# Gadersd/stable-diffusion-burn

Hardware: AMD Instinct MI355X
Metric: images/sec @512x512, 20-step DDIM CFG=7.5, SD v1.4 (higher is better)
Workload: dtype f32

## Files before the change

### stable_diffusion_burn_amd/build.py

```python
from __future__ import annotations

import hashlib
import os
import subprocess
import sys
from concurrent.futures import ThreadPoolExecutor
from pathlib import Path

PKG = Path(__file__).resolve().parent
CSRC = PKG / "csrc"
LIBDIR = PKG / "lib"
LIB = LIBDIR / "libsdmi.so"
OBJDIR = PKG / "build"
BINDIR = PKG / "bin"
CLI = BINDIR / "sdmi_sample"

SOURCES = ["k_gemm.hip", "k_gemm2.hip", "k_gemm2x.hip", "k_gemm3x.hip", "k_gemm3p.hip", "k_gemm_bf16.hip", "k_gemm_bf16x.hip", "k_gemm_bf16t.hip", "k_attn.hip", "k_attn_bf16.hip", "k_attn_split.hip", "k_norm.hip", "k_elem.hip", "k_img2img.hip", "k_inpaint.hip", "k_control.hip", "k_sampler.hip", "k_resize.hip", "k_lora.hip", "k_unpack.hip", "k_bf16.hip", "k_fp8.hip", "engine.cpp", "gemm_plan.cpp", "attn_plan.cpp", "multi.cpp", "mpk_reader.cpp", "safetensors_reader.cpp", "ckpt_keys.cpp", "lora_keys.cpp", "tokenizer.cpp", "prompt.cpp", "png_writer.cpp", "sdmi_capi.cpp"]
CLI_SOURCE = "sample_main.cpp"
HEADERS = [CLI_SOURCE] + sorted(p.name for p in CSRC.glob("*.hpp")) + sorted(p.name for p in CSRC.glob("*.inc")) + ["../../include/sdmi.h"]
ARCH = "gfx950"
CXXFLAGS = ["-O3", "-std=c++17", "-fPIC", f"--offload-arch={ARCH}", "-Wall", "-Wno-unused-function"]


def hipcc() -> str:
# ... 2 lines not shown
            return cand
    raise RuntimeError("hipcc not found")


_TOOLCHAIN = None


def _toolchain() -> bytes:
    global _TOOLCHAIN
    if _TOOLCHAIN is None:
        try:
            _TOOLCHAIN = subprocess.run([hipcc(), "--version"], capture_output=True, text=True, timeout=60).stdout.encode()
        except Exception:
            _TOOLCHAIN = b"unknown"
    return _TOOLCHAIN


def _digest() -> str:
    h = hashlib.sha256()
    h.update(_toolchain())
    for name in SOURCES + HEADERS:
        h.update(name.encode())
        h.update((CSRC / name).read_bytes())
    h.update(" ".join(CXXFLAGS).encode())
    return h.hexdigest()


def gen_tuning_table() -> None:
    _gen_table("gfx950_fp32.txt", "tuning_table.inc")
    _gen_table("gfx950_fp32_mfma.txt", "tuning_table_mfma.inc")
    _gen_table("gfx950_bf16.txt", "tuning_table_bf16.inc")
    _gen_table("gfx950_fp32_planes.txt", "tuning_table_planes.inc")
    _gen_table("gfx950_fp32_pairs.txt", "tuning_table_pairs.inc")


def _gen_table(src_name: str, out_name: str) -> None:
    src = PKG / "tuning" / src_name
    lines = []
    if src.exists():
        for ln in src.read_text().split():
            if "=" in ln and not ln.startswith("#"):
                key, val = ln.split("=")
                cfg, splits = val.split(",")
                lines.append(f'{{"{key}", {int(cfg)}, {int(splits)}}},')
    out = CSRC / out_name
    text = f"// generated by build.py from tuning/{src_name} -- do not edit\n" + "\n".join(lines) + "\n"
    if not out.exists() or out.read_text() != text:
        out.write_text(text)


def _unit_digest(src: str) -> str:
    h = hashlib.sha256()
    h.update(_toolchain())
    for name in [src] + HEADERS:
        h.update(name.encode())
        h.update((CSRC / name).read_bytes())
    h.update(" ".join(CXXFLAGS).encode())
    return h.hexdigest()


def _compile(src: str) -> Path:
    obj = OBJDIR / (src.replace("/", "_") + ".o")
    stamp = obj.with_suffix(".sha256")
    digest = _unit_digest(src)
    if obj.exists() and stamp.exists() and stamp.read_text().strip() == digest and not os.environ.get("SDMI_REBUILD_ALL"):
        return obj
# ... 42 lines not shown
```

### stable_diffusion_burn_amd/csrc/engine.cpp

```cpp
#include "engine.hpp"
#include "ckpt_keys.hpp"
#include "lora_keys.hpp"
#include "mpk_reader.hpp"
#include "safetensors_reader.hpp"

#include <dlfcn.h>

#include <algorithm>
#include <cmath>
#include <cstdarg>
#include <cstdio>
#include <cstring>
#include <fstream>
#include <sstream>

namespace sdmi {

static constexpr size_t kAlign = 256;
static constexpr size_t kSlabMin = (size_t)1 << 30;

DevPool::~DevPool() {
    for (auto& s : slabs_) (void)hipFree(s.base);
}

// ... 385 lines not shown
        s.fold_entries[2] = entry_index_.at(path + "/proj_out/weight");
    };

    add(this, "alphas_cumprod", 3, {1000}, nullptr);
    add_meta("n_steps", 1, 1000.f, 0.f, nullptr);

    lin(lin1_time_, "unet/lin1_time_embed", mc, ed, true, true);
    lin(lin2_time_, "unet/lin2_time_embed", ed, ed, true, true);
    struct Spec { BlockKind kind; const char* name; int cin, cout; };
    const Spec in_spec[12] = {
        {BK_CONV, "conv", cfg_.unet_in_ch, c1},   {BK_RES_ST, "rt1", c1, c1}, {BK_RES_ST, "rt2", c1, c1}, {BK_DOWN, "d1", c1, c1},
        {BK_RES_ST, "rt3", c1, c2}, {BK_RES_ST, "rt4", c2, c2}, {BK_DOWN, "d2", c2, c2},    {BK_RES_ST, "rt5", c2, c4},
        {BK_RES_ST, "rt6", c4, c4}, {BK_DOWN, "d3", c4, c4},    {BK_RES, "r1", c4, c4},     {BK_RES, "r2", c4, c4}};
    const Spec out_spec[12] = {
        {BK_RES, "r1", 2 * c4, c4},        {BK_RES, "r2", 2 * c4, c4},        {BK_RES_UP, "ru", 2 * c4, c4},
        {BK_RES_ST, "rt1", 2 * c4, c4},    {BK_RES_ST, "rt2", 2 * c4, c4},    {BK_RES_ST_UP, "rtu1", c4 + c2, c4},
        {BK_RES_ST, "rt3", c4 + c2, c2},   {BK_RES_ST, "rt4", 2 * c2, c2},    {BK_RES_ST_UP, "rtu2", c2 + c1, c2},
        {BK_RES_ST, "rt5", c2 + c1, c1},   {BK_RES_ST, "rt6", 2 * c1, c1},    {BK_RES_ST, "rt7", 2 * c1, c1}};
    in_blocks_.resize(12);
    out_blocks_.resize(12);
    auto def_block = [&](UBlock& b, const Spec& s, const std::string& root) {
        b.kind = s.kind; b.cin = s.cin; b.cout = s.cout;
        const std::string path = root + "/" + s.name;
        switch (s.kind) {
            case BK_CONV: conv(b.conv, path, s.cin, s.cout, 3); break;
            case BK_DOWN: conv(b.conv, path, s.cin, s.cout, 3, 2); fp8_copy(b.conv, path + "/weight"); break;
            case BK_RES: res(b.res, path, s.cin, s.cout, true); break;
            default:
                res(b.res, path + "/res", s.cin, s.cout, true);
                if (s.kind == BK_RES_ST || s.kind == BK_RES_ST_UP) spatial(b.st, path + "/transformer", s.cout);
                if (s.kind == BK_RES_UP || s.kind == BK_RES_ST_UP) { conv(b.up, path + "/upsample/conv", s.cout, s.cout, 3); fp8_copy(b.up, path + "/upsample/conv/weight"); }
        }
    };
    for (int i = 0; i < 12; ++i) def_block(in_blocks_[i], in_spec[i], "unet/input_blocks");
    res(mid_res1_, "unet/middle_block/res1", c4, c4, true);
    spatial(mid_st_, "unet/middle_block/transformer", c4);
    res(mid_res2_, "unet/middle_block/res2", c4, c4, true);
    for (int i = 0; i < 12; ++i) def_block(out_blocks_[i], out_spec[i], "unet/output_blocks");
    norm(unet_norm_out_, "unet/norm_out", c1);
    conv(unet_conv_out_, "unet/conv_out", c1, 4, 3);

    auto idx_res = [&](ResW& r) { r.temb_index = (int)res_list_.size(); res_list_.push_back(&r); };
    auto idx_st = [&](SpatialW& s) {
        s.ctx_index = (int)st_list_.size();
        st_list_.push_back(&s);
        for (int i : s.fold_entries) entries_[(size_t)i].fold_st = s.ctx_index;
    };
    auto idx_block = [&](UBlock& b) {
        if (b.kind == BK_CONV || b.kind == BK_DOWN) return;
        idx_res(b.res);
        if (b.kind == BK_RES_ST || b.kind == BK_RES_ST_UP) idx_st(b.st);
    };
    for (auto& b : in_blocks_) idx_block(b);
    idx_res(mid_res1_); idx_st(mid_st_); idx_res(mid_res2_);
    for (auto& b : out_blocks_) idx_block(b);
    n_res_unet_ = res_list_.size();
    n_st_unet_ = st_list_.size();

    const int vc = cfg_.vae_ch;
    const int dch[4][2] = {{4 * vc, 4 * vc}, {4 * vc, 4 * vc}, {4 * vc, 2 * vc}, {2 * vc, vc}};
    conv(post_quant_, "autoencoder/post_quant_conv", 4, 4, 1);
    conv(dec_conv_in_, "autoencoder/decoder/conv_in", 4, 4 * vc, 3);
    res(dec_mid1_, "autoencoder/decoder/mid/block_1", 4 * vc, 4 * vc, false);
    dec_attn_.c = 4 * vc;
    norm(dec_attn_.norm, "autoencoder/decoder/mid/attn/norm", 4 * vc);
    conv(dec_attn_.q, "autoencoder/decoder/mid/attn/q", 4 * vc, 4 * vc, 1);
    conv(dec_attn_.k, "autoencoder/decoder/mid/attn/k", 4 * vc, 4 * vc, 1);
    conv(dec_attn_.v, "autoencoder/decoder/mid/attn/v", 4 * vc, 4 * vc, 1);
    conv(dec_attn_.proj_out, "autoencoder/decoder/mid/attn/proj_out", 4 * vc, 4 * vc, 1);
    res(dec_mid2_, "autoencoder/decoder/mid/block_2", 4 * vc, 4 * vc, false);
    for (int i = 0; i < 4; ++i) {
        DecBlockW& b = dec_blocks_[i];
        b.cin = dch[i][0]; b.cout = dch[i][1]; b.has_up = i != 3;
        const std::string bp = "autoencoder/decoder/blocks/" + std::to_string(i);
        res(b.res[0], bp + "/res1", b.cin, b.cout, false);
        res(b.res[1], bp + "/res2", b.cout, b.cout, false);
        res(b.res[2], bp + "/res3", b.cout, b.cout, false);
        if (b.has_up) conv(b.upsampler, bp + "/upsampler", b.cout, b.cout, 3);
    }
    norm(dec_norm_out_, "autoencoder/decoder/norm_out", vc);
    conv(dec_conv_out_, "autoencoder/decoder/conv_out", vc, 3, 3);

    if (cfg_.clip_layers > 0) {
        const int cs = cd, L = cfg_.clip_layers, H = cfg_.clip_heads;
        if (H <= 0 || cs % H || !attn_supported_head_dim(cs / H) || cfg_.clip_vocab <= 0 || cfg_.clip_ctx <= 0 || cs % 32)
            throw Error(SDMI_ERR_UNSUPPORTED, "CLIP: ctx_dim / clip_heads must be one of the fused attention head dims (40, 64, 80, 160)");
        cur_group_ = 1;
        add(this, "clip/token_embedding/weight", 2, {cfg_.clip_vocab, cs}, &clip_tok_);
        add(this, "clip/position_embedding/weight", 2, {cfg_.clip_ctx, cs}, &clip_pos_);
        clip_blocks_.resize(L);
        for (int i = 0; i < L; ++i) {
            ClipBlockW& b = clip_blocks_[i];
            const std::string bp = "clip/blocks/" + std::to_string(i);
            void* w = persistent_alloc((size_t)3 * cs * cs * sizeof(float));
            weight_allocs_.push_back(w);
            void* bias = persistent_alloc((size_t)3 * cs * sizeof(float));
            weight_allocs_.push_back(bias);
            b.q.bt = reinterpret_cast<float*>(w); b.k.bt = b.q.bt + (size_t)cs * cs; b.v.bt = b.q.bt + (size_t)2 * cs * cs;
            b.q.bias = reinterpret_cast<float*>(bias); b.k.bias = b.q.bias + cs; b.v.bias = b.q.bias + 2 * cs;
            norm(b.attn_ln, bp + "/attn_ln", cs, false);
            lin(b.q, bp + "/attn/query", cs, cs, true, true);
            lin(b.k, bp + "/attn/key", cs, cs, true, true);
            lin(b.v, bp + "/attn/value", cs, cs, true, true);
            lin(b.out, bp + "/attn/out", cs, cs, true, true);
            norm(b.mlp_ln, bp + "/mlp_ln", cs, false);
            lin(b.fc1, bp + "/mlp/fc1", cs, 4 * cs, true, true);
            lin(b.fc2, bp + "/mlp/fc2", 4 * cs, cs, true, true);
        }
        norm(clip_ln_, "clip/layer_norm", cs, false);
        cur_group_ = 0;
    }
// ... 565 lines not shown
}


void Engine::fold_weights(const float* proj_bt, const float* lin_bt, const float* lin_bias, int cout, int cmid, int k_main, float* wf, float* bf) {
    ProfScope ps(this, PC_OTHER, 2.0 * cout * (double)cmid * k_main, ((double)cout * cmid + (double)cmid * k_main + (double)cout * k_main) * 4.0);
    ps.set_tag("fold %d,%d,%d", cout, k_main, cmid);
    SDMI_HIP(launch_fold_matmul_f64(proj_bt, lin_bt, wf, cout, cmid, k_main, cmid, k_main, k_main, stream_));
    if (lin_bias) SDMI_HIP(launch_fold_matmul_f64(proj_bt, lin_bias, bf, cout, cmid, 1, cmid, 1, 1, stream_));
    else SDMI_HIP(hipMemsetAsync(bf, 0, (size_t)cout * sizeof(float), stream_));
}

void Engine::rebuild_folds() {
    if (bf16_) return;
    for (SpatialW* s : st_list_) {
        if (s->fold_fresh || s->fold_entries[0] < 0) continue;
        bool ready = true;
        for (int i : s->fold_entries) ready = ready && entries_[(size_t)i].set;
        const int C = s->c;
        if (!ready || C % 32 || !split_planes(s->proj_out.bt) || !split_planes(s->mlp_lin.bt)) continue;
        const size_t w_bytes = (size_t)C * 4 * C * sizeof(float);
        if (!s->fold_bt) {
            char* base = static_cast<char*>(persistent_alloc(w_bytes + (size_t)C * sizeof(float)));
            weight_allocs_.push_back(base);
            char* planes = static_cast<char*>(persistent_alloc(w_bytes / 2 * 3));
            weight_allocs_.push_back(planes);
            split_regions_.push_back(SplitRegion{base, w_bytes, planes});
            s->fold_bt = reinterpret_cast<float*>(base);
            s->fold_bias = reinterpret_cast<float*>(base + w_bytes);
        }
        fold_weights(s->proj_out.bt, s->mlp_lin.bt, s->mlp_lin.bias, C, C, 4 * C, s->fold_bt, s->fold_bias);
        SDMI_HIP(launch_pack_split3(s->fold_bt, const_cast<void*>(split_planes(s->fold_bt)), C, 4 * C, stream_, b3_grouped(C)));
        s->fold_fresh = true;
    }
}
bool Engine::lora_owned(const sdmi_lora* a) const { return a && std::find(loras_.begin(), loras_.end(), a) != loras_.end(); }

bool Engine::lora_active_on(int entry) const {
    for (const sdmi_lora* a : loras_) {
        if (a->scale == 0) continue;
        for (const LoraTarget& t : a->targets)
            if (t.entry == entry) return true;
    }
    return false;
}

void Engine::lora_refuse_bulk_load(const char* what) const {
    for (const sdmi_lora* a : loras_)
        if (a->scale != 0 && !a->targets.empty())
            throw Error(SDMI_ERR_STATE, std::string(what) + ": a LoRA adapter with a non-zero scale is attached: set its scale to 0 first");
}

sdmi_lora* Engine::lora_create() {
    if (!finalized_) throw Error(SDMI_ERR_STATE, "lora_create: weights not finalized");
    if (!opt_keep_masters_) throw Error(SDMI_ERR_STATE, "lora_create: the context keeps no fp32 master weights (option keep_masters=1, set before the weights are loaded)");
    sdmi_lora* a = new sdmi_lora{};
    a->engine = this;
    loras_.push_back(a);
    return a;
}

void Engine::lora_add(sdmi_lora* a, const char* target, const float* down, const float* up, int rank, float alpha) {
    if (!lora_owned(a)) throw Error(SDMI_ERR_INVALID, "lora_add: not an adapter of this context");
    if (!target || !down || !up) throw Error(SDMI_ERR_INVALID, "lora_add: null argument");
    if (a->scale != 0) throw Error(SDMI_ERR_STATE, "lora_add: targets are added while the adapter's scale is 0");
    auto it = entry_index_.find(target);
    if (it == entry_index_.end()) throw Error(SDMI_ERR_INVALID, std::string("lora_add: unknown tensor '") + target + "'");
    const WeightEntry& e = entries_[it->second];
// ... 344 lines not shown
    else if (key == "attn_kv_splits") aopt_.attn_kv_splits = std::stoi(value);
    else if (key == "attn_kv_prefer8") aopt_.attn_kv_prefer8 = std::stoi(value);
    else if (key == "b3_grouped") {
        if (!entries_.empty() && std::any_of(entries_.begin(), entries_.end(), [](const WeightEntry& w) { return w.set; }))
            throw Error(SDMI_ERR_STATE, "b3_grouped selects the layout the weight planes are packed in: set it before the first weight is loaded");
        opt_b3_grouped_ = std::stoi(value);
    }
    else if (key == "keep_masters") {
        if (std::any_of(entries_.begin(), entries_.end(), [](const WeightEntry& w) { return w.set; }) || arena_done_[0] || arena_done_[1] || arena_done_[2] || arena_done_[3])
            throw Error(SDMI_ERR_STATE, "keep_masters decides what the weight arenas hold: set it before the first weight is loaded");
        opt_keep_masters_ = std::stoi(value) != 0;
    }
    else if (key == "attn_pack_tail") aopt_.attn_pack_tail = (value == "default") ? AttnPlanOpts().attn_pack_tail : std::stoi(value);
    else if (key == "gn32_min_wgs") opt_gn32_min_wgs_ = (opt_gn32_min_wgs_ & ~0xFFFF) | (std::stoi(value) & 0xFFFF);
    else if (key == "gn32_stats_min_wgs") opt_gn32_min_wgs_ = (opt_gn32_min_wgs_ & 0xFFFF) | ((std::stoi(value) + 1) << 16);
    else if (key == "gn_target_wgs") gn_tune_.target_wgs = std::stoi(value);
    else if (key == "gn_max_threads") gn_tune_.max_threads = std::stoi(value);
    else if (key == "gn_unroll") gn_tune_.unroll = std::stoi(value);
    else if (key == "fp8_tile") opt_fp8_tile_ = (value == "auto") ? -1 : std::stoi(value);
    else if (key == "resid_acc") opt_resid_acc_ = std::stoi(value);
    else if (key == "attn_bf16") aopt_.attn_bf16 = std::stoi(value);
    else if (key == "attn_bf16_variant") aopt_.attn_bf16_variant = (value == "default") ? AttnPlanOpts().attn_bf16_variant : std::stoi(value, nullptr, 0);
    else if (key == "attn_split") aopt_.attn_split = std::stoi(value);
    else if (key == "gemm_bf16x") gopt_.gemm_bf16x = std::stoi(value);
    else if (key == "gemm_x32") gopt_.gemm_x32 = std::stoi(value);
    else if (key == "gemm_f32s") gopt_.gemm_f32s = std::stoi(value);
    else if (key == "bench_cold") opt_bench_cold_ = std::stoi(value);
    else if (key == "gemm_probe") opt_gemm_probe_ = std::stoi(value);
    else if (key == "conv3_reuse") gopt_.conv3_reuse = std::stoi(value);
    else if (key == "gemm_planes") gopt_.gemm_planes = (value == "default") ? GemmPlanOpts().gemm_planes : std::stoi(value);
    else if (key == "gemm3x_variant") opt_gemm3x_variant_ = (value == "default") ? kGemm3xVariantDefault : std::stoi(value);
    else if (key == "gemm_bf16x_variant") opt_gemm_bf16x_variant_ = (value == "default") ? kGemmBf16xVariantDefault : std::stoi(value);
    else if (key == "geglu_fuse") opt_geglu_fuse_ = std::stoi(value);
    else if (key == "record_shapes") { record_shapes_ = std::stoi(value) != 0; if (record_shapes_) { shape_counts_.clear(); choice_counts_.clear(); } }
    else if (key == "dump_shapes") {
        std::ofstream f(value);
        if (!f) throw Error(SDMI_ERR_IO, "dump_shapes: cannot write " + value);
        for (auto& kv : shape_counts_) f << kv.first << " " << kv.second << "\n";
    }
    else if (key == "dump_choices") {
        std::ofstream f(value);
        if (!f) throw Error(SDMI_ERR_IO, "dump_choices: cannot write " + value);
        for (auto& kv : choice_counts_) f << kv.first << " x" << kv.second << "\n";
    }
    else if (key == "profile") { prof_flush(); profiling_ = std::stoi(value) != 0; prof_tagging_ = std::stoi(value) >= 2; if (profiling_) prof_calibrate(); }
    else if (key == "dump_profile_tags") {
        prof_flush();
        std::ofstream f(value);
        if (!f) throw Error(SDMI_ERR_IO, "dump_profile_tags: cannot write " + value);
        for (auto& kv : prof_tags_) f << kv.second.ms << " " << kv.second.launches << " " << kv.second.flops << " " << kv.second.bytes << "\t" << kv.first << "\n";
    }
    else if (key == "profile_reset") prof_reset();
    else if (key == "tune" || key == "tune_bf16") tuning_.set(value, key == "tune_bf16");
    else if (key == "tune_clear") tuning_.clear();
    else throw Error(SDMI_ERR_INVALID, "unknown option '" + key + "'");
}

void Engine::set_resid_acc(ConvGemm& p, bool eligible, bool resid_ok) const {
    p.resid_acc = 0;
    if (!eligible || (p.N % 8) || (p.ldc % 8)) return;
    if ((opt_resid_acc_ & 1) && p.resid && resid_ok && (p.ldr % 4) == 0 && ((uintptr_t)p.resid & 7) == 0) p.resid_acc |= 1;
    if ((opt_resid_acc_ & 2) && (p.bias || p.rowvec) && (p.rowvec_stride % 4) == 0 && (((uintptr_t)p.bias | (uintptr_t)p.rowvec) & 15) == 0) p.resid_acc |= 2;
}

void Engine::record_choice(const ConvGemm& p, const char* kind, int cfg, const char* note) {
    if (!record_shapes_) return;
// ... 80 lines not shown
    std::unique_ptr<Buf> a3_tmp;
    if (a_planes && !p.A3) {
        const long long rows = (long long)p.NB * p.Hs * p.Ws;
        p.a3_ld = (p.Cin / 32) * 192;
        a3_tmp.reset(new Buf(this, (size_t)rows * p.a3_ld));
        ProfScope ps(this, PC_SPLIT_ROWS, 0, (double)rows * p.Cin * 10.0);
        SDMI_HIP(launch_split3_rows(p.A, a3_tmp->p, rows, p.Cin, p.a_ld, p.a3_ld, stream_));
        count_kernel();
        p.A3 = a3_tmp->p;
    }
    set_resid_acc(p, in_dt && g.tile.family == kFamX && g.splits == 1, !p.geglu);
    record_choice(p, "", g.cfg, p.Bt3 || in_dt ? "" : " (no planes)");
    const double a_es = in_dt ? 2.0 : (a_planes ? 6.0 : 4.0), w_es = in_dt ? 2.0 : (w_planes ? 6.0 : 4.0);
    const double c_es = in_dt ? (p.out_mode == 1 ? 4.0 : 2.0) : (p.out_mode == 2 ? 2.0 : ((p.C ? 4.0 : 0.0) + (c3_native ? 6.0 : 0.0)));
    const double gemm_bytes = (double)p.NB * p.Hs * p.Ws * p.Cin * a_es + (double)p.N * (p.geglu ? 2.0 : 1.0) * p.K * w_es + (double)p.M * p.N * c_es;
    static const GemmLauncher kLaunchers[2][kNumGemmFamilies] = {{launch_conv_gemm2, launch_conv_gemm2x, launch_conv_gemm3x, launch_conv_gemm3p},
                                                                 {launch_conv_gemm_bf16, launch_conv_gemm_bf16_large, nullptr, nullptr}};
    run_gemm(p, GemmRun{kLaunchers[in_dt ? 1 : 0][g.tile.family], g.tile.index, "gemm", g.cfg, w_planes ? PC_CONV_SPLIT : PC_CONV_GEMM, in_dt != 0, true, flops, gemm_bytes});
    if (c3_want && !c3_native) {
        ProfScope ps(this, PC_SPLIT_ROWS, 0, (double)p.M * p.N * 10.0);
        SDMI_HIP(launch_split3_rows(p.C, c3_want, p.M, p.N, p.ldc, ldc3_want, stream_));
        count_kernel();
    }
}

void Engine::conv(const ConvW& w, const Act& x, Act& y, int stride, int ups, const float* rowvec, int rowvec_stride,
                  const Act* resid, bool pad_br) {
    if (x.c != w.cin) throw Error(SDMI_ERR_INVALID, "conv: input channels mismatch");
    const int pad = pad_br ? 0 : (w.k == 3 ? 1 : 0);
    const int hin = x.h << ups, win = x.w << ups;
    const int extra = pad_br ? 1 : 0;
    const int ho = (hin + 2 * pad + extra - w.k) / stride + 1, wo = (win + 2 * pad + extra - w.k) / stride + 1;
    if (y.n != x.n || y.h != ho || y.w != wo || y.c != w.cout) throw Error(SDMI_ERR_INVALID, "conv: output shape mismatch");
    ConvGemm p{};
    const int resid_dt = (!x.dt && y.dt) ? 0 : y.dt;
    if (resid && !x.dt && y.dt && (w.cout % 4 || y.stride() % 4 || resid->stride() % 4))
        throw Error(SDMI_ERR_STATE, "conv: a residual on an fp32 -> bf16 layer needs cout and the row strides to be multiples of 4");
    if (resid && (resid->rows() != y.rows() || resid->c != y.c || resid->dt != resid_dt)) throw Error(SDMI_ERR_STATE, "conv: residual shape / type mismatch");
    p.A = x.p; p.Bt = w.bt; p.C = y.p; p.bias = w.bias; p.rowvec = rowvec; p.resid = resid ? resid->p : nullptr;
    if (resid && !resid->p) throw Error(SDMI_ERR_STATE, "conv: the residual must exist as fp32");
    if (!x.dt && plane_gemm(w.cin, w.cout) && split_planes(w.bt)) { p.A3 = x.p3; p.a3_ld = x.ld3; }
    if (!x.p && !p.A3) throw Error(SDMI_ERR_STATE, "conv: the input exists only as planes, which this layer cannot read");
    p.C3 = y.p3; p.ldc3 = y.ld3;
    p.M = x.n * ho * wo; p.N = w.cout; p.K = w.cin * w.k * w.k;
    p.NB = x.n; p.Hs = x.h; p.Ws = x.w; p.Cin = w.cin; p.Ho = ho; p.Wo = wo;
    p.KH = w.k; p.KW = w.k; p.stride = stride; p.pad = pad; p.ups = ups;
    p.ldc = y.stride(); p.ldr = resid ? resid->stride() : y.stride(); p.a_ld = x.stride(); p.b_ld = p.K; p.rowvec_stride = rowvec_stride;
    p.CS = std::min(32, w.cin);
    if (!y.p && !y.p3) throw Error(SDMI_ERR_STATE, "conv: no output buffer");
    if (x.dt != w.dt) throw Error(SDMI_ERR_STATE, "conv: activation / weight storage types disagree");
    p.out_mode = x.dt ? (y.dt ? 0 : 1) : (y.dt ? 2 : 0);
    launch_gemm(p, x.dt);
}

bool Engine::conv_pair(const ConvW& w_out, const Act& h, const ConvW& w_skip, const Act& x, Act& y) {
    if (bf16_ || h.dt || x.dt || y.dt || w_out.dt || w_skip.dt || w_out.k != 3 || w_skip.k != 1 || probe_buf_) return false;
    if (h.c != w_out.cin || x.c != w_skip.cin || w_out.cout != w_skip.cout || y.c != w_out.cout) return false;
    if (h.n != x.n || h.h != x.h || h.w != x.w || y.n != h.n || y.h != h.h || y.w != h.w) return false;
    if (!plane_gemm(w_out.cin, w_out.cout) || !plane_gemm(w_skip.cin, w_skip.cout) || !h.p3 || !x.p3 || (!y.p && !y.p3)) return false;
    if (gopt_.force_splits > 0 && opt_splitk_aux_ <= 0) return false;
    ConvGemm p{};
    p.Bt = w_out.bt; p.bias = w_out.bias; p.bias_aux = w_skip.bias;
    p.Bt3 = split_planes(w_out.bt); p.Bt3_aux = split_planes(w_skip.bt);
    if (!p.Bt3 || !p.Bt3_aux) return false;
    p.A3 = h.p3; p.a3_ld = h.ld3; p.A3_aux = x.p3; p.a3_ld_aux = x.ld3;
    p.C = y.p; p.C3 = y.p3; p.ldc3 = y.ld3;
    p.M = (int)h.rows(); p.N = w_out.cout; p.K = w_out.cin * 9;
    p.NB = h.n; p.Hs = h.h; p.Ws = h.w; p.Cin = w_out.cin; p.Ho = h.h; p.Wo = h.w;
    p.KH = 3; p.KW = 3; p.stride = 1; p.pad = 1; p.ups = 0;
    p.ldc = y.p ? y.stride() : p.N; p.ldr = p.ldc; p.a_ld = h.stride(); p.b_ld = p.K; p.CS = 32;
    p.kt_total = p.K / 32; p.Cin_aux = w_skip.cin; p.kt_total_aux = w_skip.cin / 32;
    p.b3_grouped = b3_grouped(p.N) ? 1 : 0;
    p.variant = opt_gemm3x_variant_;
    p.zero_page = zero_page_;
    if (!splitk_reduce_vec(p, false) || ((uintptr_t)p.bias_aux & 15) || (p.C3 && (p.N % 32 || p.ldc3 % 192))) return false;
    const GemmPlanIn in = gemm_plan_in(p, 0, -1, 0);
    if (!in.p_ok) return false;
    if ((unsigned long long)p.N * (unsigned long long)p.kt_total_aux * 192ull >= 0xFFFFFF00ull || (unsigned long long)p.NB * p.Hs * p.Ws * (unsigned long long)p.a3_ld_aux >= 0xFFFFFF00ull) return false;
    const GemmPairPlan g = plan_gemm_pair(in, w_skip.cin, p.kt_total_aux, gopt_, tuning_, opt_splitk_aux_ > 0 ? std::max(gopt_.force_splits, 1) : 0, std::max(opt_splitk_aux_, 0));
    if (!g.pair) return false;
    p.kt_per_split = g.kt_per_split; p.splits = g.splits_main + g.splits_aux; p.z_aux = g.splits_main;
    if (record_shapes_) {
        char note[48];
        std::snprintf(note, sizeof note, " +aux K%d z%d", w_skip.cin, p.z_aux);
        record_choice(p, " pair", g.cfg, note);
// ... 1592 lines not shown
        Act r = y;
        r.view = true; r.p3 = nullptr;
        r.ld = epi->resid_ld ? epi->resid_ld : y.c;
        r.p = const_cast<float*>(stage_epi(rb, epi->resid, y.rows(), y.c, r.ld, y.dt, (long long)y.h * y.w));
        return r;
    };
    if (!opt_op_f32_ && fp8_ && opt_fp8_convs_ && k == 3 && stride == 1 && !ups && cin % 32 == 0 && cout % 8 == 0) {
        const int cp = (cin + 127) / 128 * 128;
        ConvW w; w.cin = cin; w.cout = cout; w.k = 3; w.dt = 1; w.bias = const_cast<float*>(bias);
        Buf bt8(this, (size_t)cout * cp * 9), bs8(this, (size_t)cout * cp * 9 / 32);
        SDMI_HIP(launch_pack_conv_weight_fp8(wt, bt8.p, bs8.p, cout, cin, 3, 3, stream_));
        w.bt8 = bt8.f(); w.bs8 = bs8.f();
        Act a32 = new_act(n, h, wd, cin, 0);
        SDMI_HIP(launch_nchw_to_nhwc(x, a32.p, n, cin, h, wd, 1.0f, stream_));
        ActQ q = new_actq(n, h, wd, cin);
        SDMI_HIP(launch_quantize_fp8(a32.p, q.q, q.s, a32.rows(), cin, stream_));
        release(a32);
        Act y = new_act(n, h, wd, cout, 1);
        Act r;
        if (epi && epi->resid) r = epi_resid(y);
        conv_fp8(w, q, y, temb, r.p ? &r : nullptr, 1, 0, epi ? epi->temb_stride : 0);
        SDMI_HIP(launch_nhwc_bf16_to_nchw_f32(y.p, out, n, cout, h, wd, stream_));
        release(q); release(y);
        return;
    }
    ConvW w; w.cin = cin; w.cout = cout; w.k = k;
    w.dt = (bf16_ && cin % 64 == 0 && !opt_op_f32_) ? 1 : 0;
    if (bf16_ && !w.dt && cin >= 32 && !opt_op_f32_) throw Error(SDMI_ERR_UNSUPPORTED, "bf16 conv2d: Cin must be a multiple of 64 (or < 32)");
    Buf bt(this, (size_t)cout * cin * k * k * 4);
    if (w.dt) SDMI_HIP(launch_pack_conv_weight_bf16(wt, bt.p, cout, cin, k, k, stream_));
    else SDMI_HIP(launch_pack_conv_weight(wt, bt.f(), cout, cin, k, k, stream_));
    TempSplit planes(this, bt.f(), w.dt ? 0 : cout, (long long)cin * k * k);
    w.bt = bt.f(); w.bias = const_cast<float*>(bias);
    Act a = new_act(n, h, wd, cin, w.dt);
    if (w.dt) SDMI_HIP(launch_nchw_f32_to_nhwc_bf16(x, a.p, n, cin, h, wd, 1.0f, stream_));
    else SDMI_HIP(launch_nchw_to_nhwc(x, a.p, n, cin, h, wd, 1.0f, stream_));
    const int hin = h << ups, win = wd << ups;
    const int ho = (hin + 2 * pad - k) / stride + 1, wo = (win + 2 * pad - k) / stride + 1;
    Act y = new_act(n, ho, wo, cout, (bf16_ && cout > 4 && !opt_op_f32_) ? 1 : 0);
    const bool with_resid = opt_op_resid_ && cin == cout && stride == 1 && !ups && a.dt == y.dt;
    Act r;
    if (epi && epi->resid) r = epi_resid(y);
    conv(w, a, y, stride, ups, temb, epi ? epi->temb_stride : 0, r.p ? &r : with_resid ? &a : nullptr);
    if (y.dt) SDMI_HIP(launch_nhwc_bf16_to_nchw_f32(y.p, out, n, cout, ho, wo, stream_));
    else SDMI_HIP(launch_nhwc_to_nchw(y.p, out, n, cout, ho, wo, stream_));
    release(a); release(y);
}

void Engine::op_conv2d_pair(const float* x, const float* hp, const float* w_skip, const float* b_skip, const float* w_out, const float* b_out, int n, int cin_x, int cout,
                            int h, int wd, float* out, float* out3) {
    if (n <= 0 || h <= 0 || wd <= 0 || cin_x <= 0 || cout <= 0) throw Error(SDMI_ERR_INVALID, "conv2d_pair: bad shape");
    if (bf16_ || !plane_gemm(cin_x, cout) || !plane_gemm(cout, cout)) throw Error(SDMI_ERR_UNSUPPORTED, "conv2d_pair: the fp32 plane kernels only (channels in multiples of 32)");
    Buf bt_o(this, (size_t)cout * cout * 9 * 4), bt_s(this, (size_t)cout * cin_x * 4);
    SDMI_HIP(launch_pack_conv_weight(w_out, bt_o.f(), cout, cout, 3, 3, stream_));
    SDMI_HIP(launch_pack_conv_weight(w_skip, bt_s.f(), cout, cin_x, 1, 1, stream_));
    TempSplit po(this, bt_o.f(), cout, (long long)cout * 9), psk(this, bt_s.f(), cout, cin_x);
    ConvW wo; wo.cin = cout; wo.cout = cout; wo.k = 3; wo.bt = bt_o.f(); wo.bias = const_cast<float*>(b_out);
    ConvW ws; ws.cin = cin_x; ws.cout = cout; ws.k = 1; ws.bt = bt_s.f(); ws.bias = const_cast<float*>(b_skip);
    Act ax = new_act3(n, h, wd, cin_x, 3), ah = new_act3(n, h, wd, cout, 3);
    SDMI_HIP(launch_nchw_to_nhwc(x, ax.p, n, cin_x, h, wd, 1.0f, stream_));
    SDMI_HIP(launch_nchw_to_nhwc(hp, ah.p, n, cout, h, wd, 1.0f, stream_));
    SDMI_HIP(launch_split3_rows(ax.p, ax.p3, ax.rows(), cin_x, cin_x, ax.ld3, stream_));
    SDMI_HIP(launch_split3_rows(ah.p, ah.p3, ah.rows(), cout, cout, ah.ld3, stream_));
    Act y = new_act3(n, h, wd, cout, out3 ? 3 : 1);
    if (opt_skip_slices_) {
        if (!conv_pair(wo, ah, ws, ax, y)) throw Error(SDMI_ERR_UNSUPPORTED, "conv2d_pair: this shape / these options do not pair (skip_slices=0 runs the two launches)");
// ... 86 lines not shown
            if (y.p) SDMI_HIP(hipMemcpyAsync(yp, y.p, y.bytes(), hipMemcpyDeviceToDevice, stream_));
            if (y.p3) SDMI_HIP(launch_join3_rows(y.p3, y.p ? yp3 : yp, y.rows(), v.out_ld, y.ld3, v.out_ld, stream_));
        }
    };
    try {
        Act xs = slice(a, v.in_off, cin), ys = slice(y, v.out_off, cout);
        std::unique_ptr<Buf> tb, rb;
        const float* temb = (epi && epi->temb) ? stage_epi(tb, epi->temb, epi->temb_stride ? n : 1, cout, epi->temb_stride ? epi->temb_stride : cout, 0) : nullptr;
        Act r;
        if (epi && epi->resid) {
            if (!ys.p) throw Error(SDMI_ERR_INVALID, "view: a residual needs the output as fp32");
            r = ys;
            r.view = true; r.p3 = nullptr;
            r.ld = epi->resid_ld ? epi->resid_ld : cout;
            r.p = const_cast<float*>(stage_epi(rb, epi->resid, ys.rows(), cout, r.ld, ydt, (long long)ho * wo));
        }
        if (q8) {
            const int cp = (cin + 127) / 128 * 128;
            ConvW w; w.cin = cin; w.cout = cout; w.k = 3; w.dt = 1; w.bias = const_cast<float*>(bias);
            Buf bt8(this, (size_t)cout * cp * 9), bs8(this, (size_t)cout * cp * 9 / 32);
            SDMI_HIP(launch_pack_conv_weight_fp8(wt, bt8.p, bs8.p, cout, cin, 3, 3, stream_));
            w.bt8 = bt8.f(); w.bs8 = bs8.f();
            ActQ q = new_actq(n, h, wd, cin);
            quantize(xs, q);
            conv_fp8(w, q, ys, temb, r.p ? &r : nullptr, 1, 0, epi ? epi->temb_stride : 0);
            release(q);
        } else {
            ConvW w; w.cin = cin; w.cout = cout; w.k = k; w.dt = wdt;
            Buf bt(this, (size_t)cout * cin * k * k * 4);
            if (w.dt) SDMI_HIP(launch_pack_conv_weight_bf16(wt, bt.p, cout, cin, k, k, stream_));
            else SDMI_HIP(launch_pack_conv_weight(wt, bt.f(), cout, cin, k, k, stream_));
            TempSplit planes(this, bt.f(), w.dt ? 0 : cout, (long long)cin * k * k);
            w.bt = bt.f(); w.bias = const_cast<float*>(bias);
            conv(w, xs, ys, stride, ups, temb, epi ? epi->temb_stride : 0, r.p ? &r : nullptr);
        }
    } catch (...) {
        try { give_back(); } catch (...) {}
        throw;
    }
    give_back();
    release(a); release(y);
}

void Engine::op_linear_view(const float* x, const float* wt, const float* bias, int rows, int cin, int cout, const sdmi_op_view& v, const EpiOps* epi, float* yp) {
    check_view(v, cin, cout);
    if (v.in_ld != cin || v.in_off || v.in_planes > 1 || v.out_planes > 1)
        throw Error(SDMI_ERR_UNSUPPORTED, "linear view: Engine::gemm reads dense rows and writes fp32 / bf16 slices only");
    const int rld = (epi && epi->resid) ? (epi->resid_ld ? epi->resid_ld : cout) : 0;
    const bool q8 = fp8_ && opt_fp8_ops_ && cin % 32 == 0 && cout % 8 == 0;
    const int dt = (q8 || (bf16_ && cin % 64 == 0)) ? 1 : 0;
    Act y = new_act(1, 1, rows, v.out_ld, dt);
    if (dt) SDMI_HIP(launch_f32_to_bf16(yp, y.p, (long long)rows * v.out_ld, stream_));
    else SDMI_HIP(hipMemcpyAsync(y.p, yp, y.bytes(), hipMemcpyDeviceToDevice, stream_));
    auto give_back = [&] {
        if (dt) SDMI_HIP(launch_nhwc_bf16_to_nchw_f32(y.p, yp, rows, v.out_ld, 1, 1, stream_));
        else SDMI_HIP(hipMemcpyAsync(yp, y.p, y.bytes(), hipMemcpyDeviceToDevice, stream_));
    };
    try {
            Act ys = slice(y, v.out_off, cout);
            std::unique_ptr<Buf> rb;
            const float* resid = rld ? stage_epi(rb, epi->resid, rows, cout, rld, dt) : nullptr;
            if (q8) {
                const size_t kp = (size_t)(cin + 127) / 128 * 128;
                Buf xh(this, (size_t)rows * cin * 2), w8(this, (size_t)cout * kp), s8(this, (size_t)cout * kp / 32);
                SDMI_HIP(launch_f32_to_bf16(x, xh.p, (long long)rows * cin, stream_));
                SDMI_HIP(launch_pack_linear_weight_fp8(wt, w8.p, s8.p, cin, cout, stream_));
// ... 252 lines not shown
        try {
            conv_fp8(cw, q, y, nullptr, nullptr);
            SDMI_HIP(hipEventRecord(ev0_, stream_));
            for (int i = 0; i < iters; ++i) conv_fp8(cw, q, y, nullptr, nullptr);
            SDMI_HIP(hipEventRecord(ev1_, stream_));
            SDMI_HIP(hipEventSynchronize(ev1_));
            SDMI_HIP(hipEventElapsedTime(&ms, ev0_, ev1_));
        } catch (...) {
            release(x32); release(y); release(q);
            throw;
        }
        release(x32); release(y); release(q);
        return (double)ms / std::max(1, iters);
    }
    const int wdt = (bf16_ && cin % 64 == 0) ? 1 : 0;
    Act a = new_act(n, h, w, cin, wdt), y = new_act(n, ho, wo, cout, (bf16_ && cout > 4) ? 1 : 0);
    Buf bt(this, (size_t)cout * cin * k * k * 4), bias(this, (size_t)cout * 4);
    {
        Buf tmp(this, std::max((size_t)a.rows() * cin, (size_t)cout * cin * k * k) * 4);
        SDMI_HIP(launch_fill_normal(wdt ? tmp.f() : a.p, (long long)a.rows() * cin, 11, stream_));
        if (wdt) SDMI_HIP(launch_f32_to_bf16(tmp.f(), a.p, (long long)a.rows() * cin, stream_));
        SDMI_HIP(launch_fill_normal(wdt ? tmp.f() : bt.f(), (long long)cout * cin * k * k, 12, stream_));
        if (wdt) SDMI_HIP(launch_f32_to_bf16(tmp.f(), bt.p, (long long)cout * cin * k * k, stream_));
        SDMI_HIP(hipStreamSynchronize(stream_));
    }
    SDMI_HIP(launch_fill_normal(bias.f(), cout, 13, stream_));
    TempSplit planes(this, bt.f(), wdt ? 0 : cout, (long long)cin * k * k);
    const bool plane_tile = tile_cfg >= 0 && gemm_tile_id(tile_cfg).family == kFamP;
    if (!wdt && plane_tile && cin % 32 == 0) {
        a.p3 = pool_.alloc(a.bytes3()); a.ld3 = (cin / 32) * 192;
        SDMI_HIP(launch_split3_rows(a.p, a.p3, a.rows(), cin, cin, a.ld3, stream_));
    }
    ConvW cw; cw.cin = cin; cw.cout = cout; cw.k = k; cw.bt = bt.f(); cw.bias = bias.f(); cw.dt = wdt;
    const OptRestore r1{gopt_.force_tile}, r2{gopt_.force_splits}, r3{gopt_.gemm_planes};
    gopt_.force_tile = tile_cfg; gopt_.force_splits = splitk;
    if (plane_tile && !gopt_.gemm_planes) gopt_.gemm_planes = 2;
    float ms = 0;
    try {
        conv(cw, a, y, stride, ups, nullptr, 0, nullptr);
        if (opt_bench_cold_) {
            const size_t flush_bytes = (size_t)512 << 20;
            Buf flush(this, flush_bytes);
            Buf a_copy(this, a.bytes());
            SDMI_HIP(hipMemcpyAsync(a_copy.p, a.p, a.bytes(), hipMemcpyDeviceToDevice, stream_));
            for (int i = 0; i < iters; ++i) {
                SDMI_HIP(hipMemsetAsync(flush.p, i, flush_bytes, stream_));
                SDMI_HIP(hipMemcpyAsync(a.p, a_copy.p, a.bytes(), hipMemcpyDeviceToDevice, stream_));
                if (a.p3) SDMI_HIP(launch_split3_rows(a.p, a.p3, a.rows(), cin, cin, a.ld3, stream_));
                SDMI_HIP(hipEventRecord(ev0_, stream_));
                conv(cw, a, y, stride, ups, nullptr, 0, nullptr);
                SDMI_HIP(hipEventRecord(ev1_, stream_));
                SDMI_HIP(hipEventSynchronize(ev1_));
                float t = 0;
                SDMI_HIP(hipEventElapsedTime(&t, ev0_, ev1_));
                ms += t;
            }
        } else {
        SDMI_HIP(hipEventRecord(ev0_, stream_));
        for (int i = 0; i < iters; ++i) conv(cw, a, y, stride, ups, nullptr, 0, nullptr);
        SDMI_HIP(hipEventRecord(ev1_, stream_));
        SDMI_HIP(hipEventSynchronize(ev1_));
        SDMI_HIP(hipEventElapsedTime(&ms, ev0_, ev1_));
        }
        if (opt_gemm_probe_ && a.p3) {
            constexpr size_t kMaxBlocks = kGemmProbeBlocks;
            Buf pb(this, kMaxBlocks * 24 * sizeof(unsigned long long));
// ... 52 lines not shown
```

### stable_diffusion_burn_amd/csrc/engine.hpp

```cpp
#pragma once
#include <hip/hip_runtime.h>

#include <functional>
#include <map>
#include <memory>
#include <stdexcept>
#include <string>
#include <vector>

#include "../../include/sdmi.h"
#include "error.hpp"
#include "gemm_plan.hpp"
#include "kernels.hpp"

namespace sdmi {

#define SDMI_HIP(expr)                                                                                   \
    do {                                                                                                 \
        hipError_t _e = (expr);                                                                          \
        if (_e != hipSuccess)                                                                            \
            throw ::sdmi::Error(SDMI_ERR_HIP, std::string(#expr) + ": " + hipGetErrorString(_e) + " (" + \
                                                  __FILE__ + ":" + std::to_string(__LINE__) + ")");      \
    } while (0)

// ... 9 lines not shown
    void set_stream(hipStream_t s) { stream_ = s; }
    void set_fill(int byte) { fill_ = byte; }
    int fill() const { return fill_; }
    void note_fill(size_t bytes) { ++fill_blocks_; fill_bytes_ += bytes; }
    void take_fill_counts(unsigned long long* blocks, unsigned long long* bytes) { *blocks = fill_blocks_; *bytes = fill_bytes_; fill_blocks_ = fill_bytes_ = 0; }

private:
    struct Block { size_t off, size; };
    struct Slab { char* base; size_t size; std::vector<Block> free_list; };
    std::vector<Slab> slabs_;
    struct Live { int slab; size_t size; unsigned long long serial; };
    std::map<void*, Live> live_;
    size_t reserved_ = 0, in_use_ = 0, high_ = 0;
    unsigned long long serial_ = 0;
    hipStream_t stream_ = nullptr;
    int fill_ = -1;
    unsigned long long fill_blocks_ = 0, fill_bytes_ = 0;
};

struct Act {
    float* p = nullptr;
    int n = 0, h = 0, w = 0, c = 0;
    int dt = 0;
    int ld = 0;
    bool view = false;
    void* p3 = nullptr;
    int ld3 = 0;
    size_t bytes3() const { return (size_t)rows() * (size_t)(c / 32) * 192; }
    long long rows() const { return (long long)n * h * w; }
    int stride() const { return ld ? ld : c; }
    size_t bytes() const { return (size_t)rows() * c * (dt ? 2 : 4); }
};

struct ConvW { float* bt = nullptr; float* bias = nullptr; int cin = 0, cout = 0, k = 1; int dt = 0; float* bt8 = nullptr; float* bs8 = nullptr; };
struct ActQ {
    void* q = nullptr; void* s = nullptr;
    int n = 0, h = 0, w = 0, c = 0, cp = 0;
    long long rows() const { return (long long)n * h * w; }
};
struct LinW { float* bt = nullptr; float* bias = nullptr; int cin = 0, cout = 0; int dt = 0; float* bt8 = nullptr; float* bs8 = nullptr; };
struct NormW { float* gamma = nullptr; float* beta = nullptr; int c = 0; float eps = 1e-5f; };

struct ResW {
    NormW norm_in; ConvW conv_in; LinW lin_embed; NormW norm_out; ConvW conv_out; ConvW skip;
    bool has_skip = false, has_embed = false;
    int cin = 0, cout = 0, temb_index = -1;
};
struct MhaW { LinW q, k, v, out; };
struct SpatialW {
    NormW norm; ConvW proj_in, proj_out; NormW ln1, ln2, ln3; MhaW attn1, attn2; LinW geglu_proj, mlp_lin;
    int c = 0, ctx_index = -1;
    float* fold_bt = nullptr; float* fold_bias = nullptr;
    bool fold_fresh = false;
    int fold_entries[3] = {-1, -1, -1};
};
enum BlockKind { BK_CONV, BK_DOWN, BK_RES, BK_RES_ST, BK_RES_UP, BK_RES_ST_UP };
struct UBlock { BlockKind kind; int cin, cout; ConvW conv; ResW res; SpatialW st; ConvW up; };
struct VaeAttnW { NormW norm; ConvW q, k, v, proj_out; int c = 0; };
struct DecBlockW { ResW res[3]; ConvW upsampler; bool has_up = false; int cin = 0, cout = 0; };

struct ClipBlockW { NormW attn_ln, mlp_ln; LinW q, k, v, out, fc1, fc2; };

struct WeightEntry {
    std::string name;
    int kind;
    int ndim;
    int64_t dims[4];
    float** dst;
    int wdt = 0;
    int group = 0;
    float** dst8 = nullptr;
    float** dsts = nullptr;
    float pre_scale = 1.f;
    bool set = false;
    int fold_st = -1;
    float* master = nullptr;
};

struct LoraTarget { int entry; int rank; double alpha; const void* down; const void* up; int dtype = 0; int kind = 0; const void* down2 = nullptr; const void* up2 = nullptr; };

struct MetaEntry { std::string name; int n; float expect[2]; float* store; };

class Engine {
public:
    explicit Engine(const sdmi_config& cfg);
    ~Engine();
    Engine(const Engine&) = delete;
    Engine& operator=(const Engine&) = delete;

    void set_weight(const char* name, const float* data, int ndim, const int64_t* dims);
    void load_weights_dir(const char* dir);
    void load_weights_mpk(const char* path);
    void load_weights_safetensors(const char* path);
    void load_safetensors_groups(const char* path, bool control);
    void load_control_safetensors(const char* path);
    void load_weights_packed(const float* data, size_t n_floats, int groups);
    size_t packed_size(int groups) const;
    void finalize_weights();
    const std::vector<WeightEntry>& entries() const { return entries_; }
    sdmi_lora* lora_create();
    void lora_add(sdmi_lora* a, const char* target, const float* down, const float* up, int rank, float alpha);
    void lora_set_scale(sdmi_lora* a, double scale);
    void lora_destroy(sdmi_lora* a);
    sdmi_lora* lora_load_safetensors(const char* path, int which, int flags, int* n_skipped);
    static int64_t padded_conv_cin(int64_t cin);
    void effective_weight(const char* name, float* out, size_t n);

    void unet_forward_dev(const float* x_nchw, int t, const float* context, int n, int T, float* out_nchw, const float* cond_nchw = nullptr);
// ... 141 lines not shown
    std::vector<sdmi_lora*> loras_;
    bool lora_owned(const sdmi_lora* a) const;
    void lora_refuse_bulk_load(const char* what) const;
    bool lora_active_on(int entry) const;
    void lora_compose(int entry, float* dst);
    void lora_repack(int entry);
    void upload_weight(WeightEntry& e, const float* data);
    void stager_release();
    void ensure_arena(int group);
    bool set_meta(const std::string& name, const float* values, size_t n);
    void add_meta(const std::string& name, int n, float e0, float e1, float* store);
    std::vector<MetaEntry> meta_;
    std::map<std::string, int> meta_index_;
    void add_entry(const std::string& name, int kind, std::initializer_list<int64_t> dims, float** dst, int wdt = 0);
    int cur_group_ = 0;
    void build_model();

    Act new_act(int n, int h, int w, int c, int dt = -1);
    Act new_act3(int n, int h, int w, int c, int what);
    void release(Act& a);
    void probe_report(void* pb_dev, size_t max_blocks, int n, int cin, int h, int w, int cout, int k, int tile_cfg, int splitk);
    void conv(const ConvW& w, const Act& x, Act& y, int stride, int ups, const float* rowvec, int rowvec_stride,
              const Act* resid, bool pad_br = false);
    bool conv_pair(const ConvW& w_out, const Act& h, const ConvW& w_skip, const Act& x, Act& y);
    struct LinearPair {
        const void* u3; int u3_ld; const float* bt; const float* bias; int k_main;
        const void* h3; int h3_ld; const float* bt_aux; const float* bias_aux; int k_aux;
        int rows, cout; const float* resid; int ldr; float* C; int ldc; void* C3; int ldc3;
        bool measured_only = false;
    };
    bool linear_pair(const LinearPair& a, bool plan_only = false);
    void fold_weights(const float* proj_bt, const float* lin_bt, const float* lin_bias, int cout, int cmid, int k_main, float* wf, float* bf);
    void rebuild_folds();
    void fold_touch(const WeightEntry& e) { if (e.fold_st >= 0) st_list_[(size_t)e.fold_st]->fold_fresh = false; }
    static Act slice(const Act& parent, int c_off, int c);
    void gemm(const float* A, int a_rows, const float* bt, const float* bias, int cin, int cout, float* C, int ldc,
              const float* resid, int ldr, int dt = -1, int out_mode = 0, const void* A3 = nullptr, void* C3 = nullptr);
    bool plane_gemm(int cin, int cout) const { return !bf16_ && gopt_.gemm_planes != 0 && gopt_.gemm_f32s != 0 && cin % 32 == 0 && cout >= 32; }
    void launch_gemm(ConvGemm& p, int in_dt, int force_cfg = -1, int force_splits = 0);
    GemmPlanIn gemm_plan_in(const ConvGemm& p, int in_dt, int force_cfg, int force_splits) const;
    using GemmLauncher = hipError_t (*)(const ConvGemm&, int, hipStream_t);
    struct GemmRun { GemmLauncher launch; int index; const char* what; int cfg; int pc; bool bf16_reduce, reduce_tag; double flops, bytes; };
    void record_choice(const ConvGemm& p, const char* kind, int cfg, const char* note);
    void run_gemm(ConvGemm& p, const GemmRun& r);
    int edt() const { return bf16_ ? 1 : 0; }
    size_t esz() const { return bf16_ ? 2 : 4; }
    static float* adv(const float* p, long long elems, int dt) { return (float*)((char*)const_cast<float*>(p) + elems * (dt ? 2 : 4)); }
    void group_norm(const NormW& w, const Act& x, Act& y, bool silu);
    ActQ new_actq(int n, int h, int w, int c);
    void release(ActQ& a);
    void group_norm_fp8(const NormW& w, const Act& x, ActQ& y, bool silu);
    void conv_fp8(const ConvW& w, const ActQ& x, Act& y, const float* rowvec, const Act* resid, int stride = 1, int ups = 0, int rowvec_stride = 0);
    bool use_fp8(const ConvW& w, const Act& x) const;
    bool use_fp8_wide(const float* bt8, long long rows) const { return fp8_ && opt_fp8_convs_ && opt_fp8_linear_ && bt8 && rows >= opt_fp8_min_rows_; }
    void set_resid_acc(ConvGemm& p, bool eligible, bool resid_ok) const;
    void launch_fp8(ConvGemm& p, double flops);
    void gemm_fp8(const ActQ& x, const LinW& w, int n_rows_w, void* C, int ldc, const float* resid, int ldr);
    void conv_raw(const ConvW& w, const Act& x, Act& y, int stride, int ups);
    void quantize(const Act& x, ActQ& y);
    void layer_norm_fp8(const NormW& w, const float* x, long long rows, ActQ& y);
    ActQ new_rowsq(long long rows, int c) { return new_actq(1, 1, (int)rows, c); }
    void layer_norm(const NormW& w, const float* x, long long rows, float* y, int dt = -1, void* y3 = nullptr);
    void gemm_geglu(const float* x, long long rows, const float* bt, const float* bias, int cin, int hidden, float* out, int dt,
                    const void* x3 = nullptr, void* out3 = nullptr);
    void attention(const float* q, int ldq, long long q_bs, const float* k, int ldk, long long k_bs, const float* v,
                   int ldv, long long v_bs, float* o, int ldo, long long o_bs, int n, int nq, int nk, int n_head,
                   int d_head, const int* kv_len_dev, const int* kv_len_host, const float* mask, int mask_ld, int dt = -1, void* o3 = nullptr, bool q_log2 = false);
// ... 190 lines not shown
```

### stable_diffusion_burn_amd/csrc/gemm_plan.cpp

```cpp
#include "gemm_plan.hpp"

#include <algorithm>
#include <cstdio>

#include "error.hpp"

namespace sdmi {

struct TuneRow { const char* key; int cfg, splits; };
static const TuneRow kTuneRows[] = {
#include "tuning_table.inc"
    {nullptr, 0, 0},
#include "tuning_table_mfma.inc"
    {nullptr, 0, 0},
#include "tuning_table_planes.inc"
    {nullptr, 0, 0},
#include "tuning_table_bf16.inc"
    {nullptr, 0, 0}};

static const TuneRow kPairRows[] = {
#include "tuning_table_pairs.inc"
    {nullptr, 0, 0}};

struct CostRow { int bf16; GemmFamily family; int n; double eff[kNumGemmTiles]; double flop, rate, wg, area_num, area_den; };
static const CostRow kCost[] = {
    {0, kFam4, kNumGemmTiles, {0.85, 0.75, 0.60, 0.90, 0.75, 0.85, 0.75, 0.85, 0.65, 0.75}, 64.0, 256.0, 3000.0, 0.0, 1.0},
    {0, kFamX, kNumGemmTilesX, {0.90, 0.90, 0.88, 0.90}, 64.0, 256.0, 8000.0, 4.0, 10.0},
    {0, kFamS, kNumGemmTilesS, {0.55, 0.55, 0.52, 0.52, 0.46, 0.44}, 384.0, 4096.0, 8000.0, 4.0, 10.0},
    {0, kFamP, kNumGemmTilesP, {0.62, 0.60, 0.60, 0.52, 0.50, 0.34, 0.40, 0.50, 0.40}, 384.0, 4096.0, 8000.0, 4.0, 10.0},
    {1, kFam4, kNumGemmTiles, {0.31, 0.22, 0.16, 0.22, 0.20, 0.20, 0.22, 0.26, 0.15, 0.28}, 128.0, 4096.0, 3000.0, 0.0, 1.0},
    {1, kFamX, kNumGemmTilesX, {0.54, 0.46, 0.38, 0.48}, 128.0, 4096.0, 6000.0, 2.0, 20.0}};
static const int kSplitOpts[] = {1, 2, 3, 4, 6, 8, 12, 16, 24, 32, 48};

static TileChoice cost_model(int bf16, unsigned families, int M, int N, int kt_total, bool pairs_only) {
    const int n_cu = 256;
    double best = 1e300;
    TileChoice bc{0, 1};
    for (const CostRow& r : kCost) {
        if (r.bf16 != bf16 || !(families >> r.family & 1)) continue;
        for (int c = 0; c < r.n; ++c) {
            const GemmTileInfo& ti = kGemmFamilies[r.family].tiles[c];
            if (pairs_only && !ti.geglu_pairs) continue;
            const int bm = ti.bm, bn = ti.bn;
            const long long tiles = (long long)((M + bm - 1) / bm) * ((N + bn - 1) / bn);
            const double overhead = r.wg + bm * bn * r.area_num / r.area_den;
            for (int s : kSplitOpts) {
                if (s > 1 && kt_total / s < 4) break;
                const int kt_per = (kt_total + s - 1) / s;
                const long long wgs = tiles * ((kt_total + kt_per - 1) / kt_per);
                const double per_cu = (double)((wgs + n_cu - 1) / n_cu);
                double t = per_cu * ((double)bm * bn * kt_per * r.flop / r.rate / r.eff[c] + overhead);
                if (s > 1) t += 8000.0 + (double)M * N * 4.0 * (s + 1) / (5.0e12 / 2.4e9);
                if (t < best) { best = t; bc = {kGemmFamilies[r.family].base + c, s}; }
            }
        }
    }
    return bc;
}

static int clamp_splits(int splits, int kt_total, int* kt_per_split) {
    splits = std::max(1, std::min(splits, kt_total));
    *kt_per_split = (kt_total + splits - 1) / splits;
    return (kt_total + *kt_per_split - 1) / *kt_per_split;
}

static const TileChoice* find(const std::map<std::string, TileChoice>& m, const char* key) {
    const auto it = m.find(key);
    return it == m.end() ? nullptr : &it->second;
}

static TileChoice plane_choice(const GemmTuning& t, const char* key, int M, int N, int kt_total, bool pairs_only) {
    if (const TileChoice* tc = find(t.planes, key)) {
        const GemmTileId id = gemm_tile_id(tc->cfg);
        if (!(pairs_only && id.family == kFamP && id.in_range(false) && !id.info().geglu_pairs)) return *tc;
    }
    return cost_model(0, 1u << kFamP, M, N, kt_total, pairs_only);
}

void GemmTuning::load_builtin() {
    std::map<std::string, TileChoice>* const tables[] = {&f32, &mfma, &planes, &bf16};
    int t = 0;
    for (const TuneRow& r : kTuneRows)
        if (r.key) (*tables[t])[r.key] = TileChoice{r.cfg, r.splits};
        else ++t;
    for (const TuneRow& r : kPairRows)
        if (r.key) pairs[r.key] = TileChoice{r.cfg, r.splits};
}

void GemmTuning::set(const std::string& value, bool b16) {
    const size_t eq = value.find('=');
    if (eq == std::string::npos) throw Error(SDMI_ERR_INVALID, "tune expects M,N,K=cfg,splits");
    TileChoice tc{0, 1};
    if (!b16 && value.find('+') < eq) {
        if (std::sscanf(value.c_str() + eq + 1, "%d,%d", &tc.cfg, &tc.splits) != 2 || tc.splits < 0 || gemm_tile_id(tc.cfg).family != kFamP || !gemm_tile_id(tc.cfg).in_range(false))
            throw Error(SDMI_ERR_INVALID, "tune: a pair row is M,N,Kmain+Kaux=cfg,kt_per_split with a plane tile (300 + x)");
        pairs[value.substr(0, eq)] = tc;
        return;
    }
    if (std::sscanf(value.c_str() + eq + 1, "%d,%d", &tc.cfg, &tc.splits) != 2 || tc.cfg < 0 || tc.splits < 1 || !gemm_tile_id(tc.cfg).in_range(b16))
        throw Error(SDMI_ERR_INVALID, "tune: bad value");
    (b16 ? bf16 : (gemm_tile_id(tc.cfg).family == kFamP ? planes : f32))[value.substr(0, eq)] = tc;
}

GemmPlan plan_gemm(const GemmPlanIn& in, const GemmPlanOpts& o, const GemmTuning& t) {
    if (in.from_planes && !in.p_ok)
        throw Error(in.s_ok ? SDMI_ERR_UNSUPPORTED : SDMI_ERR_STATE,
                    in.s_ok ? "fp32 GEMM: an activation tensor stored as bf16 planes (6 bytes per element) reaches 4 GiB (32-bit piece offsets): lower the batch (at 64x64x960 the CFG "
                              "batch 2n must stay <= 182) or set option gemm_planes=0"
                            : "gemm: activation planes given for a layer the plane kernel does not take");
    auto applicable = [&](int f) { return f == kFam4 || in.bf16 || (f == kFamP ? in.p_ok : f == kFamS ? in.s_ok : in.x32_ok); };
    auto enabled = [&](int f) { return f == kFam4 || (in.bf16 ? o.gemm_bf16x != 0 : f == kFamX ? o.gemm_x32 != 0 : f == kFamS ? o.gemm_f32s != 0 : true); };
    auto usable = [&](const TileChoice* tc) { return tc && applicable(gemm_tile_id(tc->cfg).family) && enabled(gemm_tile_id(tc->cfg).family); };
    char key[64];
    std::snprintf(key, sizeof key, "%d,%d,%d", in.M, in.N, in.K);
    const TileChoice* const t1 = find(in.bf16 ? t.bf16 : t.f32, key);
    const TileChoice* const t2 = in.bf16 ? nullptr : find(t.mfma, key);
    TileChoice tc;
    if (in.from_planes) tc = plane_choice(t, key, in.M, in.N, in.kt_total, in.geglu != 0);
    else if (usable(t1)) tc = *t1;
    else if (usable(t2)) tc = *t2;
    else {
        unsigned fams = 0;
        for (int f : {kFam4, kFamX, kFamS})
            if (applicable(f) && enabled(f)) fams |= 1u << f;
        tc = cost_model(in.bf16, fams, in.M, in.N, in.kt_total, false);
    }
    bool tile_forced = false;
    if (o.force_tile >= 0 && (in.from_planes ? gemm_tile_id(o.force_tile).family == kFamP : applicable(gemm_tile_id(o.force_tile).family))) { tc.cfg = o.force_tile; tile_forced = true; }
    if (o.force_splits > 0) tc.splits = o.force_splits;
// ... 25 lines not shown
    const int ktm = main.kt_total;
    auto slices = [](int kt_total, int kt) { return (kt_total + kt - 1) / kt; };
    int kt = 0;
    if (force_main > 0 || force_aux > 0) {
        const int sm = std::max(1, std::min(force_main, ktm)), sa = std::max(1, std::min(force_aux, kt_aux));
        kt = std::max(slices(ktm, sm), slices(kt_aux, sa));
    } else {
        char key[80];
        std::snprintf(key, sizeof key, "%d,%d,%d+%d", main.M, main.N, main.K, k_aux);
        const TileChoice* const row = g.tile_forced ? nullptr : find(t.pairs, key);
        if (row) {
            if (row->splits <= 0) return pp;
            const GemmTileId id = gemm_tile_id(row->cfg);
            if (id.family != kFamP || !id.in_range(false)) throw Error(SDMI_ERR_INVALID, "pairs table: not a plane tile");
            pp.tile = id; pp.cfg = id.cfg();
            kt = std::min(row->splits, std::max(ktm, kt_aux));
        } else {
            if (g.splits <= 1) return pp;
            const GemmTileInfo& ti = g.tile.info();
            const long long tiles = (long long)((main.M + ti.bm - 1) / ti.bm) * ((main.N + ti.bn - 1) / ti.bn);
            const long long rounds_today = (tiles * g.splits + 255) / 256;
            for (int c = std::max(std::min(4, ktm), g.kt_per_split); c <= ktm; ++c)
                if ((tiles * (slices(ktm, c) + slices(kt_aux, c)) + 255) / 256 <= rounds_today) { kt = c; break; }
            if (!kt) return pp;
        }
    }
    pp.kt_per_split = kt;
    pp.splits_main = slices(ktm, kt);
    pp.splits_aux = slices(kt_aux, kt);
    pp.pair = true;
    return pp;
}

TileChoice plan_gemm_fp8(int M, int N, int kt_total, int fp8_tile, int force_splits, int* kt_per_split) {
    static const double kRate[kNumGemmTilesQ] = {2400.0, 2100.0, 1700.0};
    if (fp8_tile >= kNumGemmTilesQ) throw Error(SDMI_ERR_INVALID, "fp8_tile out of range");
    double best = 1e300;
    TileChoice bc{fp8_tile, 1};
    for (int c = std::max(fp8_tile, 0); c < (fp8_tile < 0 ? kNumGemmTilesQ : fp8_tile + 1); ++c) {
        const int bm = kTilesQ[c].bm, bn = kTilesQ[c].bn;
        const long long tiles = (long long)((M + bm - 1) / bm) * ((N + bn - 1) / bn);
        int s = 1;
        if (tiles <= 128) s = (int)std::max<long long>(1, std::min<long long>(kt_total / 4, (256 + tiles - 1) / tiles));
        const double rounds = (double)((tiles * s + 255) / 256);
        const double t = rounds * (double)bm * bn / kRate[c] / s + (s > 1 ? 0.15 * (double)bm * bn / kRate[c] : 0.0);
        if (t < best) { best = t; bc = {c, s}; }
    }
    if (force_splits > 0) bc.splits = force_splits;
    bc.splits = clamp_splits(bc.splits, kt_total, kt_per_split);
    return bc;
}

int plan_geglu_plane_tile(long long rows, int hidden, int cin, const GemmPlanOpts& o, const GemmTuning& t) {
    char key[64];
    std::snprintf(key, sizeof key, "%lld,%d,%d", rows, 2 * hidden, cin);
    const TileChoice tc = plane_choice(t, key, (int)rows, 2 * hidden, (cin + 31) / 32, false);
    const bool forced = o.force_tile >= 0 && gemm_tile_id(o.force_tile).family == kFamP;
    const GemmTileId id = gemm_tile_id(forced ? o.force_tile : tc.cfg);
    const bool wave_cols = !id.in_range(false) || id.info().geglu_wave_cols;
    return id.family == kFamP && wave_cols && (tc.splits == 1 || forced) && o.force_splits <= 1 ? id.cfg() : -1;
}

int plan_geglu_paired_tile(long long rows, int hidden, int fuse, bool f32s) {
    const long long mt = (rows + 255) / 256;
    const long long t256 = mt * ((hidden + 127) / 128), t128 = mt * ((hidden + 63) / 64);
    int cfg = -1;
// ... 8 lines not shown
```

### stable_diffusion_burn_amd/csrc/gemm_plan.hpp

```cpp
#pragma once
#include <map>
#include <string>

#include "gemm_tiles.hpp"

namespace sdmi {

struct TileChoice { int cfg; int splits; };

struct GemmPlanIn {
    int M, N, K, kt_total;
    int bf16;
    int geglu;
    int out_mode;
    bool x32_ok, s_ok, p_ok;
    bool from_planes;
    int force_cfg = -1, force_splits = 0;
    int KH, KW, stride, pad, ups, Cin, Hs, Ws, Ho, Wo;
    bool zero_page;
};

struct GemmPlanOpts {
    int force_tile = -1, force_splits = 0;
    int gemm_x32 = 1;
    int gemm_f32s = 1;
    int gemm_planes = 1;
    int gemm_bf16x = 1;
    int conv3_reuse = 1;
};

struct GemmTuning {
    std::map<std::string, TileChoice> f32;
    std::map<std::string, TileChoice> mfma;
    std::map<std::string, TileChoice> planes;
    std::map<std::string, TileChoice> bf16;
    std::map<std::string, TileChoice> pairs;
    void load_builtin();
    void set(const std::string& value, bool b16);
    void clear() { f32.clear(); mfma.clear(); planes.clear(); bf16.clear(); pairs.clear(); }
};

struct GemmPlan { GemmTileId tile; int cfg, splits, kt_per_split; bool tile_forced; };

GemmPlan plan_gemm(const GemmPlanIn& in, const GemmPlanOpts& o, const GemmTuning& t);

struct GemmPairPlan { bool pair; GemmTileId tile; int cfg, kt_per_split, splits_main, splits_aux; };
GemmPairPlan plan_gemm_pair(const GemmPlanIn& main, int k_aux, int kt_aux, const GemmPlanOpts& o, const GemmTuning& t, int force_main = 0, int force_aux = 0);
TileChoice plan_gemm_fp8(int M, int N, int kt_total, int fp8_tile, int force_splits, int* kt_per_split);
int plan_geglu_plane_tile(long long rows, int hidden, int cin, const GemmPlanOpts& o, const GemmTuning& t);
int plan_geglu_paired_tile(long long rows, int hidden, int fuse, bool f32s);

}
```

### stable_diffusion_burn_amd/csrc/k_fp8.hip

```cpp
#include "kernels.hpp"
#include "k_common.hpp"
#include "k_gemm_bf16_epi.hpp"

namespace sdmi {

typedef float f32x4 __attribute__((ext_vector_type(4)));
typedef unsigned int u32x4 __attribute__((ext_vector_type(4)));
typedef unsigned int u32x2 __attribute__((ext_vector_type(2)));
typedef int i32x8 __attribute__((ext_vector_type(8)));
typedef __attribute__((address_space(3))) void lds_void;
typedef __attribute__((address_space(1))) const void global_cvoid;

__device__ __forceinline__ float qbf16_lo(unsigned w) { return __uint_as_float(w << 16); }
__device__ __forceinline__ float qbf16_hi(unsigned w) { return __uint_as_float(w & 0xFFFF0000u); }
__device__ __forceinline__ unsigned qbf16_bits(float f) {
    unsigned u = __float_as_uint(f);
    u += 0x7FFFu + ((u >> 16) & 1u);
    return u >> 16;
}
__device__ __forceinline__ unsigned qpack_bf16x2(float a, float b) { return xpack_bf16x2(a, b); }

__device__ __forceinline__ unsigned mx_scale_byte(float amax, float* inv_scale) {
    const unsigned ex = (__float_as_uint(amax) >> 23) & 0xFFu;
    unsigned b = ex > 9u ? ex - 8u : 1u;
// ... 194 lines not shown
    const int a_base = wm * 16 * MI * 128;
    const int b_base = BM * 128 + wn * 16 * NI * 128;
    const int as_base = SCALE_OFF + (wm * 16 * MI + c15) * 4 + g4;
    const int bs_base = SCALE_OFF + BM * 4 + (wn * 16 * NI + c15) * 4 + g4;

    f32x4 acc[MI][NI];
    issue(0);
    gemm_acc_init_bf16<MI, NI, WM, WN, 0>(p, acc, m0, n0, wave, lane, HoWo);
    for (int t = 0; t < n_t; ++t) {
        const int cur = t & 1;
        sdmi_dma_landed();
        __syncthreads();
        if (t + 1 < n_t) issue(cur ^ 1);
        const unsigned char* stage = smem_q + cur * STAGE;
        constexpr int NH = (NI > 4) ? 2 : 1;
        constexpr int NI0 = (NI + NH - 1) / NH;
        mx_columns<MI, NI, 0, NI0>(stage, acc, a_base, b_base, as_base, bs_base, fr_off0, fr_off1);
        if constexpr (NH == 2) mx_columns<MI, NI, NI0, NI - NI0>(stage, acc, a_base, b_base, as_base, bs_base, fr_off0, fr_off1);
    }

    gemm_epilogue_bf16<MI, NI, WM, WN>(p, acc, smem_q, m0, n0, z, wave, lane, HoWo);
}

template <int MI, int NI, int WM, int WN>
static hipError_t launch_cfg_fp8x(const ConvGemm& p, dim3 grid, hipStream_t stream) {
    auto k = conv_gemm_fp8x_kernel<MI, NI, WM, WN>;
    constexpr size_t lds = 2 * (size_t)(16 * MI * WM + 16 * NI * WN) * 132;
    if (hipError_t e = set_max_dynamic_lds(reinterpret_cast<const void*>(k), (int)lds); e != hipSuccess) return e;
    hipLaunchKernelGGL(k, grid, dim3(512), lds, stream, p);
    return hipGetLastError();
}

hipError_t launch_conv_gemm_fp8x(const ConvGemm& p, int cfg, hipStream_t stream) {
    if (p.z_aux) return hipErrorInvalidValue;
    if (cfg < 0 || cfg >= kNumGemmTilesQ) return hipErrorInvalidValue;
    if ((p.a_ld % 128) || (p.b_ld % 128) || !p.zero_page || !p.a_scale || !p.b_scale || p.geglu) return hipErrorInvalidValue;
    if ((p.N & 7) || (p.ldc & 7) || (p.resid && (p.ldr & 7))) return hipErrorInvalidValue;
    const int bm = kTilesQ[cfg].bm, bn = kTilesQ[cfg].bn;
    const int MT = (p.M + bm - 1) / bm, NT = (p.N + bn - 1) / bn;
    const dim3 grid = gemm_grid(p, MT * NT);
    switch (cfg) {
        case 0: return launch_cfg_fp8x<8, 5, 2, 4>(p, grid, stream);
        case 1: return launch_cfg_fp8x<8, 4, 2, 4>(p, grid, stream);
        case 2: return launch_cfg_fp8x<4, 4, 4, 2>(p, grid, stream);
    }
    return hipErrorInvalidValue;
}

__global__ void pack_conv_weight_fp8_kernel(const float* __restrict__ w, unsigned char* __restrict__ bt, unsigned char* __restrict__ bs,
                                            int cout, int cin, int kh, int kw, int cp) {
    const int T = kh * kw;
    const int nblk = cp / 32;
    const long long total = (long long)cout * T * nblk;
    const long long Kp = (long long)cp * T;
    for (long long i = (long long)blockIdx.x * blockDim.x + threadIdx.x; i < total; i += (long long)gridDim.x * blockDim.x) {
        const int blk = (int)(i % nblk);
        const long long r = i / nblk;
        const int tap = (int)(r % T);
        const int n = (int)(r / T);
        const int c0 = blk * 32;
        float v[32];
        float amax = 0.f;
#pragma unroll
        for (int j = 0; j < 32; ++j) {
            const int c = c0 + j;
            v[j] = c < cin ? w[((long long)n * cin + c) * T + tap] : 0.f;
            amax = fmaxf(amax, fabsf(v[j]));
// ... 382 lines not shown
```

### stable_diffusion_burn_amd/csrc/k_gemm.hip

```cpp
#include "kernels.hpp"
#include "k_split3.hpp"

#include <mutex>
#include <set>
#include <utility>

namespace sdmi {

hipError_t set_max_dynamic_lds(const void* kernel, int bytes) {
    static std::mutex mu;
    static std::set<std::pair<const void*, int>> done;
    int dev = 0;
    hipError_t e = hipGetDevice(&dev);
    if (e != hipSuccess) return e;
    std::lock_guard<std::mutex> lock(mu);
    if (done.count({kernel, dev})) return hipSuccess;
    e = hipFuncSetAttribute(kernel, hipFuncAttributeMaxDynamicSharedMemorySize, bytes);
    if (e == hipSuccess) done.insert({kernel, dev});
    return e;
}

typedef float f32x4 __attribute__((ext_vector_type(4)));

template <int G>
__global__ __launch_bounds__(256) void splitk_reduce_kernel(const ConvGemm p) {
    const float* slabs = p.slabs;
    float* C = p.C;
    const int HoWo = p.Ho * p.Wo;
    const bool vec_ok = splitk_reduce_vec(p, false);
    if (vec_ok) {
        const int n4 = p.N >> 2;
        const long long total = (long long)p.M * n4;
        const long long rounded = (total * G + 255) / 256 * 256;
        for (long long t = (long long)blockIdx.x * blockDim.x + threadIdx.x; t < rounded; t += (long long)gridDim.x * blockDim.x) {
            const long long i = t / G;
            const int g = (int)(t - i * G);
            const bool live = i < total;
            const long long ii = live ? i : 0;
            const int m = (int)(ii / n4);
            const int n = (int)(ii - (long long)m * n4) * 4;
            const long long off = (long long)m * p.N + n;
            f32x4 eb = {0.f, 0.f, 0.f, 0.f}, ev = eb, er = eb;
            if (live && g == 0) {
                if (p.bias) eb = *reinterpret_cast<const f32x4*>(p.bias + n);
                if (p.bias_aux) eb += *reinterpret_cast<const f32x4*>(p.bias_aux + n);
                if (p.rowvec) ev = *reinterpret_cast<const f32x4*>(p.rowvec + (long long)(m / HoWo) * p.rowvec_stride + n);
                if (p.resid) er = *reinterpret_cast<const f32x4*>(p.resid + (long long)m * p.ldr + n);
            }
            f32x4 v = {0.f, 0.f, 0.f, 0.f};
            int s = g;
            for (; s + 3 * G < p.splits; s += 4 * G) {
                const f32x4 a0 = *reinterpret_cast<const f32x4*>(slabs + (long long)s * p.slab_stride + off);
                const f32x4 a1 = *reinterpret_cast<const f32x4*>(slabs + (long long)(s + G) * p.slab_stride + off);
                const f32x4 a2 = *reinterpret_cast<const f32x4*>(slabs + (long long)(s + 2 * G) * p.slab_stride + off);
                const f32x4 a3 = *reinterpret_cast<const f32x4*>(slabs + (long long)(s + 3 * G) * p.slab_stride + off);
                v += a0; v += a1; v += a2; v += a3;
            }
            for (; s < p.splits; s += G) v += *reinterpret_cast<const f32x4*>(slabs + (long long)s * p.slab_stride + off);
#pragma unroll
            for (int o = 1; o < G; o <<= 1) {
#pragma unroll
                for (int e = 0; e < 4; ++e) v[e] += __shfl_xor(v[e], o, 64);
            }
            if (live && g == 0) {
                if (p.bias || p.bias_aux) v += eb;
                if (p.rowvec) v += ev;
                if (p.resid) v += er;
                if (C) *reinterpret_cast<f32x4*>(C + (long long)m * p.ldc + n) = v;
                if (p.C3) s3_store4(reinterpret_cast<unsigned char*>(p.C3) + (long long)m * p.ldc3, n, v);
            }
        }
    } else {
        const long long total = (long long)p.M * p.N;
        for (long long i = (long long)blockIdx.x * blockDim.x + threadIdx.x; i < total;
             i += (long long)gridDim.x * blockDim.x) {
            const int m = (int)(i / p.N);
            const int n = (int)(i - (long long)m * p.N);
            float v = slabs[i];
            for (int s = 1; s < p.splits; ++s) v += slabs[s * p.slab_stride + i];
            if (p.bias_aux) v += (p.bias ? p.bias[n] : 0.f) + p.bias_aux[n];
            else if (p.bias) v += p.bias[n];
            if (p.rowvec) v += p.rowvec[(long long)(m / HoWo) * p.rowvec_stride + n];
            if (p.resid) v += p.resid[(long long)m * p.ldr + n];
            C[(long long)m * p.ldc + n] = v;
        }
    }
}

__global__ void pack_conv_weight_kernel(const float* __restrict__ w, float* __restrict__ bt, int cout, int cin,
                                        int kh, int kw) {
    const int T = kh * kw;
    const int CS = cin < 32 ? cin : 32;
    const long long K = (long long)cin * T;
    const long long total = (long long)cout * K;
    for (long long i = (long long)blockIdx.x * blockDim.x + threadIdx.x; i < total;
         i += (long long)gridDim.x * blockDim.x) {
        const int n = (int)(i / K);
        const int k = (int)(i - (long long)n * K);
        const int sl = k / CS;
        const int ci = k - sl * CS;
        const int cs = sl / T;
        const int tap = sl - cs * T;
        const int c = cs * CS + ci;
        bt[i] = w[((long long)n * cin + c) * T + tap];
    }
}

__global__ void pack_linear_weight_kernel(const float* __restrict__ w, float* __restrict__ bt, int cin, int cout) {
    __shared__ float tile[32][33];
    const int bx = blockIdx.x * 32, by = blockIdx.y * 32;
    const int tx = threadIdx.x & 31, ty = threadIdx.x >> 5;
    for (int r = ty; r < 32; r += 8) {
        const int ci = by + r, co = bx + tx;
        tile[r][tx] = (ci < cin && co < cout) ? w[(long long)ci * cout + co] : 0.f;
    }
    __syncthreads();
    for (int r = ty; r < 32; r += 8) {
        const int co = bx + r, ci = by + tx;
        if (co < cout && ci < cin) bt[(long long)co * cin + ci] = tile[tx][r];
    }
}

__global__ __launch_bounds__(256) void fold_matmul_f64_kernel(const float* __restrict__ a, const float* __restrict__ b, float* __restrict__ out, int N, int Cn, int K,
                                                             long long lda, long long ldb, long long ldo) {
    __shared__ float ta[16][17], tb[16][17];
    const int tx = threadIdx.x & 15, ty = threadIdx.x >> 4;
    const int n = blockIdx.y * 16 + ty, k = blockIdx.x * 16 + tx;
    double acc = 0.0;
    for (int c0 = 0; c0 < Cn; c0 += 16) {
        ta[ty][tx] = (n < N && c0 + tx < Cn) ? a[(long long)n * lda + c0 + tx] : 0.f;
        tb[ty][tx] = (c0 + ty < Cn && k < K) ? b[(long long)(c0 + ty) * ldb + k] : 0.f;
        __syncthreads();
#pragma unroll
        for (int c = 0; c < 16; ++c) acc += (double)ta[ty][c] * (double)tb[c][tx];
        __syncthreads();
    }
    if (n < N && k < K) out[(long long)n * ldo + k] = (float)acc;
}

hipError_t launch_fold_matmul_f64(const float* a, const float* b, float* out, int N, int Cn, int K, long long lda, long long ldb, long long ldo, hipStream_t s) {
    if (N <= 0 || Cn <= 0 || K <= 0 || lda < Cn || ldb < K || ldo < K) return hipErrorInvalidValue;
    const dim3 grid((unsigned)((K + 15) / 16), (unsigned)((N + 15) / 16));
    if (grid.y > 65535u) return hipErrorInvalidValue;
    hipLaunchKernelGGL(fold_matmul_f64_kernel, grid, dim3(256), 0, s, a, b, out, N, Cn, K, lda, ldb, ldo);
    return hipGetLastError();
}

hipError_t launch_splitk_reduce(const ConvGemm& p, hipStream_t stream) {
    const bool vec = splitk_reduce_vec(p, false);
    if (!vec && (p.C3 || !p.C)) return hipErrorInvalidValue;
    if (p.z_aux && p.rowvec) return hipErrorInvalidValue;
    if (p.bias_aux && vec && ((uintptr_t)p.bias_aux & 15)) return hipErrorInvalidValue;
    const long long work = ((long long)p.M * p.N + 3) / 4;
    int g = 1;
    if (vec)
        while (g < 8 && work * g < 262144 && 4 * g <= p.splits) g *= 2;
    long long blocks = (work * g + 255) / 256;
    if (blocks > 4096) blocks = 4096;
    if (blocks < 1) blocks = 1;
    switch (g) {
        case 1: hipLaunchKernelGGL(splitk_reduce_kernel<1>, dim3((unsigned)blocks), dim3(256), 0, stream, p); break;
        case 2: hipLaunchKernelGGL(splitk_reduce_kernel<2>, dim3((unsigned)blocks), dim3(256), 0, stream, p); break;
        case 4: hipLaunchKernelGGL(splitk_reduce_kernel<4>, dim3((unsigned)blocks), dim3(256), 0, stream, p); break;
        default: hipLaunchKernelGGL(splitk_reduce_kernel<8>, dim3((unsigned)blocks), dim3(256), 0, stream, p); break;
    }
    return hipGetLastError();
}

hipError_t launch_pack_conv_weight(const float* w, float* bt, int cout, int cin, int kh, int kw, hipStream_t s) {
    const long long total = (long long)cout * cin * kh * kw;
    int blocks = (int)((total + 255) / 256);
    if (blocks > 4096) blocks = 4096;
    hipLaunchKernelGGL(pack_conv_weight_kernel, dim3(blocks), dim3(256), 0, s, w, bt, cout, cin, kh, kw);
    return hipGetLastError();
}

hipError_t launch_pack_linear_weight(const float* w, float* bt, int cin, int cout, hipStream_t s) {
    dim3 grid((cout + 31) / 32, (cin + 31) / 32);
    hipLaunchKernelGGL(pack_linear_weight_kernel, grid, dim3(256), 0, s, w, bt, cin, cout);
    return hipGetLastError();
}

}
```

### stable_diffusion_burn_amd/csrc/k_gemm2.hip

```cpp
#include "kernels.hpp"
#include "k_common.hpp"

namespace sdmi {

typedef float f32x4 __attribute__((ext_vector_type(4)));
typedef unsigned int u32x4 __attribute__((ext_vector_type(4)));

constexpr unsigned kOob = 0xFFFFFFF0u;

__device__ __forceinline__ f32x4 buf_load16(__amdgpu_buffer_rsrc_t r, unsigned off) {
    return __builtin_bit_cast(f32x4, __builtin_amdgcn_raw_buffer_load_b128(r, (int)off, 0, 0));
}

template <int MI, int NI, int WM, int WN, bool GENERIC>
__global__ __launch_bounds__(256) void conv_gemm2_kernel(const ConvGemm p) {
    constexpr int BM = 16 * MI * WM;
    constexpr int BN = 16 * NI * WN;
    constexpr int PA = (BM + 31) / 32;
    constexpr int PB = (BN + 31) / 32;
    static_assert(WM * WN == 4, "4 waves per workgroup");

    extern __shared__ __attribute__((aligned(16))) float smem[];
    constexpr int BMR = PA * 32;
    constexpr int BNR = PB * 32;
// ... 227 lines not shown
                            if (p.bias) s += p.bias[n + r];
                            if (p.rowvec) s += p.rowvec[(long long)smp * p.rowvec_stride + n + r];
                            if (p.resid) s += p.resid[(long long)m * p.ldr + n + r];
                        }
                        Cbase[(long long)m * ldc + n + r] = s;
                    }
                }
            }
        }
    }
}

size_t gemm2_tile_lds_bytes(int cfg) {
    const int bmr = (gemm_tile_info(cfg).bm + 31) / 32 * 32, bnr = (gemm_tile_info(cfg).bn + 31) / 32 * 32;
    return (size_t)2 * (bmr + bnr) * 32 * sizeof(float);
}

template <int MI, int NI, int WM, int WN>
static hipError_t launch_cfg2(const ConvGemm& p, size_t lds, dim3 grid, hipStream_t stream) {
    const bool generic = (p.Cin % 32) != 0;
    if (generic) {
        auto k = conv_gemm2_kernel<MI, NI, WM, WN, true>;
        if (hipError_t e = set_max_dynamic_lds(reinterpret_cast<const void*>(k), (int)lds); e != hipSuccess) return e;
        hipLaunchKernelGGL(k, grid, dim3(256), lds, stream, p);
    } else {
        auto k = conv_gemm2_kernel<MI, NI, WM, WN, false>;
        if (hipError_t e = set_max_dynamic_lds(reinterpret_cast<const void*>(k), (int)lds); e != hipSuccess) return e;
        hipLaunchKernelGGL(k, grid, dim3(256), lds, stream, p);
    }
    return hipGetLastError();
}

hipError_t launch_conv_gemm2(const ConvGemm& p, int cfg, hipStream_t stream) {
    if (p.z_aux) return hipErrorInvalidValue;
    if (cfg < 0 || cfg >= kNumGemmTiles) return hipErrorInvalidValue;
    const int bm = gemm_tile_info(cfg).bm, bn = gemm_tile_info(cfg).bn;
    const int MT = (p.M + bm - 1) / bm, NT = (p.N + bn - 1) / bn;
    const int tiles = MT * NT;
    const dim3 grid = gemm_grid(p, tiles);
    const size_t lds = gemm2_tile_lds_bytes(cfg);
    switch (cfg) {
        case 0: return launch_cfg2<4, 4, 2, 2>(p, lds, grid, stream);
        case 1: return launch_cfg2<4, 2, 2, 2>(p, lds, grid, stream);
        case 2: return launch_cfg2<2, 2, 2, 2>(p, lds, grid, stream);
        case 3: return launch_cfg2<8, 4, 2, 2>(p, lds, grid, stream);
        case 4: return launch_cfg2<2, 5, 4, 1>(p, lds, grid, stream);
        case 5: return launch_cfg2<4, 5, 4, 1>(p, lds, grid, stream);
        case 6: return launch_cfg2<2, 4, 2, 2>(p, lds, grid, stream);
        case 7: return launch_cfg2<4, 5, 2, 2>(p, lds, grid, stream);
        case 8: return launch_cfg2<1, 5, 4, 1>(p, lds, grid, stream);
        case 9: return launch_cfg2<2, 5, 2, 2>(p, lds, grid, stream);
    }
    return hipErrorInvalidValue;
}

}
```

### stable_diffusion_burn_amd/csrc/k_gemm2x.hip

```cpp
#include "kernels.hpp"
#include "k_common.hpp"
#include "k_gemm_epi.hpp"

namespace sdmi {

typedef float f32x4 __attribute__((ext_vector_type(4)));
typedef unsigned int u32x4 __attribute__((ext_vector_type(4)));
typedef unsigned int u32x2 __attribute__((ext_vector_type(2)));
typedef __attribute__((address_space(3))) void lds_void;
typedef __attribute__((address_space(1))) const void global_cvoid;


template <int MI, int NI, int WM, int WN>
__global__ __launch_bounds__(512) void conv_gemm2x_kernel(const ConvGemm p) {
    constexpr int BM = 16 * MI * WM;
    constexpr int BN = 16 * NI * WN;
    static_assert(WM * WN == 8, "8 waves per workgroup");
    static_assert(BM % 64 == 0 && BN % 64 == 0, "every wave issues whole 8-row DMA pieces");
    constexpr int NA = BM / 64;
    constexpr int NB = BN / 64;
    constexpr int STAGE = (BM + BN) * 128;

    extern __shared__ __attribute__((aligned(16))) unsigned char smem_x32[];

// ... 133 lines not shown
                }
#pragma unroll
                for (int i = 0; i < GM; ++i)
#pragma unroll
                    for (int j = 0; j < 4; ++j)
#pragma unroll
                        for (int ni = 0; ni < NI; ++ni)
                            acc[g * GM + i][ni] = __builtin_amdgcn_mfma_f32_16x16x4f32(fb[ni][j], fa[g & 1][i][j], acc[g * GM + i][ni], 0, 0, 0);
            }
            __builtin_amdgcn_sched_group_barrier(0x100, NI + GM, 0);
#pragma unroll
            for (int g = 0; g < NG; ++g)
#pragma unroll
                for (int i = 0; i < GM; ++i) {
                    if (g + 1 < NG) __builtin_amdgcn_sched_group_barrier(0x100, 1, 0);
                    __builtin_amdgcn_sched_group_barrier(0x008, 4 * NI, 0);
                }
        }
    }

    gemm_epilogue_f32<MI, NI, WM, WN>(p, acc, smem_x32, m0, n0, z, lid, wave, lane, HoWo);
}

template <int MI, int NI, int WM, int WN>
static hipError_t launch_cfg_2x(const ConvGemm& p, dim3 grid, hipStream_t stream) {
    auto k = conv_gemm2x_kernel<MI, NI, WM, WN>;
    constexpr size_t lds = 2 * (size_t)(16 * MI * WM + 16 * NI * WN) * 128;
    if (hipError_t e = set_max_dynamic_lds(reinterpret_cast<const void*>(k), (int)lds); e != hipSuccess) return e;
    hipLaunchKernelGGL(k, grid, dim3(512), lds, stream, p);
    return hipGetLastError();
}

hipError_t launch_conv_gemm2x(const ConvGemm& p, int cfg, hipStream_t stream) {
    if (p.z_aux) return hipErrorInvalidValue;
    if (cfg < 0 || cfg >= kNumGemmTilesX) return hipErrorInvalidValue;
    if ((p.Cin % 32) || p.CS != 32 || !p.zero_page || p.out_mode != 0) return hipErrorInvalidValue;
    if (p.geglu && (cfg == 0 || cfg == 3 || p.splits != 1 || (p.N & 7) || (p.ldc & 7) || p.rowvec || p.resid)) return hipErrorInvalidValue;
    const int bm = gemm_tile_info_x(cfg).bm, bn = gemm_tile_info_x(cfg).bn;
    const int bno = p.geglu ? bn / 2 : bn;
    const int MT = (p.M + bm - 1) / bm, NT = (p.N + bno - 1) / bno;
    const int tiles = MT * NT;
    const dim3 grid = gemm_grid(p, tiles);
    switch (cfg) {
        case 0: return launch_cfg_2x<8, 5, 2, 4>(p, grid, stream);
        case 1: return launch_cfg_2x<8, 4, 2, 4>(p, grid, stream);
        case 2: return launch_cfg_2x<4, 4, 4, 2>(p, grid, stream);
        case 3: return launch_cfg_2x<4, 5, 2, 4>(p, grid, stream);
    }
    return hipErrorInvalidValue;
}

}
```

### stable_diffusion_burn_amd/csrc/k_gemm3p.hip

```cpp
#include "kernels.hpp"
#include "k_common.hpp"
#include "k_gemm_epi.hpp"
#include "k_split3.hpp"

namespace sdmi {

typedef float f32x4 __attribute__((ext_vector_type(4)));
typedef unsigned int u32x4 __attribute__((ext_vector_type(4)));
typedef unsigned int u32x2 __attribute__((ext_vector_type(2)));
typedef __bf16 bf16x8 __attribute__((ext_vector_type(8)));
typedef __attribute__((address_space(3))) void lds_void;
typedef __attribute__((address_space(1))) const void global_cvoid;

template <int MI, int NI, int NAG, int NBW, int A_BYTES, int NWV>
struct P3Wave {
    static constexpr int NA = 3 * NAG;
    static constexpr int NP = NA + NBW;
    static constexpr int NMF = 6 * NI;
    static constexpr int NAF = MI > 2 ? 3 : MI;
    static_assert(MI == 2 || MI == 4, "fragment rows per wave");
    static_assert(NI >= 2, "plane reads of a fragment take three instruction slots (behind())");

    f32x4 acc[MI][NI];
    u32x4 wf[3][NI];
// ... 96 lines not shown
        head_w<0>();
        __builtin_amdgcn_sched_barrier(0);
        rows<0>();
    }
};

template <int MI, int NI, int WM, int WN, int NSTG, bool PROBE = false>
__global__ __launch_bounds__(WM * WN * 64, 2) void conv_gemm3p_kernel(const ConvGemm p) {
    static_assert(NSTG == 2 || NSTG == 3, "LDS stages");
    constexpr int BM = 16 * MI * WM;
    constexpr int BN = 16 * NI * WN;
    constexpr int NWV = WM * WN;
    static_assert(NWV == 8 || NWV == 4, "8 or 4 waves per workgroup");
    static_assert(BM % (16 * NWV) == 0, "every wave owns whole 16-row fragment groups of the activation tile");
    constexpr int NAG = BM / (16 * NWV);
    constexpr int PW = (BN / 16) * 3;
    constexpr int NBW = (PW + NWV - 1) / NWV;
    constexpr int A_BYTES = (BM / 16) * 3 * 1024;
    constexpr int STAGE = A_BYTES + NBW * NWV * 1024;

    extern __shared__ __attribute__((aligned(16))) unsigned char smem_p3[];

    const int tid = threadIdx.x;
    const int lane = tid & 63;
    const int wave = __builtin_amdgcn_readfirstlane(tid >> 6);
    const int wm = wave / WN;
    const int wn = wave - wm * WN;

    constexpr int WNC = 16 * NI;
    const bool geglu = p.geglu != 0;
    const int BNO = geglu ? BN / 2 : BN;
    const int MT = (p.M + BM - 1) / BM;
    const int NT = (p.N + BNO - 1) / BNO;
    const GemmWork gw = gemm_work_of_block(p, MT, NT);
    if (!gw.live) return;
    const int lid = gw.lid;
    const int m0 = gw.tm * BM;
    const int n0 = gw.tn * BNO;
    const int z = gw.z;
    const bool aux = p.z_aux != 0 && z >= p.z_aux;
    const int kt_total = aux ? p.kt_total_aux : p.kt_total;
    const int kt_begin = (aux ? z - p.z_aux : z) * p.kt_per_split;
    const int kt_end = min(kt_begin + p.kt_per_split, kt_total);
    const int n_t = kt_end - kt_begin;
    const int KH = aux ? 1 : p.KH, KW = aux ? 1 : p.KW, pad = aux ? 0 : p.pad;
    const int T = KH * KW;
    const int HoWo = p.Ho * p.Wo;

    P3Wave<MI, NI, NAG, NBW, A_BYTES, NWV> w;
    w.Hin = p.Hs << p.ups;
    w.Win = p.Ws << p.ups;
    w.ups = p.ups;
    w.Ws = p.Ws;
    w.KH = KH;
    w.KW = KW;
    w.wave = wave;
    w.pix_bytes = (unsigned)(aux ? p.a3_ld_aux : p.a3_ld);
    w.Abase = reinterpret_cast<const char*>(aux ? p.A3_aux : p.A3);
    w.Wbase = reinterpret_cast<const char*>(aux ? p.Bt3_aux : p.Bt3);
    w.zero = reinterpret_cast<const char*>(p.zero_page);
    w.a_src = w.zero;

    const int r16 = lane >> 2;
    const int ch = (lane & 3) ^ ((-(r16 >> 2)) & 3);
#pragma unroll
    for (int j = 0; j < NAG; ++j) {
        const int m = m0 + (wave + NWV * j) * 16 + r16;
        const bool ok = m < p.M;
        const int mm = ok ? m : 0;
        const int nb = mm / HoWo;
        const int rem = mm - nb * HoWo;
        const int oy = rem / p.Wo;
        const int ox = rem - oy * p.Wo;
        w.a_off[j] = (unsigned)nb * (unsigned)(p.Hs * p.Ws) * w.pix_bytes + ch * 16;
        w.a_iy0[j] = ok ? oy * p.stride - pad : -(1 << 28);
        w.a_ix0[j] = ox * p.stride - pad;
    }
    const unsigned w_row_bytes = (unsigned)kt_total * 192u;
#pragma unroll
    for (int j = 0; j < NBW; ++j) {
        const int q = wave + NWV * j;
        const int f = q / 3, pl = q - 3 * f;
        int n = n0 + f * 16 + r16;
        long long wrow = n;
        if (p.geglu == 2) {
            const int fw = f / NI, ni = f - fw * NI;
            const int vg = fw / (WN / 2 > 0 ? WN / 2 : 1), col = fw - vg * (WN / 2);
            n = n0 + col * WNC + ni * 16 + r16;
            wrow = (long long)n + (vg ? p.N : 0);
        } else if (geglu) {
            const int fw = f / NI, ni = f - fw * NI;
            n = n0 + fw * (WNC / 2) + (ni >> 1) * 16 + r16;
            wrow = (long long)n + ((ni & 1) ? p.N : 0);
        }
        if (n >= p.N) wrow -= (n - (p.N - 1));
        w.w_off[j] = p.b3_grouped ? (unsigned)(wrow >> 4) * (w_row_bytes * 16u) + pl * 1024 + (unsigned)(wrow & 15) * 64 + ch * 16
                                  : (unsigned)wrow * w_row_bytes + pl * 64 + ch * 16;
    }
    w.w_kstep = p.b3_grouped ? 3072u : 192u;

    w.cs = kt_begin / T;
    const int tap0 = kt_begin - w.cs * T;
    w.ky = tap0 / KW;
    w.kx = tap0 - w.ky * KW;
    w.kt_next = kt_begin;
    w.kt_end = kt_end;

    const int c15 = lane & 15, g4 = lane >> 4;
    const int fr = c15 * 64 + ((g4 ^ ((-(c15 >> 2)) & 3)) << 4);
// ... 20 lines not shown
            unsigned long long pa = 0;
            if constexpr (PROBE) pa = __builtin_amdgcn_s_memtime();
            sdmi_dma_landed();
            __syncthreads();
            if constexpr (PROBE) pwait += __builtin_amdgcn_s_memtime() - pa;
            w.next_stage = smem_p3 + (cur ^ 1) * STAGE;
            w.a_tile = smem_p3 + cur * STAGE + a_fr;
            w.w_tile = smem_p3 + cur * STAGE + w_fr;
            w.tile();
        }
    } else {
        w.next_stage = smem_p3 + STAGE;
        w.template pieces<0, NAG * 3 + NBW>();
        int cur = 0;
        for (int t = 0; t < n_t; ++t) {
            unsigned long long pa = 0;
            if constexpr (PROBE) pa = __builtin_amdgcn_s_memtime();
            asm volatile("s_waitcnt vmcnt(%0)" ::"n"(NAG * 3 + NBW) : "memory");
            __builtin_amdgcn_s_barrier();
            asm volatile("" ::: "memory");
            if constexpr (PROBE) pwait += __builtin_amdgcn_s_memtime() - pa;
            const int nxt = cur == 0 ? 2 : cur - 1;
            w.next_stage = smem_p3 + nxt * STAGE;
            w.a_tile = smem_p3 + cur * STAGE + a_fr;
            w.w_tile = smem_p3 + cur * STAGE + w_fr;
            w.tile();
            cur = cur == 2 ? 0 : cur + 1;
        }
    }
    asm volatile("s_waitcnt vmcnt(0)" ::: "memory");
    unsigned long long pt2 = 0, pc2 = 0;
    if constexpr (PROBE) { pt2 = __builtin_amdgcn_s_memrealtime(); pc2 = __builtin_amdgcn_s_memtime(); }

    gemm_epilogue_f32<MI, NI, WM, WN>(p, w.acc, smem_p3, m0, n0, z, lid, wave, lane, HoWo);
    if constexpr (PROBE) {
        asm volatile("s_waitcnt vmcnt(0)" ::: "memory");
        __syncthreads();
        unsigned long long* d = p.probe + 24ull * (blockIdx.x + (unsigned long long)gridDim.x * blockIdx.z);
        if (lane == 0) { d[4 + 2 * wave] = pc2 - pc0; d[5 + 2 * wave] = pwait; }
        if (tid == 0) { d[0] = pt0; d[1] = pt1; d[2] = pt2; d[3] = __builtin_amdgcn_s_memrealtime(); }
    }
}

template <int MI, int NI, int WM, int WN, int NSTG, bool PROBE = false>
static hipError_t launch_cfg_3p(const ConvGemm& p, dim3 grid, hipStream_t stream) {
    auto k = conv_gemm3p_kernel<MI, NI, WM, WN, NSTG, PROBE>;
    constexpr int NWV = WM * WN;
    constexpr size_t stage = (size_t)(MI * WM) * 3 * 1024 + (size_t)((NI * WN * 3 + NWV - 1) / NWV) * NWV * 1024;
    constexpr size_t lds = NSTG * stage > (size_t)NWV * 16 * (16 * NI + 4) * 4 ? NSTG * stage : (size_t)NWV * 16 * (16 * NI + 4) * 4;
    static_assert(lds <= 160 * 1024, "the stages must fit the CU's LDS");
    hipError_t e = set_max_dynamic_lds(reinterpret_cast<const void*>(k), (int)lds);
    if (e != hipSuccess) return e;
    hipLaunchKernelGGL(k, grid, dim3(NWV * 64), lds, stream, p);
    return hipGetLastError();
}

hipError_t launch_conv_gemm3p(const ConvGemm& p, int cfg, hipStream_t stream) {
    if (cfg < 0 || cfg >= kNumGemmTilesP) return hipErrorInvalidValue;
    if ((p.Cin % 32) || p.CS != 32 || !p.zero_page || !p.Bt3 || !p.A3 || p.a3_ld <= 0 || (p.a3_ld % 192) || p.out_mode != 0) return hipErrorInvalidValue;
    const bool odd_ni = (cfg == 0 || cfg == 3 || cfg == 7);
    if (p.geglu == 1 && (odd_ni || p.splits != 1 || (p.N & 7) || (p.ldc & 7) || p.rowvec || p.resid)) return hipErrorInvalidValue;
    if (p.geglu == 2 && (cfg == 8 || p.splits != 1 || (p.N & 3) || (p.C && (p.ldc & 3)) || (p.C3 && (p.N & 31)) || p.rowvec || p.resid || (!p.C && !p.C3))) return hipErrorInvalidValue;
    if (p.geglu != 0 && p.geglu != 1 && p.geglu != 2) return hipErrorInvalidValue;
    if ((unsigned long long)p.N * (p.geglu ? 2 : 1) * (unsigned long long)p.kt_total * 192ull >= 0xFFFFFF00ull) return hipErrorInvalidValue;
    if ((unsigned long long)p.NB * p.Hs * p.Ws * (unsigned long long)p.a3_ld >= 0xFFFFFF00ull) return hipErrorInvalidValue;
    if (p.z_aux) {
        if (p.stride != 1 || p.ups != 0 || p.Hs != p.Ho || p.Ws != p.Wo || p.geglu || p.probe || p.rowvec) return hipErrorInvalidValue;
        if (!p.A3_aux || !p.Bt3_aux || p.Cin_aux <= 0 || (p.Cin_aux % 32) || p.kt_total_aux != p.Cin_aux / 32 || p.a3_ld_aux < p.kt_total_aux * 192 || (p.a3_ld_aux % 192)) return hipErrorInvalidValue;
        if (p.kt_per_split <= 0 || p.z_aux != (p.kt_total + p.kt_per_split - 1) / p.kt_per_split ||
            p.splits - p.z_aux != (p.kt_total_aux + p.kt_per_split - 1) / p.kt_per_split || !p.slabs) return hipErrorInvalidValue;
        if ((unsigned long long)p.N * (unsigned long long)p.kt_total_aux * 192ull >= 0xFFFFFF00ull) return hipErrorInvalidValue;
        if ((unsigned long long)p.NB * p.Hs * p.Ws * (unsigned long long)p.a3_ld_aux >= 0xFFFFFF00ull) return hipErrorInvalidValue;
    }
    const int bm = kTilesP[cfg].bm, bn = kTilesP[cfg].bn;
    const int bno = p.geglu ? bn / 2 : bn;
    const int MT = (p.M + bm - 1) / bm, NT = (p.N + bno - 1) / bno;
    const dim3 grid = gemm_grid(p, MT * NT);
    if (p.probe) {
        if ((unsigned long long)grid.x * grid.z > (unsigned long long)kGemmProbeBlocks) return hipErrorInvalidValue;
        switch (cfg) {
            case 0: return launch_cfg_3p<4, 5, 4, 2, 2, true>(p, grid, stream);
            case 3: return launch_cfg_3p<2, 5, 4, 2, 2, true>(p, grid, stream);
            case 4: return launch_cfg_3p<2, 4, 4, 2, 3, true>(p, grid, stream);
        }
        return hipErrorInvalidValue;
    }
    switch (cfg) {
        case 0: return launch_cfg_3p<4, 5, 4, 2, 2>(p, grid, stream);
        case 1: return launch_cfg_3p<4, 4, 4, 2, 2>(p, grid, stream);
        case 2: return launch_cfg_3p<4, 4, 2, 4, 2>(p, grid, stream);
        case 3: return launch_cfg_3p<2, 5, 4, 2, 2>(p, grid, stream);
        case 4: return launch_cfg_3p<2, 4, 4, 2, 3>(p, grid, stream);
        case 5: return launch_cfg_3p<2, 2, 2, 2, 3>(p, grid, stream);
        case 6: return launch_cfg_3p<2, 4, 2, 2, 2>(p, grid, stream);
        case 7: return launch_cfg_3p<4, 5, 1, 4, 2>(p, grid, stream);
        case 8: return launch_cfg_3p<2, 4, 4, 1, 2>(p, grid, stream);
    }
    return hipErrorInvalidValue;
}

__global__ void split3_rows_kernel(const float* __restrict__ x, unsigned short* __restrict__ y3, long long rows, int kt, long long ld, long long ld3_elems) {
    const long long total = rows * kt * 4;
    for (long long i = (long long)blockIdx.x * blockDim.x + threadIdx.x; i < total; i += (long long)gridDim.x * blockDim.x) {
        const int g = (int)(i & 3);
        const long long rk = i >> 2;
        const long long row = rk / kt;
        const int k = (int)(rk - row * kt);
        const float* src = x + row * ld + k * 32;
        const f32x4 lo = *reinterpret_cast<const f32x4*>(src + 4 * g);
// ... 47 lines not shown
```

### stable_diffusion_burn_amd/csrc/k_gemm3x.hip

```cpp
#include "kernels.hpp"
#include "k_common.hpp"
#include "k_gemm_epi.hpp"
#include "k_split3.hpp"

namespace sdmi {

typedef float f32x4 __attribute__((ext_vector_type(4)));
typedef float f32x2 __attribute__((ext_vector_type(2)));
typedef unsigned int u32x4 __attribute__((ext_vector_type(4)));
typedef __bf16 bf16x2 __attribute__((ext_vector_type(2)));
typedef __bf16 bf16x8 __attribute__((ext_vector_type(8)));
typedef __attribute__((address_space(3))) void lds_void;
typedef __attribute__((address_space(1))) const void global_cvoid;

template <int MI, int NI, int NA, int NBW, int PW, int A_BYTES, bool SPREAD, bool SCALAR, int NSTG = 2>
struct S3Wave {
    using S3Split = S3SplitT<SCALAR>;
    static constexpr int kS3Steps = S3Split::kSteps;
    static constexpr int NMF = 6 * NI;
    static constexpr int NP = NA + NBW;
    static constexpr int DMA_ROWS = (MI > 1) ? 2 : 1;

    f32x4 acc[MI][NI];
    u32x4 wf[3][NI];
// ... 222 lines not shown
    } else {
        w.next_stage = smem_x32 + STAGE;
        w.template pieces<0, NA + NBW>();
        int cur = 0;
        for (int t = 0; t < n_t; ++t) {
            asm volatile("s_waitcnt vmcnt(%0)" ::"n"(NA + NBW) : "memory");
            __builtin_amdgcn_s_barrier();
            asm volatile("" ::: "memory");
            const int nxt = cur == 0 ? 2 : cur - 1;
            w.next_stage = smem_x32 + nxt * STAGE;
            w.a_tile = smem_x32 + cur * STAGE + a_base;
            w.w_tile = smem_x32 + cur * STAGE + w_fr;
            w.tile();
            cur = cur == 2 ? 0 : cur + 1;
        }
    }
    asm volatile("s_waitcnt vmcnt(0)" ::: "memory");
    if (p.variant & 16) __builtin_amdgcn_s_setprio(0);

    gemm_epilogue_f32<MI, NI, WM, WN>(p, w.acc, smem_x32, m0, n0, z, lid, wave, lane, HoWo);
}

template <int MI, int NI, int WM, int WN, bool SPREAD, bool SCALAR, int NSTG = 2>
static hipError_t launch_cfg_3x(const ConvGemm& p, dim3 grid, hipStream_t stream) {
    auto k = conv_gemm3x_kernel<MI, NI, WM, WN, SPREAD, SCALAR, NSTG>;
    constexpr size_t lds = NSTG * ((size_t)(16 * MI * WM) * 128 + (size_t)((NI * WN * 3 + 7) / 8) * 8192);
    static_assert(lds <= 160 * 1024, "the stages must fit the CU's LDS");
    if (hipError_t e = set_max_dynamic_lds(reinterpret_cast<const void*>(k), (int)lds); e != hipSuccess) return e;
    hipLaunchKernelGGL(k, grid, dim3(512), lds, stream, p);
    return hipGetLastError();
}

hipError_t launch_conv_gemm3x(const ConvGemm& p, int cfg, hipStream_t stream) {
    if (p.z_aux) return hipErrorInvalidValue;
    if (cfg < 0 || cfg >= kNumGemmTilesS) return hipErrorInvalidValue;
    if ((p.Cin % 32) || p.CS != 32 || !p.zero_page || !p.Bt3 || p.out_mode != 0) return hipErrorInvalidValue;
    const bool odd_ni = (cfg == 0 || cfg == 1 || cfg == 4);
    if (p.geglu != 0 && p.geglu != 1) return hipErrorInvalidValue;
    if (p.geglu && (odd_ni || p.splits != 1 || (p.N & 7) || (p.ldc & 7) || p.rowvec || p.resid)) return hipErrorInvalidValue;
    if ((unsigned long long)p.N * (p.geglu ? 2 : 1) * (unsigned long long)p.kt_total * 192ull >= 0xFFFFFF00ull) return hipErrorInvalidValue;
    const int bm = kTilesS[cfg].bm, bn = kTilesS[cfg].bn;
    const int bno = p.geglu ? bn / 2 : bn;
    const int MT = (p.M + bm - 1) / bm, NT = (p.N + bno - 1) / bno;
    const int tiles = MT * NT;
    const dim3 grid = gemm_grid(p, tiles);
    const bool spread = !(p.variant & 1), scalar = (p.variant & 2) != 0;
#define SDMI_3X(MI, NI, WM, WN)                                                                                       \
    (spread ? (scalar ? launch_cfg_3x<MI, NI, WM, WN, true, true>(p, grid, stream) : launch_cfg_3x<MI, NI, WM, WN, true, false>(p, grid, stream)) \
            : (scalar ? launch_cfg_3x<MI, NI, WM, WN, false, true>(p, grid, stream) : launch_cfg_3x<MI, NI, WM, WN, false, false>(p, grid, stream)))
    switch (cfg) {
        case 0: return SDMI_3X(4, 5, 4, 2);
        case 1: return SDMI_3X(4, 5, 2, 4);
        case 2: return SDMI_3X(4, 4, 4, 2);
        case 3: return SDMI_3X(4, 4, 2, 4);
        case 4: return (p.variant & 4) ? SDMI_3X(2, 5, 4, 2) : (scalar ? launch_cfg_3x<2, 5, 4, 2, true, true, 3>(p, grid, stream) : launch_cfg_3x<2, 5, 4, 2, true, false, 3>(p, grid, stream));
        case 5: return (p.variant & 4) ? SDMI_3X(2, 4, 4, 2) : (scalar ? launch_cfg_3x<2, 4, 4, 2, true, true, 3>(p, grid, stream) : launch_cfg_3x<2, 4, 4, 2, true, false, 3>(p, grid, stream));
    }
#undef SDMI_3X
    return hipErrorInvalidValue;
}

__global__ void pack_split3_grouped_kernel(const float* __restrict__ x, unsigned short* __restrict__ y3, long long rows, int kt) {
    const long long total = rows * kt * 4;
    for (long long i = (long long)blockIdx.x * blockDim.x + threadIdx.x; i < total; i += (long long)gridDim.x * blockDim.x) {
        const int g = (int)(i & 3);
        const long long rk = i >> 2;
        const long long row = rk / kt;
// ... 27 lines not shown
```

### stable_diffusion_burn_amd/csrc/k_gemm_bf16.hip

```cpp
#include "kernels.hpp"
#include "k_common.hpp"

namespace sdmi {

typedef float f32x4 __attribute__((ext_vector_type(4)));
typedef unsigned int u32x4 __attribute__((ext_vector_type(4)));
typedef unsigned int u32x2 __attribute__((ext_vector_type(2)));
typedef __bf16 bf16x8 __attribute__((ext_vector_type(8)));

constexpr unsigned kOobB = 0xFFFFFFF0u;

__device__ __forceinline__ u32x4 buf_load16u(__amdgpu_buffer_rsrc_t r, unsigned off) {
    return __builtin_amdgcn_raw_buffer_load_b128(r, (int)off, 0, 0);
}
__device__ __forceinline__ float bf16_lo(unsigned w) { return __uint_as_float(w << 16); }
__device__ __forceinline__ float bf16_hi(unsigned w) { return __uint_as_float(w & 0xFFFF0000u); }
__device__ __forceinline__ unsigned f32_to_bf16_bits(float f) {
    unsigned u = __float_as_uint(f);
    u += 0x7FFFu + ((u >> 16) & 1u);
    return u >> 16;
}
typedef float g16_f32x2 __attribute__((ext_vector_type(2)));
typedef __bf16 g16_bf16x2 __attribute__((ext_vector_type(2)));
__device__ __forceinline__ unsigned pack_bf16x2(float a, float b) {
// ... 320 lines not shown
        const int sl = k / CS;
        const int ci = k - sl * CS;
        const int cs = sl / T;
        const int tap = sl - cs * T;
        const int c = cs * CS + ci;
        bt[i] = (unsigned short)f32_to_bf16_bits(w[((long long)n * cin + c) * T + tap]);
    }
}

__global__ void pack_linear_weight_bf16_kernel(const float* __restrict__ w, unsigned short* __restrict__ bt, int cin, int cout) {
    __shared__ float tile[32][33];
    const int bx = blockIdx.x * 32, by = blockIdx.y * 32;
    const int tx = threadIdx.x & 31, ty = threadIdx.x >> 5;
    for (int r = ty; r < 32; r += 8) {
        const int ci = by + r, co = bx + tx;
        tile[r][tx] = (ci < cin && co < cout) ? w[(long long)ci * cout + co] : 0.f;
    }
    __syncthreads();
    for (int r = ty; r < 32; r += 8) {
        const int co = bx + r, ci = by + tx;
        if (co < cout && ci < cin) bt[(long long)co * cin + ci] = (unsigned short)f32_to_bf16_bits(tile[tx][r]);
    }
}

template <int MI, int NI, int WM, int WN>
static hipError_t launch_cfg_bf16(const ConvGemm& p, size_t lds, dim3 grid, hipStream_t stream) {
    auto k = conv_gemm_bf16_kernel<MI, NI, WM, WN>;
    if (hipError_t e = set_max_dynamic_lds(reinterpret_cast<const void*>(k), (int)lds); e != hipSuccess) return e;
    hipLaunchKernelGGL(k, grid, dim3(256), lds, stream, p);
    return hipGetLastError();
}

hipError_t launch_conv_gemm_bf16(const ConvGemm& p, int cfg, hipStream_t stream) {
    if (p.z_aux) return hipErrorInvalidValue;
    if (cfg < 0 || cfg >= kNumGemmTiles) return hipErrorInvalidValue;
    if (p.Cin % 64) return hipErrorInvalidValue;
    const int bm = gemm_tile_info(cfg).bm, bn = gemm_tile_info(cfg).bn;
    const int MT = (p.M + bm - 1) / bm, NT = (p.N + bn - 1) / bn;
    const int tiles = MT * NT;
    const dim3 grid = gemm_grid(p, tiles);
    const size_t lds = gemm2_tile_lds_bytes(cfg);
    switch (cfg) {
        case 0: return launch_cfg_bf16<4, 4, 2, 2>(p, lds, grid, stream);
        case 1: return launch_cfg_bf16<4, 2, 2, 2>(p, lds, grid, stream);
        case 2: return launch_cfg_bf16<2, 2, 2, 2>(p, lds, grid, stream);
        case 3: return launch_cfg_bf16<8, 4, 2, 2>(p, lds, grid, stream);
        case 4: return launch_cfg_bf16<2, 5, 4, 1>(p, lds, grid, stream);
        case 5: return launch_cfg_bf16<4, 5, 4, 1>(p, lds, grid, stream);
        case 6: return launch_cfg_bf16<2, 4, 2, 2>(p, lds, grid, stream);
        case 7: return launch_cfg_bf16<4, 5, 2, 2>(p, lds, grid, stream);
        case 8: return launch_cfg_bf16<1, 5, 4, 1>(p, lds, grid, stream);
        case 9: return launch_cfg_bf16<2, 5, 2, 2>(p, lds, grid, stream);
    }
    return hipErrorInvalidValue;
}

hipError_t launch_splitk_reduce_bf16(const ConvGemm& p, hipStream_t stream) {
    if (p.z_aux) return hipErrorInvalidValue;
    const bool vec = splitk_reduce_vec(p, true);
    const long long work = (long long)p.M * p.N / (vec ? 4 : 1);
    int blocks = (int)((work + 255) / 256);
    if (blocks > 4096) blocks = 4096;
    if (blocks < 1) blocks = 1;
    hipLaunchKernelGGL(splitk_reduce_bf16_kernel, dim3(blocks), dim3(256), 0, stream, p);
    return hipGetLastError();
}

hipError_t launch_pack_conv_weight_bf16(const float* w, void* bt, int cout, int cin, int kh, int kw, hipStream_t s) {
    const long long total = (long long)cout * cin * kh * kw;
    int blocks = (int)((total + 255) / 256);
    if (blocks > 4096) blocks = 4096;
    hipLaunchKernelGGL(pack_conv_weight_bf16_kernel, dim3(blocks), dim3(256), 0, s, w, reinterpret_cast<unsigned short*>(bt), cout, cin, kh, kw);
    return hipGetLastError();
}

hipError_t launch_pack_linear_weight_bf16(const float* w, void* bt, int cin, int cout, hipStream_t s) {
    dim3 grid((cout + 31) / 32, (cin + 31) / 32);
    hipLaunchKernelGGL(pack_linear_weight_bf16_kernel, grid, dim3(256), 0, s, w, reinterpret_cast<unsigned short*>(bt), cin, cout);
    return hipGetLastError();
}

}
```

### stable_diffusion_burn_amd/csrc/k_gemm_bf16t.hip

```cpp
#include "kernels.hpp"
#include "k_common.hpp"
#include "k_gemm_bf16_epi.hpp"
#include <type_traits>

namespace sdmi {

typedef float f32x4 __attribute__((ext_vector_type(4)));
typedef unsigned int u32x4 __attribute__((ext_vector_type(4)));
typedef __bf16 bf16x8 __attribute__((ext_vector_type(8)));
typedef __attribute__((address_space(3))) void lds_void;
typedef __attribute__((address_space(1))) const void global_cvoid;

template <int NI, int WF>
__global__ __launch_bounds__(512) void conv3_gemm_bf16t_kernel(const ConvGemm p) {
    constexpr int MI = 8, WM = 2, WN = 4;
    constexpr int BM = 16 * MI * WM;
    constexpr int BN = 16 * NI * WN;
    constexpr int W = 16 * WF;
    constexpr int RPT = BM / W;
    constexpr int PADW = W + 2;
    constexpr int A_ROWS = (RPT * PADW + 7) / 8 * 8;
    constexpr int PA = A_ROWS / 8;
    constexpr int NAJ = (PA + 7) / 8;
    constexpr int NB = BN / 64;
// ... 130 lines not shown
                        acc[gg * GM + i][ni] = __builtin_amdgcn_mfma_f32_16x16x32_bf16(__builtin_bit_cast(bf16x8, fb[ni]), __builtin_bit_cast(bf16x8, fa[gg & 1][i]),
                                                                                   acc[gg * GM + i][ni], 0, 0, 0);
            }
            __builtin_amdgcn_sched_group_barrier(0x100, NI + GM, 0);
#pragma unroll
            for (int gg = 0; gg < NG; ++gg)
#pragma unroll
                for (int i = 0; i < GM; ++i) {
                    if (gg + 1 < NG) __builtin_amdgcn_sched_group_barrier(0x100, 1, 0);
                    __builtin_amdgcn_sched_group_barrier(0x008, NI, 0);
                }
        }
        ++kt;
        if (++kx == 3) {
            kx = 0; ++g;
            if (++ky == 3) { ky = 0; ++cs; }
        }
    }

    gemm_epilogue_bf16<MI, NI, WM, WN>(p, acc, smem_t, m0, n0, z, wave, lane, HoWo);
}

template <int NI, int WF>
static hipError_t launch_cfg_bf16t(const ConvGemm& p, dim3 grid, hipStream_t stream) {
    auto k = conv3_gemm_bf16t_kernel<NI, WF>;
    constexpr size_t lds = 2 * (size_t)(((256 / (16 * WF)) * (16 * WF + 2) + 7) / 8 * 8 + 64 * NI) * 128;
    static_assert(lds <= 160 * 1024, "two activation + two weight buffers must fit the CU's LDS");
    if (hipError_t e = set_max_dynamic_lds(reinterpret_cast<const void*>(k), (int)lds); e != hipSuccess) return e;
    hipLaunchKernelGGL(k, grid, dim3(512), lds, stream, p);
    return hipGetLastError();
}

hipError_t launch_conv_gemm_bf16t(const ConvGemm& p, int cfg, hipStream_t stream) {
    if (p.z_aux) return hipErrorInvalidValue;
    if (cfg < 0 || cfg >= kNumGemmTilesT || !conv_gemm_bf16t_supported(p, p.kt_per_split)) return hipErrorInvalidValue;
    const int bm = gemm_tile_info_t(cfg).bm, bn = gemm_tile_info_t(cfg).bn;
    const int MT = p.M / bm, NT = (p.N + bn - 1) / bn;
    const dim3 grid = gemm_grid(p, MT * NT);
    const int wf = p.Ws / 16;
#define SDMI_T(NI_)                                                              \
    switch (wf) {                                                                \
        case 1: return launch_cfg_bf16t<NI_, 1>(p, grid, stream);                \
        case 2: return launch_cfg_bf16t<NI_, 2>(p, grid, stream);                \
        case 4: return launch_cfg_bf16t<NI_, 4>(p, grid, stream);                \
        case 8: return launch_cfg_bf16t<NI_, 8>(p, grid, stream);                \
    }
    if (cfg == 0) { SDMI_T(5) } else { SDMI_T(4) }
#undef SDMI_T
    return hipErrorInvalidValue;
}

}
```

### stable_diffusion_burn_amd/csrc/k_gemm_bf16x.hip

```cpp
#include "kernels.hpp"
#include "k_common.hpp"
#include "k_gemm_bf16_epi.hpp"

namespace sdmi {

typedef float f32x4 __attribute__((ext_vector_type(4)));
typedef unsigned int u32x4 __attribute__((ext_vector_type(4)));
typedef unsigned int u32x2 __attribute__((ext_vector_type(2)));
typedef __bf16 bf16x8 __attribute__((ext_vector_type(8)));
typedef __attribute__((address_space(3))) void lds_void;
typedef __attribute__((address_space(1))) const void global_cvoid;

template <int MI, int NI, int WM, int WN, int PM, bool LIN = false>
__global__ __launch_bounds__(512) void conv_gemm_bf16x_kernel(const ConvGemm p) {
    constexpr bool PERSIST = PM >= 0;
    constexpr int BM = 16 * MI * WM;
    constexpr int BN = 16 * NI * WN;
    static_assert(WM * WN == 8, "8 waves per workgroup");
    static_assert(BM % 64 == 0 && BN % 64 == 0, "every wave issues whole 8-row DMA pieces");
    constexpr int NA = BM / 64;
    constexpr int NB = BN / 64;
    constexpr int STAGE = (BM + BN) * 128;

    extern __shared__ __attribute__((aligned(16))) unsigned char smem_x[];
// ... 261 lines not shown
template <int MI, int NI, int WM, int WN>
static hipError_t launch_persist_bf16x(const ConvGemm& p, int mode, dim3 grid, hipStream_t stream) {
    const bool lin = p.KH * p.KW == 1 && p.stride == 1 && p.pad == 0 && p.ups == 0 && p.Ho == p.Hs && p.Wo == p.Ws;
    if (mode == 0) return lin ? launch_cfg_bf16x<MI, NI, WM, WN, 0, true>(p, grid, stream) : launch_cfg_bf16x<MI, NI, WM, WN, 0>(p, grid, stream);
    if constexpr (NI % 2 == 0) {
        if (mode == 2) return lin ? launch_cfg_bf16x<MI, NI, WM, WN, 2, true>(p, grid, stream) : launch_cfg_bf16x<MI, NI, WM, WN, 2>(p, grid, stream);
    }
    return hipErrorInvalidValue;
}

static int persistent_workgroups() {
    static int n_cu[64] = {};
    int dev = 0;
    if (hipGetDevice(&dev) != hipSuccess || dev < 0 || dev >= 64) return 256;
    if (!n_cu[dev]) {
        int v = 0;
        if (hipDeviceGetAttribute(&v, hipDeviceAttributeMultiprocessorCount, dev) != hipSuccess || v <= 0) v = 256;
        n_cu[dev] = (v / 8) * 8 > 0 ? (v / 8) * 8 : 8;
    }
    return n_cu[dev];
}

int conv_gemm_bf16x_persistent_mode(const ConvGemm& p, int cfg) {
    if (!(p.variant & 1) || p.splits != 1 || cfg < 0 || cfg >= kNumGemmTilesX || p.out_mode == 1) return -1;
    if ((p.N & 7) || (p.ldc & 7) || (p.resid && !(p.resid_acc & 1))) return -1;
    const int bm = kTilesX[cfg].bm, bn = kTilesX[cfg].bn;
    const int bno = p.geglu ? bn / 2 : bn;
    const long long tiles = (long long)((p.M + bm - 1) / bm) * ((p.N + bno - 1) / bno);
    if (tiles <= persistent_workgroups()) return -1;
    return p.geglu ? 2 : 0;
}

hipError_t launch_conv_gemm_bf16x(const ConvGemm& p, int cfg, hipStream_t stream) {
    if (p.z_aux) return hipErrorInvalidValue;
    if (cfg < 0 || cfg >= kNumGemmTilesX) return hipErrorInvalidValue;
    if ((p.Cin % 64) || !p.zero_page) return hipErrorInvalidValue;
    if (p.geglu && (cfg == 0 || cfg == 3 || p.splits != 1 || (p.N & 7) || (p.ldc & 7) || p.rowvec || p.resid)) return hipErrorInvalidValue;
    const int bm = kTilesX[cfg].bm, bn = kTilesX[cfg].bn;
    const int bno = p.geglu ? bn / 2 : bn;
    const int MT = (p.M + bm - 1) / bm, NT = (p.N + bno - 1) / bno;
    const int tiles = MT * NT;
    if (const int mode = conv_gemm_bf16x_persistent_mode(p, cfg); mode >= 0) {
        const dim3 grid((unsigned)persistent_workgroups(), 1, 1);
        switch (cfg) {
            case 0: return launch_persist_bf16x<8, 5, 2, 4>(p, mode, grid, stream);
            case 1: return launch_persist_bf16x<8, 4, 2, 4>(p, mode, grid, stream);
            case 2: return launch_persist_bf16x<4, 4, 4, 2>(p, mode, grid, stream);
            case 3: return launch_persist_bf16x<4, 5, 2, 4>(p, mode, grid, stream);
        }
    }
    const dim3 grid = gemm_grid(p, tiles);
    switch (cfg) {
        case 0: return launch_cfg_bf16x<8, 5, 2, 4, -1>(p, grid, stream);
        case 1: return launch_cfg_bf16x<8, 4, 2, 4, -1>(p, grid, stream);
        case 2: return launch_cfg_bf16x<4, 4, 4, 2, -1>(p, grid, stream);
        case 3: return launch_cfg_bf16x<4, 5, 2, 4, -1>(p, grid, stream);
    }
    return hipErrorInvalidValue;
}

}
```

### stable_diffusion_burn_amd/csrc/k_gemm_epi.hpp

```cpp
#pragma once
#include "kernels.hpp"
#include "k_common.hpp"
#include "k_split3.hpp"

namespace sdmi {

typedef float epi_f32x4 __attribute__((ext_vector_type(4)));

template <int MI, int NI, int WM, int WN>
__device__ __forceinline__ void gemm_epilogue_f32(const ConvGemm& p, epi_f32x4 (&acc)[MI][NI], unsigned char* smem_x32, const int m0,
                                                  const int n0, const int z, const int lid, const int wave, const int lane,
                                                  const int HoWo) {
    typedef epi_f32x4 f32x4;
    constexpr int BM = 16 * MI * WM;
    constexpr int BN = 16 * NI * WN;
    constexpr int WNC = 16 * NI;
    const int wm = wave / WN;
    const int wn = wave - wm * WN;
    const int c15 = lane & 15, g4 = lane >> 4;
    const bool geglu = p.geglu != 0;
    const bool split = p.splits > 1;
    float* Cf = split ? (p.slabs + (long long)z * p.slab_stride) : p.C;
    const int ldc = split ? p.N : p.ldc;
    const bool has_resid = !split && p.resid;
    const bool vec_ok = ((p.N & 3) == 0) && ((ldc & 3) == 0) && ((p.ldr & 3) == 0 || !has_resid);
    constexpr int LDSW = WNC + 4;
    if (p.geglu == 2) {
        if constexpr (WN % 2 == 0) {
            constexpr int HWN = WN / 2;
            const int vg = wn / HWN, col = wn - vg * HWN;
            const int pw = wm * WN + (vg ? wn - HWN : wn + HWN);
            __syncthreads();
            float* scr = reinterpret_cast<float*>(smem_x32 + wave * (16 * LDSW * 4));
            const float* scr_v = reinterpret_cast<const float*>(smem_x32 + (vg ? pw : wave) * (16 * LDSW * 4));
            const float* scr_g = reinterpret_cast<const float*>(smem_x32 + (vg ? wave : pw) * (16 * LDSW * 4));
            const int nw0 = n0 + col * WNC;
            const float* bias = p.bias ? p.bias + (vg ? p.N : 0) : nullptr;
            f32x4 bias_g[NI];
#pragma unroll
            for (int ni = 0; ni < NI; ++ni) {
                const int n = nw0 + ni * 16 + g4 * 4;
                bias_g[ni] = f32x4{0.f, 0.f, 0.f, 0.f};
                if (bias && n < p.N) bias_g[ni] = *reinterpret_cast<const f32x4*>(bias + n);
            }
#pragma unroll
            for (int mi = 0; mi < MI; ++mi) {
                const int mrow0 = m0 + (wm * MI + mi) * 16;
#pragma unroll
                for (int ni = 0; ni < NI; ++ni) {
                    const int n = nw0 + ni * 16 + g4 * 4;
                    f32x4 v = acc[mi][ni];
                    if (bias && n < p.N) v += bias_g[ni];
                    *reinterpret_cast<f32x4*>(scr + c15 * LDSW + ni * 16 + g4 * 4) = v;
                }
                __syncthreads();
// ... 26 lines not shown
            float* scr = reinterpret_cast<float*>(smem_x32 + wave * (16 * LDSW2 * 4));
            const int nw0 = n0 + wn * WNO;
#pragma unroll
            for (int mi = 0; mi < MI; ++mi) {
                const int mrow0 = m0 + (wm * MI + mi) * 16;
#pragma unroll
                for (int j = 0; j < NI / 2; ++j) {
                    const int n = nw0 + j * 16 + g4 * 4;
                    f32x4 v = acc[mi][2 * j], g = acc[mi][2 * j + 1];
                    if (p.bias && n < p.N) {
                        v += *reinterpret_cast<const f32x4*>(p.bias + n);
                        g += *reinterpret_cast<const f32x4*>(p.bias + p.N + n);
                    }
                    f32x4 o;
#pragma unroll
                    for (int e = 0; e < 4; ++e) o[e] = v[e] * (0.5f * g[e] * (1.0f + erff(g[e] * 0.70710678118654752440f)));
                    *reinterpret_cast<f32x4*>(scr + c15 * LDSW2 + j * 16 + g4 * 4) = o;
                }
                __builtin_amdgcn_wave_barrier();
                constexpr int CH = WNO / 4;
#pragma unroll
                for (int q0 = 0; q0 < 16 * CH; q0 += 64) {
                    const int q = q0 + lane;
                    const int row = q / CH, c4 = q - row * CH;
                    const int m = mrow0 + row, n = nw0 + c4 * 4;
                    if (q < 16 * CH && m < p.M && n < p.N)
                        *reinterpret_cast<f32x4*>(p.C + (long long)m * p.ldc + n) = *reinterpret_cast<const f32x4*>(scr + row * LDSW2 + c4 * 4);
                }
                __builtin_amdgcn_wave_barrier();
            }
        }
        return;
    }
    if (!(p.variant & 64) && vec_ok && m0 + BM <= p.M && n0 + BN <= p.N) {
        int smp0 = 0;
        bool one_smp = true;
        if (!split && p.rowvec) {
            smp0 = m0 / HoWo;
            one_smp = (m0 + BM - 1) / HoWo == smp0;
        }
        if (one_smp) {
            typedef unsigned int u2 __attribute__((ext_vector_type(2)));
            const int wu = __builtin_amdgcn_readfirstlane(wave);
            const int wmu = wu / WN, wnu = wu - wmu * WN;
            constexpr int CH = WNC / 4;
            __syncthreads();
            float* scr = reinterpret_cast<float*>(smem_x32 + wu * (16 * LDSW * 4));
            const int nw0 = n0 + wnu * WNC;
            const bool has_c3 = !split && p.C3;
            f32x4 bias_v[NI];
#pragma unroll
            for (int ni = 0; ni < NI; ++ni) {
                const int n = nw0 + ni * 16 + g4 * 4;
                bias_v[ni] = f32x4{0.f, 0.f, 0.f, 0.f};
                if (!split && p.bias) bias_v[ni] = *reinterpret_cast<const f32x4*>(p.bias + n);
                if (!split && p.rowvec) bias_v[ni] += *reinterpret_cast<const f32x4*>(p.rowvec + (long long)smp0 * p.rowvec_stride + n);
            }
            float* wr = scr + c15 * LDSW + g4 * 4;
            const float* rd[NI];
            unsigned goff[NI], roff[NI], poff[NI];
#pragma unroll
            for (int r = 0; r < NI; ++r) {
                const int q = r * 64 + lane, row = q / CH, c4 = q - row * CH;
                rd[r] = scr + row * LDSW + c4 * 4;
                goff[r] = (unsigned)(row * ldc + c4 * 4) * 4u;
                roff[r] = has_resid ? (unsigned)(row * p.ldr + c4 * 4) * 4u : 0u;
                poff[r] = has_c3 ? (unsigned)(row * p.ldc3) + (unsigned)s3_plane_byte(nw0 + c4 * 4, 0) : 0u;
// ... 83 lines not shown
#pragma unroll
        for (int mi = 0; mi < MI; ++mi) {
            const int mrow0 = m0 + (wm * MI + mi) * 16;
            {
                const int m = mrow0 + c15;
                const int smp = (m < p.M ? m : 0) / HoWo;
#pragma unroll
                for (int ni = 0; ni < NI; ++ni) {
                    const int n = nw0 + ni * 16 + g4 * 4;
                    f32x4 v = acc[mi][ni];
                    if (!split && n < p.N) {
                        f32x4 cv = bias_v[ni];
                        if (!early && p.bias) cv = *reinterpret_cast<const f32x4*>(p.bias + n);
                        if (p.rowvec) cv += *reinterpret_cast<const f32x4*>(p.rowvec + (long long)smp * p.rowvec_stride + n);
                        v += cv;
                    }
                    *reinterpret_cast<f32x4*>(scr + c15 * LDSW + ni * 16 + g4 * 4) = v;
                }
            }
            __builtin_amdgcn_wave_barrier();
#pragma unroll
            for (int r = 0; r < NQ; ++r) {
                const int q = r * 64 + lane;
                const int row = q / CH, c4 = q - row * CH;
                const int m = mrow0 + row, n = nw0 + c4 * 4;
                if (q < 16 * CH && m < p.M && n < p.N) {
                    f32x4 v = *reinterpret_cast<const f32x4*>(scr + row * LDSW + c4 * 4);
                    if (has_resid) {
                        if (PRE_R && early) v += res_v[PRE_R ? mi : 0][PRE_R ? r : 0];
                        else v += *reinterpret_cast<const f32x4*>(p.resid + (long long)m * p.ldr + n);
                    }
                    if (split) *reinterpret_cast<f32x4*>(Cf + (long long)m * ldc + n) = v;
                    else {
                        if (Cf) *reinterpret_cast<f32x4*>(Cf + (long long)m * ldc + n) = v;
                        if (p.C3) s3_store4(reinterpret_cast<unsigned char*>(p.C3) + (long long)m * p.ldc3, n, v);
                    }
                }
            }
            __builtin_amdgcn_wave_barrier();
        }
    } else {
#pragma unroll
    for (int mi = 0; mi < MI; ++mi) {
        const int m = m0 + (wm * MI + mi) * 16 + c15;
        if (m >= p.M) continue;
        const int smp = m / HoWo;
#pragma unroll
        for (int ni = 0; ni < NI; ++ni) {
            const int n = n0 + (wn * NI + ni) * 16 + g4 * 4;
            if (n >= p.N) continue;
            const f32x4 v = acc[mi][ni];
#pragma unroll
            for (int r = 0; r < 4; ++r) {
                if (n + r < p.N) {
                    float sv = v[r];
                    if (!split) {
                        float cv = p.bias ? p.bias[n + r] : 0.f;
                        if (p.rowvec) cv += p.rowvec[(long long)smp * p.rowvec_stride + n + r];
                        sv += cv;
                        if (p.resid) sv += p.resid[(long long)m * p.ldr + n + r];
                    }
                    Cf[(long long)m * ldc + n + r] = sv;
                }
            }
        }
    }
    }
}

}
```

### stable_diffusion_burn_amd/csrc/kernels.hpp

```cpp
#pragma once
#include <hip/hip_runtime.h>
#include <stdint.h>
#include "attn_plan.hpp"
#include "gemm_tiles.hpp"

namespace sdmi {

struct ConvGemm {
    const float* A;
    const float* Bt;
    const void* Bt3;
    int b3_grouped;
    const void* A3;
    int a3_ld;
    float* C;
    void* C3;
    int ldc3;
    float* slabs;
    const float* bias;
    const float* rowvec;
    const float* resid;
    int M, N, K;
    int NB, Hs, Ws, Cin;
    int Ho, Wo;
    int KH, KW, stride, pad, ups;
    int ldc, ldr;
    int a_ld;
    int b_ld;
    int rowvec_stride;
    int CS;
    int kt_total;
    int kt_per_split;
    int splits;
    long long slab_stride;
    unsigned a_bytes, b_bytes;
    int out_mode;
    const void* zero_page;
    const void* a_scale;
    const void* b_scale;
    int variant;
    int resid_acc;
    int geglu;
    unsigned long long* probe;
    const void* A3_aux;
    int a3_ld_aux;
    const void* Bt3_aux;
    int Cin_aux, kt_total_aux;
    int z_aux;
    const float* bias_aux;
};

constexpr int kGemmProbeBlocks = 1 << 13;

inline dim3 gemm_grid(const ConvGemm& p, int tiles) {
    return dim3((unsigned)(((tiles + 7) / 8) * 8), 1, (unsigned)p.splits);
}

hipError_t launch_conv_gemm2(const ConvGemm& p, int tile_cfg, hipStream_t stream);
size_t gemm2_tile_lds_bytes(int cfg);
hipError_t launch_conv_gemm_bf16(const ConvGemm& p, int tile_cfg, hipStream_t stream);
hipError_t launch_splitk_reduce_bf16(const ConvGemm& p, hipStream_t stream);
hipError_t launch_conv_gemm_bf16x(const ConvGemm& p, int tile_cfg, hipStream_t stream);
hipError_t launch_conv_gemm_bf16t(const ConvGemm& p, int tile_cfg, hipStream_t stream);
inline hipError_t launch_conv_gemm_bf16_large(const ConvGemm& p, int c, hipStream_t stream) {
    return c < kNumGemmTilesX ? launch_conv_gemm_bf16x(p, c, stream) : launch_conv_gemm_bf16t(p, c - kNumGemmTilesX, stream);
}
hipError_t launch_conv_gemm2x(const ConvGemm& p, int tile_cfg, hipStream_t stream);
hipError_t launch_conv_gemm3x(const ConvGemm& p, int tile_cfg, hipStream_t stream);
hipError_t launch_pack_split3(const float* bt, void* w3, long long rows, int K, hipStream_t s, bool grouped = false);
hipError_t launch_conv_gemm3p(const ConvGemm& p, int tile_cfg, hipStream_t stream);
hipError_t launch_split3_rows(const float* x, void* y3, long long rows, int c, long long ld, long long ld3_bytes, hipStream_t s);
hipError_t launch_join3_rows(const void* x3, float* y, long long rows, int c, long long ld3_bytes, long long ld, hipStream_t s);
hipError_t set_max_dynamic_lds(const void* kernel, int bytes);
hipError_t launch_conv_gemm_fp8x(const ConvGemm& p, int tile_cfg, hipStream_t stream);
hipError_t launch_pack_conv_weight_fp8(const float* w_oihw, void* bt8, void* bs, int cout, int cin, int kh, int kw, hipStream_t s);
struct GnTune;
hipError_t launch_group_norm_fp8(const void* x, void* y8, void* y_scale, const float* gamma, const float* beta, int n, int hw, int c,
                                 int ldx, int n_group, float eps, bool silu, void* partials, hipStream_t stream, const GnTune* t = nullptr);
hipError_t launch_quantize_fp8(const float* x, void* q, void* s, long long rows, int c, hipStream_t stream);
hipError_t launch_quantize_bf16_fp8(const void* x, void* q, void* s, long long rows, int c, int ldx, hipStream_t stream);
hipError_t launch_layer_norm_fp8(const void* x, void* y8, void* y_scale, const float* gamma, const float* beta, int rows, int c, float eps, hipStream_t stream);
hipError_t launch_geglu_fp8(const void* proj, void* y8, void* y_scale, long long rows, int hidden, hipStream_t stream);
hipError_t launch_pack_linear_weight_fp8(const float* w_in_out, void* bt8, void* bs, int cin, int cout, hipStream_t s);
hipError_t launch_dequant_fp8(const void* q, const void* s, float* out, long long rows, int c, hipStream_t stream);
hipError_t launch_pack_conv_weight_bf16(const float* w_oihw, void* bt, int cout, int cin, int kh, int kw, hipStream_t s);
hipError_t launch_pack_linear_weight_bf16(const float* w_in_out, void* bt, int cin, int cout, hipStream_t s);
hipError_t launch_splitk_reduce(const ConvGemm& p, hipStream_t stream);
__host__ __device__ inline bool splitk_reduce_vec(const ConvGemm& p, bool bf16) {
    const uintptr_t ra = bf16 ? 7 : 15, ca = (bf16 && p.out_mode != 1) ? 7 : 15;
    return ((p.N | p.ldc | p.rowvec_stride) & 3) == 0 && (!p.resid || (p.ldr & 3) == 0) && (((uintptr_t)p.bias | (uintptr_t)p.rowvec) & 15) == 0 &&
           ((uintptr_t)p.resid & ra) == 0 && ((uintptr_t)p.C & ca) == 0;
}
hipError_t launch_pack_conv_weight(const float* w_oihw, float* bt, int cout, int cin, int kh, int kw, hipStream_t s);
hipError_t launch_pack_linear_weight(const float* w_in_out, float* bt, int cin, int cout, hipStream_t s);
hipError_t launch_fold_matmul_f64(const float* a, const float* b, float* out, int N, int Cn, int K, long long lda, long long ldb, long long ldo, hipStream_t s);

struct AttnParams {
    const float* q; const float* k; const float* v; float* o;
    const int* kv_len;
    const float* mask;
    int mask_ld;
    int n, n_head, nq, nk, d_head;
    int ldq, ldk, ldv, ldo;
    long long q_bs, k_bs, v_bs, o_bs;
    float scale;
    int bf16;
    int q_log2;
    void* o3;
    int ldo3;
    int kv_splits;
    float* part_o;
    float* part_ml;
};
hipError_t launch_attention(const AttnParams& p, const AttnPlan& plan, hipStream_t stream);
hipError_t launch_attention_split(const AttnParams& p, const AttnPlan& plan, hipStream_t stream);
hipError_t launch_attention_combine(const AttnParams& p, hipStream_t stream);
inline float attn_bf16_q_scale(int d_head) { return (float)(1.4426950408889634 / __builtin_sqrt((double)d_head)); }
hipError_t launch_attention_bf16(const AttnParams& p, const AttnPlan& plan, hipStream_t stream);
hipError_t launch_softmax_rows(float* x, int rows, int cols, float scale, hipStream_t stream);

size_t gn_partials_bytes(int n, int hw, int c, int min_wgs = 0);
hipError_t launch_group_norm(const float* x, float* y, const float* gamma, const float* beta,
                             int n, int hw, int c, int ldx, int n_group, float eps, bool silu,
                             void* partials, hipStream_t stream, int min_wgs = 0);
hipError_t launch_layer_norm(const float* x, float* y, const float* gamma, const float* beta,
                             int rows, int c, float eps, hipStream_t stream);
hipError_t launch_group_norm_planes(const float* x, void* y3, const float* gamma, const float* beta, int n, int hw, int c, int ldx,
                                    int n_group, float eps, bool silu, void* partials, hipStream_t stream, int min_wgs = 0);
// ... 87 lines not shown
```

Before: 4.142.

## Fold nearest-upsample into 3x3 conv via four-phase 2x2 kernels

Adds a phase-decomposed path for 3x3 convolutions that follow a nearest-neighbour 2x upsample. Each of the four output phases gets its own folded 2x2 kernel, giving K = 4*Cin instead of 9*Cin, and reads the un-upsampled input. The phase GEMM scatters its rows into the interleaved output positions. This removes redundant MACs (16 instead of 36 taps per 2x2 output block) and avoids materializing the upsampled activation. The cost is extra folded weight storage, a new tuning table, and scatter stores that cannot use the fast vectorized epilogue path.

```diff
diff --git a/stable_diffusion_burn_amd/build.py b/stable_diffusion_burn_amd/build.py
--- a/stable_diffusion_burn_amd/build.py
+++ b/stable_diffusion_burn_amd/build.py
@@ -58,6 +58,7 @@
     _gen_table("gfx950_bf16.txt", "tuning_table_bf16.inc")
     _gen_table("gfx950_fp32_planes.txt", "tuning_table_planes.inc")
     _gen_table("gfx950_fp32_pairs.txt", "tuning_table_pairs.inc")
+    _gen_table("gfx950_fp32_phases.txt", "tuning_table_phases.inc")
 
 
 def _gen_table(src_name: str, out_name: str) -> None:
diff --git a/stable_diffusion_burn_amd/csrc/engine.cpp b/stable_diffusion_burn_amd/csrc/engine.cpp
--- a/stable_diffusion_burn_amd/csrc/engine.cpp
+++ b/stable_diffusion_burn_amd/csrc/engine.cpp
@@ -441,11 +441,18 @@
                 if (s.kind == BK_RES_UP || s.kind == BK_RES_ST_UP) { conv(b.up, path + "/upsample/conv", s.cout, s.cout, 3); fp8_copy(b.up, path + "/upsample/conv/weight"); }
         }
     };
+    auto reg_up = [&](ConvW& w, const std::string& weight_name) {
+        w.up_entry = entry_index_.at(weight_name);
+        entries_[(size_t)w.up_entry].fold_up = (int)up_list_.size();
+        up_list_.push_back(&w);
+    };
     for (int i = 0; i < 12; ++i) def_block(in_blocks_[i], in_spec[i], "unet/input_blocks");
     res(mid_res1_, "unet/middle_block/res1", c4, c4, true);
     spatial(mid_st_, "unet/middle_block/transformer", c4);
     res(mid_res2_, "unet/middle_block/res2", c4, c4, true);
     for (int i = 0; i < 12; ++i) def_block(out_blocks_[i], out_spec[i], "unet/output_blocks");
+    for (int i = 0; i < 12; ++i)
+        if (out_spec[i].kind == BK_RES_UP || out_spec[i].kind == BK_RES_ST_UP) reg_up(out_blocks_[i].up, std::string("unet/output_blocks/") + out_spec[i].name + "/upsample/conv/weight");
     norm(unet_norm_out_, "unet/norm_out", c1);
     conv(unet_conv_out_, "unet/conv_out", c1, 4, 3);
 
@@ -485,7 +492,7 @@
         res(b.res[0], bp + "/res1", b.cin, b.cout, false);
         res(b.res[1], bp + "/res2", b.cout, b.cout, false);
         res(b.res[2], bp + "/res3", b.cout, b.cout, false);
-        if (b.has_up) conv(b.upsampler, bp + "/upsampler", b.cout, b.cout, 3);
+        if (b.has_up) { conv(b.upsampler, bp + "/upsampler", b.cout, b.cout, 3); reg_up(b.upsampler, bp + "/upsampler/weight"); }
     }
     norm(dec_norm_out_, "autoencoder/decoder/norm_out", vc);
     conv(dec_conv_out_, "autoencoder/decoder/conv_out", vc, 3, 3);
@@ -1117,7 +1124,38 @@
         SDMI_HIP(launch_pack_split3(s->fold_bt, const_cast<void*>(split_planes(s->fold_bt)), C, 4 * C, stream_, b3_grouped(C)));
         s->fold_fresh = true;
     }
-}
+    for (ConvW* w : up_list_) {
+        if (w->up_fresh || w->up_entry < 0 || !entries_[(size_t)w->up_entry].set || !opt_ups_phase_ || !up_fold_supported(w->cin, w->cout) || !split_planes(w->bt)) continue;
+        if (!w->up3) {
+            w->up3 = persistent_alloc((size_t)w->cout * w->cin * 96);
+            weight_allocs_.push_back(w->up3);
+        }
+        build_up_fold(w->bt, w->up3, w->cout, w->cin);
+        w->up_fresh = true;
+    }
+}
+
+bool Engine::up_fold_supported(int cin, int cout) const {
+    return !bf16_ && cin % 32 == 0 && cout >= 32 && (unsigned long long)cout * (unsigned long long)(cin / 8) * 192ull < 0xFFFFFF00ull;
+}
+
+void Engine::build_up_fold(const float* bt, void* up3, int cout, int cin) {
+    Buf img(this, (size_t)4 * cout * cin * sizeof(float));
+    ProfScope ps(this, PC_OTHER, 0, ((double)9 + 16 + 16 + 24) * cout * cin * 4.0);
+    ps.set_tag("fold ups_phase %d,%d", cout, cin);
+    for (int ph = 0; ph < 4; ++ph) {
+        SDMI_HIP(launch_fold_ups_phase_f64(bt, img.f(), cout, cin, ph, 1, stream_));
+        SDMI_HIP(launch_pack_split3(img.f(), static_cast<char*>(up3) + (size_t)ph * cout * cin * 24, cout, 4 * cin, stream_, b3_grouped(cout)));
+    }
+}
+
+Engine::TempUpFold::TempUpFold(Engine* e_, ConvW& w, int stride, int ups) : e(e_) {
+    if (!e->opt_ups_phase_ || w.dt || w.k != 3 || stride != 1 || ups != 1 || !e->up_fold_supported(w.cin, w.cout) || !e->split_planes(w.bt)) return;
+    up3 = e->pool_.alloc((size_t)w.cout * w.cin * 96);
+    try { e->build_up_fold(w.bt, up3, w.cout, w.cin); } catch (...) { e->pool_.free(up3); up3 = nullptr; throw; }
+    w.up3 = up3; w.up_fresh = true;
+}
+Engine::TempUpFold::~TempUpFold() { if (up3) e->pool_.free(up3); }
 bool Engine::lora_owned(const sdmi_lora* a) const { return a && std::find(loras_.begin(), loras_.end(), a) != loras_.end(); }
 
 bool Engine::lora_active_on(int entry) const {
@@ -1528,6 +1566,16 @@
     else if (key == "gemm3x_variant") opt_gemm3x_variant_ = (value == "default") ? kGemm3xVariantDefault : std::stoi(value);
     else if (key == "gemm_bf16x_variant") opt_gemm_bf16x_variant_ = (value == "default") ? kGemmBf16xVariantDefault : std::stoi(value);
     else if (key == "geglu_fuse") opt_geglu_fuse_ = std::stoi(value);
+    else if (key == "ups_phase") {
+        const int v = (value == "default") ? 2 : std::stoi(value);
+        if (v < 0 || v > 2) throw Error(SDMI_ERR_INVALID, "ups_phase: 0 (never), 1 (wherever supported) or 2 (where the planner takes it)");
+        opt_ups_phase_ = v;
+        if (v && finalized_) {
+            SDMI_HIP(hipSetDevice(cfg_.device));
+            rebuild_folds();
+            SDMI_HIP(hipStreamSynchronize(stream_));
+        }
+    }
     else if (key == "record_shapes") { record_shapes_ = std::stoi(value) != 0; if (record_shapes_) { shape_counts_.clear(); choice_counts_.clear(); } }
     else if (key == "dump_shapes") {
         std::ofstream f(value);
@@ -1674,6 +1722,7 @@
     const int extra = pad_br ? 1 : 0;
     const int ho = (hin + 2 * pad + extra - w.k) / stride + 1, wo = (win + 2 * pad + extra - w.k) / stride + 1;
     if (y.n != x.n || y.h != ho || y.w != wo || y.c != w.cout) throw Error(SDMI_ERR_INVALID, "conv: output shape mismatch");
+    if (ups == 1 && stride == 1 && w.k == 3 && !pad_br && conv_ups_phase(w, x, y, rowvec, resid)) return;
     ConvGemm p{};
     const int resid_dt = (!x.dt && y.dt) ? 0 : y.dt;
     if (resid && !x.dt && y.dt && (w.cout % 4 || y.stride() % 4 || resid->stride() % 4))
@@ -1693,6 +1742,74 @@
     if (x.dt != w.dt) throw Error(SDMI_ERR_STATE, "conv: activation / weight storage types disagree");
     p.out_mode = x.dt ? (y.dt ? 0 : 1) : (y.dt ? 2 : 0);
     launch_gemm(p, x.dt);
+}
+
+bool Engine::conv_ups_phase(const ConvW& w, const Act& x, Act& y, const float* rowvec, const Act* resid) {
+    if (!opt_ups_phase_ || bf16_ || x.dt || y.dt || w.dt || w.k != 3 || !w.up3 || !w.up_fresh || probe_buf_) return false;
+    if (x.c != w.cin || !plane_gemm(w.cin, w.cout) || !up_fold_supported(w.cin, w.cout) || (!x.p3 && !x.p) || (!y.p && !y.p3)) return false;
+    ConvGemm p{};
+    p.A = x.p; p.Bt = w.bt; p.bias = w.bias;
+    p.Bt3 = split_planes(w.bt);
+    if (!p.Bt3) return false;
+    p.A3 = x.p3; p.a3_ld = x.ld3;
+    p.C = y.p; p.C3 = y.p3; p.ldc3 = y.ld3;
+    p.M = (int)y.rows(); p.N = w.cout; p.K = w.cin * 9;
+    p.NB = x.n; p.Hs = x.h; p.Ws = x.w; p.Cin = w.cin; p.Ho = 2 * x.h; p.Wo = 2 * x.w;
+    p.KH = 3; p.KW = 3; p.stride = 1; p.pad = 1; p.ups = 1;
+    p.ldc = y.p ? y.stride() : p.N; p.ldr = p.ldc; p.a_ld = x.stride(); p.b_ld = p.K; p.CS = 32;
+    p.kt_total = p.K / 32;
+    p.variant = opt_gemm3x_variant_;
+    p.zero_page = zero_page_;
+    const GemmPlanIn in = gemm_plan_in(p, 0, -1, 0);
+    const UpsPhasePlan g = plan_ups_phase(in, w.up_fresh, opt_ups_phase_, gopt_, tuning_);
+    if (!g.take) return false;
+    if ((p.N % 4) || (p.C && p.ldc % 4)) { if (p.C3 || opt_ups_phase_ != 1) return false; }
+    if (rowvec || resid) {
+        if (opt_ups_phase_ != 1) return false;
+        throw Error(SDMI_ERR_INVALID, "conv: ups_phase=1 with a time-embedding row or a residual: a phase launch carries the bias only");
+    }
+    if (record_shapes_) {
+        char sk[96];
+        std::snprintf(sk, sizeof sk, "%d,%d,%d,%d,%d,%d,%d,%d", p.NB, p.Cin, p.Hs, p.Ws, p.N, 3, 1, 1);
+        ++shape_counts_[sk];
+        p.splits = g.splits;
+        record_choice(p, " phase", g.cfg, "");
+    }
+    std::unique_ptr<Buf> a3_tmp;
+    if (!p.A3) {
+        const long long rows = (long long)p.NB * p.Hs * p.Ws;
+        p.a3_ld = (p.Cin / 32) * 192;
+        a3_tmp.reset(new Buf(this, (size_t)rows * p.a3_ld));
+        ProfScope ps(this, PC_SPLIT_ROWS, 0, (double)rows * p.Cin * 10.0);
+        SDMI_HIP(launch_split3_rows(p.A, a3_tmp->p, rows, p.Cin, p.a_ld, p.a3_ld, stream_));
+        count_kernel();
+        p.A3 = a3_tmp->p;
+    }
+    p.Bt3 = w.up3; p.phases = 4; p.phase_stride = (long long)w.cout * w.cin * 24;
+    p.b3_grouped = b3_grouped(p.N) ? 1 : 0;
+    p.M = g.M; p.K = g.K; p.kt_total = g.kt_total; p.b_ld = p.K;
+    p.kt_per_split = g.kt_per_split; p.splits = g.splits;
+    const double flops = 2.0 * 4.0 * p.M * (double)p.N * p.K;
+    const double bytes = (double)p.M * p.Cin * 6.0 + 4.0 * p.N * (double)p.K * 6.0 + 4.0 * p.M * (double)p.N * ((p.C ? 4.0 : 0.0) + (p.C3 ? 6.0 : 0.0));
+    std::unique_ptr<Buf> slab;
+    if (p.splits > 1) {
+        p.slab_stride = 4ll * p.M * p.N;
+        slab.reset(new Buf(this, (size_t)p.splits * p.slab_stride * sizeof(float)));
+        p.slabs = slab->f();
+    }
+    {
+        ProfScope ps(this, PC_CONV_SPLIT, flops, bytes);
+        ps.set_tag("gemm 4x%d,%d,%d k3 phase cfg=%d splits=%d", p.M, p.N, p.K, g.cfg, p.splits);
+        SDMI_HIP(launch_conv_gemm3p(p, g.tile.index, stream_));
+    }
+    count_kernel(flops);
+    if (p.splits > 1) {
+        ProfScope ps(this, PC_SPLITK_REDUCE, 0, (double)(p.splits + 1) * p.slab_stride * 4.0);
+        ps.set_tag("reduce 4x%d,%d,%d k3 phase cfg=%d splits=%d", p.M, p.N, p.K, g.cfg, p.splits);
+        SDMI_HIP(launch_splitk_reduce(p, stream_));
+        count_kernel();
+    }
+    return true;
 }
 
 bool Engine::conv_pair(const ConvW& w_out, const Act& h, const ConvW& w_skip, const Act& x, Act& y) {
@@ -3351,6 +3468,7 @@
     else SDMI_HIP(launch_pack_conv_weight(wt, bt.f(), cout, cin, k, k, stream_));
     TempSplit planes(this, bt.f(), w.dt ? 0 : cout, (long long)cin * k * k);
     w.bt = bt.f(); w.bias = const_cast<float*>(bias);
+    TempUpFold up_fold(this, w, stride, ups);
     Act a = new_act(n, h, wd, cin, w.dt);
     if (w.dt) SDMI_HIP(launch_nchw_f32_to_nhwc_bf16(x, a.p, n, cin, h, wd, 1.0f, stream_));
     else SDMI_HIP(launch_nchw_to_nhwc(x, a.p, n, cin, h, wd, 1.0f, stream_));
@@ -3503,6 +3621,7 @@
             else SDMI_HIP(launch_pack_conv_weight(wt, bt.f(), cout, cin, k, k, stream_));
             TempSplit planes(this, bt.f(), w.dt ? 0 : cout, (long long)cin * k * k);
             w.bt = bt.f(); w.bias = const_cast<float*>(bias);
+            TempUpFold up_fold(this, w, stride, ups);
             conv(w, xs, ys, stride, ups, temb, epi ? epi->temb_stride : 0, r.p ? &r : nullptr);
         }
     } catch (...) {
@@ -3821,6 +3940,7 @@
         SDMI_HIP(launch_split3_rows(a.p, a.p3, a.rows(), cin, cin, a.ld3, stream_));
     }
     ConvW cw; cw.cin = cin; cw.cout = cout; cw.k = k; cw.bt = bt.f(); cw.bias = bias.f(); cw.dt = wdt;
+    TempUpFold up_fold(this, cw, stride, ups);
     const OptRestore r1{gopt_.force_tile}, r2{gopt_.force_splits}, r3{gopt_.gemm_planes};
     gopt_.force_tile = tile_cfg; gopt_.force_splits = splitk;
     if (plane_tile && !gopt_.gemm_planes) gopt_.gemm_planes = 2;
diff --git a/stable_diffusion_burn_amd/csrc/engine.hpp b/stable_diffusion_burn_amd/csrc/engine.hpp
--- a/stable_diffusion_burn_amd/csrc/engine.hpp
+++ b/stable_diffusion_burn_amd/csrc/engine.hpp
@@ -65,7 +65,10 @@
     size_t bytes() const { return (size_t)rows() * c * (dt ? 2 : 4); }
 };
 
-struct ConvW { float* bt = nullptr; float* bias = nullptr; int cin = 0, cout = 0, k = 1; int dt = 0; float* bt8 = nullptr; float* bs8 = nullptr; };
+struct ConvW {
+    float* bt = nullptr; float* bias = nullptr; int cin = 0, cout = 0, k = 1; int dt = 0; float* bt8 = nullptr; float* bs8 = nullptr;
+    void* up3 = nullptr; bool up_fresh = false; int up_entry = -1;
+};
 struct ActQ {
     void* q = nullptr; void* s = nullptr;
     int n = 0, h = 0, w = 0, c = 0, cp = 0;
@@ -107,6 +110,7 @@
     float pre_scale = 1.f;
     bool set = false;
     int fold_st = -1;
+    int fold_up = -1;
     float* master = nullptr;
 };
 
@@ -314,7 +318,22 @@
     bool linear_pair(const LinearPair& a, bool plan_only = false);
     void fold_weights(const float* proj_bt, const float* lin_bt, const float* lin_bias, int cout, int cmid, int k_main, float* wf, float* bf);
     void rebuild_folds();
-    void fold_touch(const WeightEntry& e) { if (e.fold_st >= 0) st_list_[(size_t)e.fold_st]->fold_fresh = false; }
+    void fold_touch(const WeightEntry& e) {
+        if (e.fold_st >= 0) st_list_[(size_t)e.fold_st]->fold_fresh = false;
+        if (e.fold_up >= 0) up_list_[(size_t)e.fold_up]->up_fresh = false;
+    }
+    std::vector<ConvW*> up_list_;
+    int opt_ups_phase_ = 2;
+    void build_up_fold(const float* bt, void* up3, int cout, int cin);
+    bool up_fold_supported(int cin, int cout) const;
+    bool conv_ups_phase(const ConvW& w, const Act& x, Act& y, const float* rowvec, const Act* resid);
+    struct TempUpFold {
+        Engine* e; void* up3 = nullptr;
+        TempUpFold(Engine* e_, ConvW& w, int stride, int ups);
+        ~TempUpFold();
+        TempUpFold(const TempUpFold&) = delete;
+        TempUpFold& operator=(const TempUpFold&) = delete;
+    };
     static Act slice(const Act& parent, int c_off, int c);
     void gemm(const float* A, int a_rows, const float* bt, const float* bias, int cin, int cout, float* C, int ldc,
               const float* resid, int ldr, int dt = -1, int out_mode = 0, const void* A3 = nullptr, void* C3 = nullptr);
diff --git a/stable_diffusion_burn_amd/csrc/gemm_plan.cpp b/stable_diffusion_burn_amd/csrc/gemm_plan.cpp
--- a/stable_diffusion_burn_amd/csrc/gemm_plan.cpp
+++ b/stable_diffusion_burn_amd/csrc/gemm_plan.cpp
@@ -22,6 +22,10 @@
 #include "tuning_table_pairs.inc"
     {nullptr, 0, 0}};
 
+static const TuneRow kPhaseRows[] = {
+#include "tuning_table_phases.inc"
+    {nullptr, 0, 0}};
+
 struct CostRow { int bf16; GemmFamily family; int n; double eff[kNumGemmTiles]; double flop, rate, wg, area_num, area_den; };
 static const CostRow kCost[] = {
     {0, kFam4, kNumGemmTiles, {0.85, 0.75, 0.60, 0.90, 0.75, 0.85, 0.75, 0.85, 0.65, 0.75}, 64.0, 256.0, 3000.0, 0.0, 1.0},
@@ -32,7 +36,7 @@
     {1, kFamX, kNumGemmTilesX, {0.54, 0.46, 0.38, 0.48}, 128.0, 4096.0, 6000.0, 2.0, 20.0}};
 static const int kSplitOpts[] = {1, 2, 3, 4, 6, 8, 12, 16, 24, 32, 48};
 
-static TileChoice cost_model(int bf16, unsigned families, int M, int N, int kt_total, bool pairs_only) {
+static TileChoice cost_model(int bf16, unsigned families, int M, int N, int kt_total, bool pairs_only, int phases = 1) {
     const int n_cu = 256;
     double best = 1e300;
     TileChoice bc{0, 1};
@@ -42,7 +46,7 @@
             const GemmTileInfo& ti = kGemmFamilies[r.family].tiles[c];
             if (pairs_only && !ti.geglu_pairs) continue;
             const int bm = ti.bm, bn = ti.bn;
-            const long long tiles = (long long)((M + bm - 1) / bm) * ((N + bn - 1) / bn);
+            const long long tiles = (long long)((M + bm - 1) / bm) * ((N + bn - 1) / bn) * phases;
             const double overhead = r.wg + bm * bn * r.area_num / r.area_den;
             for (int s : kSplitOpts) {
                 if (s > 1 && kt_total / s < 4) break;
@@ -50,7 +54,7 @@
                 const long long wgs = tiles * ((kt_total + kt_per - 1) / kt_per);
                 const double per_cu = (double)((wgs + n_cu - 1) / n_cu);
                 double t = per_cu * ((double)bm * bn * kt_per * r.flop / r.rate / r.eff[c] + overhead);
-                if (s > 1) t += 8000.0 + (double)M * N * 4.0 * (s + 1) / (5.0e12 / 2.4e9);
+                if (s > 1) t += 8000.0 + (double)M * phases * N * 4.0 * (s + 1) / (5.0e12 / 2.4e9);
                 if (t < best) { best = t; bc = {kGemmFamilies[r.family].base + c, s}; }
             }
         }
@@ -85,6 +89,8 @@
         else ++t;
     for (const TuneRow& r : kPairRows)
         if (r.key) pairs[r.key] = TileChoice{r.cfg, r.splits};
+    for (const TuneRow& r : kPhaseRows)
+        if (r.key) phases[r.key] = TileChoice{r.cfg, r.splits};
 }
 
 void GemmTuning::set(const std::string& value, bool b16) {
@@ -95,6 +101,12 @@
         if (std::sscanf(value.c_str() + eq + 1, "%d,%d", &tc.cfg, &tc.splits) != 2 || tc.splits < 0 || gemm_tile_id(tc.cfg).family != kFamP || !gemm_tile_id(tc.cfg).in_range(false))
             throw Error(SDMI_ERR_INVALID, "tune: a pair row is M,N,Kmain+Kaux=cfg,kt_per_split with a plane tile (300 + x)");
         pairs[value.substr(0, eq)] = tc;
+        return;
+    }
+    if (!b16 && value.compare(0, 3, "ph:") == 0) {
+        if (std::sscanf(value.c_str() + eq + 1, "%d,%d", &tc.cfg, &tc.splits) != 2 || tc.splits < 0 || gemm_tile_id(tc.cfg).family != kFamP || !gemm_tile_id(tc.cfg).in_range(false))
+            throw Error(SDMI_ERR_INVALID, "tune: a phase row is ph:M/4,N,4Cin=cfg,splits with a plane tile (300 + x)");
+        phases[value.substr(3, eq - 3)] = tc;
         return;
     }
     if (std::sscanf(value.c_str() + eq + 1, "%d,%d", &tc.cfg, &tc.splits) != 2 || tc.cfg < 0 || tc.splits < 1 || !gemm_tile_id(tc.cfg).in_range(b16))
@@ -186,6 +198,37 @@
     return pp;
 }
 
+UpsPhasePlan plan_ups_phase(const GemmPlanIn& layer, bool fold_fresh, int ups_phase, const GemmPlanOpts& o, const GemmTuning& t) {
+    UpsPhasePlan pp{};
+    if (ups_phase == 0 || !fold_fresh) return pp;
+    if (layer.bf16 || layer.geglu || layer.out_mode != 0 || layer.KH != 3 || layer.KW != 3 || layer.stride != 1 || layer.pad != 1 || layer.ups != 1) return pp;
+    if (!layer.p_ok || !o.gemm_planes || !o.gemm_f32s || layer.Cin % 32 || layer.Ho != 2 * layer.Hs || layer.Wo != 2 * layer.Ws || layer.M % 4) return pp;
+    const int forced = layer.force_cfg >= 0 ? layer.force_cfg : o.force_tile;
+    if (forced >= 0 && gemm_tile_id(forced).family != kFamP) return pp;
+    if (ups_phase != 1 && (!layer.from_planes || forced >= 0)) return pp;
+    pp.M = layer.M / 4; pp.K = 4 * layer.Cin; pp.kt_total = layer.Cin / 8;
+    char key[64];
+    std::snprintf(key, sizeof key, "%d,%d,%d", pp.M, layer.N, pp.K);
+    TileChoice tc;
+    if (const TileChoice* row = find(t.phases, key)) {
+        if (row->splits <= 0 && ups_phase != 1) return pp;
+        tc = *row;
+        if (tc.splits <= 0) tc.splits = 1;
+    } else {
+        if (ups_phase != 1 && pp.M < kUpsPhaseMinRows) return pp;
+        tc = cost_model(0, 1u << kFamP, pp.M, layer.N, pp.kt_total, false, 4);
+    }
+    if (forced >= 0) tc.cfg = forced;
+    if (o.force_splits > 0) tc.splits = o.force_splits;
+    if (layer.force_splits > 0) tc.splits = layer.force_splits;
+    const GemmTileId tile = gemm_tile_id(tc.cfg);
+    if (tile.family != kFamP || !tile.in_range(false)) throw Error(SDMI_ERR_INVALID, "gemm: a phase launch needs a plane tile (300 + x)");
+    pp.tile = tile; pp.cfg = tile.cfg();
+    pp.splits = clamp_splits(tc.splits, pp.kt_total, &pp.kt_per_split);
+    pp.take = true;
+    return pp;
+}
+
 TileChoice plan_gemm_fp8(int M, int N, int kt_total, int fp8_tile, int force_splits, int* kt_per_split) {
     static const double kRate[kNumGemmTilesQ] = {2400.0, 2100.0, 1700.0};
     if (fp8_tile >= kNumGemmTilesQ) throw Error(SDMI_ERR_INVALID, "fp8_tile out of range");
diff --git a/stable_diffusion_burn_amd/csrc/gemm_plan.hpp b/stable_diffusion_burn_amd/csrc/gemm_plan.hpp
--- a/stable_diffusion_burn_amd/csrc/gemm_plan.hpp
+++ b/stable_diffusion_burn_amd/csrc/gemm_plan.hpp
@@ -37,7 +37,8 @@
     std::map<std::string, TileChoice> pairs;
     void load_builtin();
     void set(const std::string& value, bool b16);
-    void clear() { f32.clear(); mfma.clear(); planes.clear(); bf16.clear(); pairs.clear(); }
+    std::map<std::string, TileChoice> phases;
+    void clear() { f32.clear(); mfma.clear(); planes.clear(); bf16.clear(); pairs.clear(); phases.clear(); }
 };
 
 struct GemmPlan { GemmTileId tile; int cfg, splits, kt_per_split; bool tile_forced; };
@@ -46,6 +47,9 @@
 
 struct GemmPairPlan { bool pair; GemmTileId tile; int cfg, kt_per_split, splits_main, splits_aux; };
 GemmPairPlan plan_gemm_pair(const GemmPlanIn& main, int k_aux, int kt_aux, const GemmPlanOpts& o, const GemmTuning& t, int force_main = 0, int force_aux = 0);
+constexpr int kUpsPhaseMinRows = 256;
+struct UpsPhasePlan { bool take; GemmTileId tile; int cfg, splits, kt_per_split, M, K, kt_total; };
+UpsPhasePlan plan_ups_phase(const GemmPlanIn& layer, bool fold_fresh, int ups_phase, const GemmPlanOpts& o, const GemmTuning& t);
 TileChoice plan_gemm_fp8(int M, int N, int kt_total, int fp8_tile, int force_splits, int* kt_per_split);
 int plan_geglu_plane_tile(long long rows, int hidden, int cin, const GemmPlanOpts& o, const GemmTuning& t);
 int plan_geglu_paired_tile(long long rows, int hidden, int fuse, bool f32s);
diff --git a/stable_diffusion_burn_amd/csrc/k_fp8.hip b/stable_diffusion_burn_amd/csrc/k_fp8.hip
--- a/stable_diffusion_burn_amd/csrc/k_fp8.hip
+++ b/stable_diffusion_burn_amd/csrc/k_fp8.hip
@@ -250,7 +250,7 @@
 }
 
 hipError_t launch_conv_gemm_fp8x(const ConvGemm& p, int cfg, hipStream_t stream) {
-    if (p.z_aux) return hipErrorInvalidValue;
+    if (p.z_aux || p.phases) return hipErrorInvalidValue;
     if (cfg < 0 || cfg >= kNumGemmTilesQ) return hipErrorInvalidValue;
     if ((p.a_ld % 128) || (p.b_ld % 128) || !p.zero_page || !p.a_scale || !p.b_scale || p.geglu) return hipErrorInvalidValue;
     if ((p.N & 7) || (p.ldc & 7) || (p.resid && (p.ldr & 7))) return hipErrorInvalidValue;
diff --git a/stable_diffusion_burn_amd/csrc/k_gemm.hip b/stable_diffusion_burn_amd/csrc/k_gemm.hip
--- a/stable_diffusion_burn_amd/csrc/k_gemm.hip
+++ b/stable_diffusion_burn_amd/csrc/k_gemm.hip
@@ -30,7 +30,7 @@
     const bool vec_ok = splitk_reduce_vec(p, false);
     if (vec_ok) {
         const int n4 = p.N >> 2;
-        const long long total = (long long)p.M * n4;
+        const long long total = (long long)p.M * (p.phases ? p.phases : 1) * n4;
         const long long rounded = (total * G + 255) / 256 * 256;
         for (long long t = (long long)blockIdx.x * blockDim.x + threadIdx.x; t < rounded; t += (long long)gridDim.x * blockDim.x) {
             const long long i = t / G;
@@ -40,6 +40,8 @@
             const int m = (int)(ii / n4);
             const int n = (int)(ii - (long long)m * n4) * 4;
             const long long off = (long long)m * p.N + n;
+            long long mo = m;
+            if (p.phases) { const int ph = m / p.M; mo = ups_phase_row(m - ph * p.M, ph, p.Hs, p.Ws); }
             f32x4 eb = {0.f, 0.f, 0.f, 0.f}, ev = eb, er = eb;
             if (live && g == 0) {
                 if (p.bias) eb = *reinterpret_cast<const f32x4*>(p.bias + n);
@@ -66,12 +68,12 @@
                 if (p.bias || p.bias_aux) v += eb;
                 if (p.rowvec) v += ev;
                 if (p.resid) v += er;
-                if (C) *reinterpret_cast<f32x4*>(C + (long long)m * p.ldc + n) = v;
-                if (p.C3) s3_store4(reinterpret_cast<unsigned char*>(p.C3) + (long long)m * p.ldc3, n, v);
+                if (C) *reinterpret_cast<f32x4*>(C + mo * p.ldc + n) = v;
+                if (p.C3) s3_store4(reinterpret_cast<unsigned char*>(p.C3) + mo * p.ldc3, n, v);
             }
         }
     } else {
-        const long long total = (long long)p.M * p.N;
+        const long long total = (long long)p.M * (p.phases ? p.phases : 1) * p.N;
         for (long long i = (long long)blockIdx.x * blockDim.x + threadIdx.x; i < total;
              i += (long long)gridDim.x * blockDim.x) {
             const int m = (int)(i / p.N);
@@ -82,7 +84,9 @@
             else if (p.bias) v += p.bias[n];
             if (p.rowvec) v += p.rowvec[(long long)(m / HoWo) * p.rowvec_stride + n];
             if (p.resid) v += p.resid[(long long)m * p.ldr + n];
-            C[(long long)m * p.ldc + n] = v;
+            long long mo = m;
+            if (p.phases) { const int ph = m / p.M; mo = ups_phase_row(m - ph * p.M, ph, p.Hs, p.Ws); }
+            C[mo * p.ldc + n] = v;
         }
     }
 }
@@ -138,6 +142,34 @@
     if (n < N && k < K) out[(long long)n * ldo + k] = (float)acc;
 }
 
+__global__ __launch_bounds__(256) void fold_ups_phase_f64_kernel(const float* __restrict__ bt, float* __restrict__ out, int N, int Cin, int ph0, int nph) {
+    const long long K4 = 4ll * Cin, K9 = 9ll * Cin;
+    const long long total = (long long)nph * N * K4;
+    for (long long i = (long long)blockIdx.x * blockDim.x + threadIdx.x; i < total; i += (long long)gridDim.x * blockDim.x) {
+        const int pi = (int)(i / (N * K4));
+        const long long r = i - pi * (N * K4);
+        const int ph = ph0 + pi;
+        const int n = (int)(r / K4), k = (int)(r - n * K4);
+        const int sl = k >> 5, ci = k & 31, cs = sl >> 2, a = (sl >> 1) & 1, b = sl & 1;
+        const int py = ph >> 1, px = ph & 1;
+        const int ky0 = a ? (py ? 2 : 1) : 0, ky1 = a ? 2 : (py ? 1 : 0);
+        const int kx0 = b ? (px ? 2 : 1) : 0, kx1 = b ? 2 : (px ? 1 : 0);
+        double acc = 0.0;
+        for (int ky = ky0; ky <= ky1; ++ky)
+            for (int kx = kx0; kx <= kx1; ++kx) acc += (double)bt[n * K9 + (long long)(cs * 9 + ky * 3 + kx) * 32 + ci];
+        out[i] = (float)acc;
+    }
+}
+
+hipError_t launch_fold_ups_phase_f64(const float* bt, float* out, int N, int Cin, int ph0, int nph, hipStream_t s) {
+    if (N <= 0 || Cin <= 0 || (Cin % 32) || ph0 < 0 || nph < 1 || ph0 + nph > 4) return hipErrorInvalidValue;
+    const long long total = 4ll * nph * N * Cin;
+    long long blocks = (total + 255) / 256;
+    if (blocks > 8192) blocks = 8192;
+    hipLaunchKernelGGL(fold_ups_phase_f64_kernel, dim3((unsigned)blocks), dim3(256), 0, s, bt, out, N, Cin, ph0, nph);
+    return hipGetLastError();
+}
+
 hipError_t launch_fold_matmul_f64(const float* a, const float* b, float* out, int N, int Cn, int K, long long lda, long long ldb, long long ldo, hipStream_t s) {
     if (N <= 0 || Cn <= 0 || K <= 0 || lda < Cn || ldb < K || ldo < K) return hipErrorInvalidValue;
     const dim3 grid((unsigned)((K + 15) / 16), (unsigned)((N + 15) / 16));
@@ -151,7 +183,8 @@
     if (!vec && (p.C3 || !p.C)) return hipErrorInvalidValue;
     if (p.z_aux && p.rowvec) return hipErrorInvalidValue;
     if (p.bias_aux && vec && ((uintptr_t)p.bias_aux & 15)) return hipErrorInvalidValue;
-    const long long work = ((long long)p.M * p.N + 3) / 4;
+    if (p.phases && (p.phases != 4 || p.rowvec || p.resid || p.z_aux || p.bias_aux || p.slab_stride != 4ll * p.M * p.N)) return hipErrorInvalidValue;
+    const long long work = ((long long)p.M * (p.phases ? p.phases : 1) * p.N + 3) / 4;
     int g = 1;
     if (vec)
         while (g < 8 && work * g < 262144 && 4 * g <= p.splits) g *= 2;
diff --git a/stable_diffusion_burn_amd/csrc/k_gemm2.hip b/stable_diffusion_burn_amd/csrc/k_gemm2.hip
--- a/stable_diffusion_burn_amd/csrc/k_gemm2.hip
+++ b/stable_diffusion_burn_amd/csrc/k_gemm2.hip
@@ -283,7 +283,7 @@
 }
 
 hipError_t launch_conv_gemm2(const ConvGemm& p, int cfg, hipStream_t stream) {
-    if (p.z_aux) return hipErrorInvalidValue;
+    if (p.z_aux || p.phases) return hipErrorInvalidValue;
     if (cfg < 0 || cfg >= kNumGemmTiles) return hipErrorInvalidValue;
     const int bm = gemm_tile_info(cfg).bm, bn = gemm_tile_info(cfg).bn;
     const int MT = (p.M + bm - 1) / bm, NT = (p.N + bn - 1) / bn;
diff --git a/stable_diffusion_burn_amd/csrc/k_gemm2x.hip b/stable_diffusion_burn_amd/csrc/k_gemm2x.hip
--- a/stable_diffusion_burn_amd/csrc/k_gemm2x.hip
+++ b/stable_diffusion_burn_amd/csrc/k_gemm2x.hip
@@ -189,7 +189,7 @@
 }
 
 hipError_t launch_conv_gemm2x(const ConvGemm& p, int cfg, hipStream_t stream) {
-    if (p.z_aux) return hipErrorInvalidValue;
+    if (p.z_aux || p.phases) return hipErrorInvalidValue;
     if (cfg < 0 || cfg >= kNumGemmTilesX) return hipErrorInvalidValue;
     if ((p.Cin % 32) || p.CS != 32 || !p.zero_page || p.out_mode != 0) return hipErrorInvalidValue;
     if (p.geglu && (cfg == 0 || cfg == 3 || p.splits != 1 || (p.N & 7) || (p.ldc & 7) || p.rowvec || p.resid)) return hipErrorInvalidValue;
diff --git a/stable_diffusion_burn_amd/csrc/k_gemm3p.hip b/stable_diffusion_burn_amd/csrc/k_gemm3p.hip
--- a/stable_diffusion_burn_amd/csrc/k_gemm3p.hip
+++ b/stable_diffusion_burn_amd/csrc/k_gemm3p.hip
@@ -152,10 +152,12 @@
     const int BNO = geglu ? BN / 2 : BN;
     const int MT = (p.M + BM - 1) / BM;
     const int NT = (p.N + BNO - 1) / BNO;
-    const GemmWork gw = gemm_work_of_block(p, MT, NT);
+    const bool phased = p.phases != 0;
+    const GemmWork gw = gemm_work_of_block(p, phased ? p.phases * MT : MT, NT);
     if (!gw.live) return;
     const int lid = gw.lid;
-    const int m0 = gw.tm * BM;
+    const int phase = phased ? gw.tm / MT : 0;
+    const int m0 = (gw.tm - phase * MT) * BM;
     const int n0 = gw.tn * BNO;
     const int z = gw.z;
     const bool aux = p.z_aux != 0 && z >= p.z_aux;
@@ -163,21 +165,24 @@
     const int kt_begin = (aux ? z - p.z_aux : z) * p.kt_per_split;
     const int kt_end = min(kt_begin + p.kt_per_split, kt_total);
     const int n_t = kt_end - kt_begin;
-    const int KH = aux ? 1 : p.KH, KW = aux ? 1 : p.KW, pad = aux ? 0 : p.pad;
+    const int KH = aux ? 1 : phased ? 2 : p.KH, KW = aux ? 1 : phased ? 2 : p.KW;
+    const int pad_y = aux ? 0 : phased ? 1 - (phase >> 1) : p.pad, pad_x = aux ? 0 : phased ? 1 - (phase & 1) : p.pad;
+    const int stride = phased ? 1 : p.stride, ups = phased ? 0 : p.ups;
+    const int Wo = phased ? p.Ws : p.Wo;
     const int T = KH * KW;
-    const int HoWo = p.Ho * p.Wo;
+    const int HoWo = phased ? p.Hs * p.Ws : p.Ho * p.Wo;
 
     P3Wave<MI, NI, NAG, NBW, A_BYTES, NWV> w;
-    w.Hin = p.Hs << p.ups;
-    w.Win = p.Ws << p.ups;
-    w.ups = p.ups;
+    w.Hin = p.Hs << ups;
+    w.Win = p.Ws << ups;
+    w.ups = ups;
     w.Ws = p.Ws;
     w.KH = KH;
     w.KW = KW;
     w.wave = wave;
     w.pix_bytes = (unsigned)(aux ? p.a3_ld_aux : p.a3_ld);
     w.Abase = reinterpret_cast<const char*>(aux ? p.A3_aux : p.A3);
-    w.Wbase = reinterpret_cast<const char*>(aux ? p.Bt3_aux : p.Bt3);
+    w.Wbase = reinterpret_cast<const char*>(aux ? p.Bt3_aux : p.Bt3) + (phased ? phase * p.phase_stride : 0ll);
     w.zero = reinterpret_cast<const char*>(p.zero_page);
     w.a_src = w.zero;
 
@@ -190,11 +195,11 @@
         const int mm = ok ? m : 0;
         const int nb = mm / HoWo;
         const int rem = mm - nb * HoWo;
-        const int oy = rem / p.Wo;
-        const int ox = rem - oy * p.Wo;
+        const int oy = rem / Wo;
+        const int ox = rem - oy * Wo;
         w.a_off[j] = (unsigned)nb * (unsigned)(p.Hs * p.Ws) * w.pix_bytes + ch * 16;
-        w.a_iy0[j] = ok ? oy * p.stride - pad : -(1 << 28);
-        w.a_ix0[j] = ox * p.stride - pad;
+        w.a_iy0[j] = ok ? oy * stride - pad_y : -(1 << 28);
+        w.a_ix0[j] = ox * stride - pad_x;
     }
     const unsigned w_row_bytes = (unsigned)kt_total * 192u;
 #pragma unroll
@@ -281,7 +286,7 @@
     unsigned long long pt2 = 0, pc2 = 0;
     if constexpr (PROBE) { pt2 = __builtin_amdgcn_s_memrealtime(); pc2 = __builtin_amdgcn_s_memtime(); }
 
-    gemm_epilogue_f32<MI, NI, WM, WN>(p, w.acc, smem_p3, m0, n0, z, lid, wave, lane, HoWo);
+    gemm_epilogue_f32<MI, NI, WM, WN, true>(p, w.acc, smem_p3, m0, n0, z, lid, wave, lane, HoWo, phase);
     if constexpr (PROBE) {
         asm volatile("s_waitcnt vmcnt(0)" ::: "memory");
         __syncthreads();
@@ -321,9 +326,17 @@
         if ((unsigned long long)p.N * (unsigned long long)p.kt_total_aux * 192ull >= 0xFFFFFF00ull) return hipErrorInvalidValue;
         if ((unsigned long long)p.NB * p.Hs * p.Ws * (unsigned long long)p.a3_ld_aux >= 0xFFFFFF00ull) return hipErrorInvalidValue;
     }
+    if (p.phases) {
+        if (p.phases != 4 || p.KH != 3 || p.KW != 3 || p.stride != 1 || p.pad != 1 || p.ups != 1 || p.Ho != 2 * p.Hs || p.Wo != 2 * p.Ws) return hipErrorInvalidValue;
+        if ((long long)p.M != (long long)p.NB * p.Hs * p.Ws || p.kt_total != p.Cin / 8 || p.K != 4 * p.Cin) return hipErrorInvalidValue;
+        if (p.rowvec || p.resid || p.geglu || p.z_aux || p.probe) return hipErrorInvalidValue;
+        if (p.phase_stride < (long long)p.N * p.kt_total * 192ll || (p.phase_stride % 16)) return hipErrorInvalidValue;
+        if (p.splits > 1 && (!p.slabs || p.slab_stride != 4ll * p.M * p.N)) return hipErrorInvalidValue;
+        if ((!p.C && !p.C3) || 4ll * p.M >= (1ll << 31)) return hipErrorInvalidValue;
+    }
     const int bm = kTilesP[cfg].bm, bn = kTilesP[cfg].bn;
     const int bno = p.geglu ? bn / 2 : bn;
-    const int MT = (p.M + bm - 1) / bm, NT = (p.N + bno - 1) / bno;
+    const int MT = ((p.M + bm - 1) / bm) * (p.phases ? p.phases : 1), NT = (p.N + bno - 1) / bno;
     const dim3 grid = gemm_grid(p, MT * NT);
     if (p.probe) {
         if ((unsigned long long)grid.x * grid.z > (unsigned long long)kGemmProbeBlocks) return hipErrorInvalidValue;
diff --git a/stable_diffusion_burn_amd/csrc/k_gemm3x.hip b/stable_diffusion_burn_amd/csrc/k_gemm3x.hip
--- a/stable_diffusion_burn_amd/csrc/k_gemm3x.hip
+++ b/stable_diffusion_burn_amd/csrc/k_gemm3x.hip
@@ -278,7 +278,7 @@
 }
 
 hipError_t launch_conv_gemm3x(const ConvGemm& p, int cfg, hipStream_t stream) {
-    if (p.z_aux) return hipErrorInvalidValue;
+    if (p.z_aux || p.phases) return hipErrorInvalidValue;
     if (cfg < 0 || cfg >= kNumGemmTilesS) return hipErrorInvalidValue;
     if ((p.Cin % 32) || p.CS != 32 || !p.zero_page || !p.Bt3 || p.out_mode != 0) return hipErrorInvalidValue;
     const bool odd_ni = (cfg == 0 || cfg == 1 || cfg == 4);
diff --git a/stable_diffusion_burn_amd/csrc/k_gemm_bf16.hip b/stable_diffusion_burn_amd/csrc/k_gemm_bf16.hip
--- a/stable_diffusion_burn_amd/csrc/k_gemm_bf16.hip
+++ b/stable_diffusion_burn_amd/csrc/k_gemm_bf16.hip
@@ -376,7 +376,7 @@
 }
 
 hipError_t launch_conv_gemm_bf16(const ConvGemm& p, int cfg, hipStream_t stream) {
-    if (p.z_aux) return hipErrorInvalidValue;
+    if (p.z_aux || p.phases) return hipErrorInvalidValue;
     if (cfg < 0 || cfg >= kNumGemmTiles) return hipErrorInvalidValue;
     if (p.Cin % 64) return hipErrorInvalidValue;
     const int bm = gemm_tile_info(cfg).bm, bn = gemm_tile_info(cfg).bn;
@@ -400,7 +400,7 @@
 }
 
 hipError_t launch_splitk_reduce_bf16(const ConvGemm& p, hipStream_t stream) {
-    if (p.z_aux) return hipErrorInvalidValue;
+    if (p.z_aux || p.phases) return hipErrorInvalidValue;
     const bool vec = splitk_reduce_vec(p, true);
     const long long work = (long long)p.M * p.N / (vec ? 4 : 1);
     int blocks = (int)((work + 255) / 256);
diff --git a/stable_diffusion_burn_amd/csrc/k_gemm_bf16t.hip b/stable_diffusion_burn_amd/csrc/k_gemm_bf16t.hip
--- a/stable_diffusion_burn_amd/csrc/k_gemm_bf16t.hip
+++ b/stable_diffusion_burn_amd/csrc/k_gemm_bf16t.hip
@@ -186,7 +186,7 @@
 }
 
 hipError_t launch_conv_gemm_bf16t(const ConvGemm& p, int cfg, hipStream_t stream) {
-    if (p.z_aux) return hipErrorInvalidValue;
+    if (p.z_aux || p.phases) return hipErrorInvalidValue;
     if (cfg < 0 || cfg >= kNumGemmTilesT || !conv_gemm_bf16t_supported(p, p.kt_per_split)) return hipErrorInvalidValue;
     const int bm = gemm_tile_info_t(cfg).bm, bn = gemm_tile_info_t(cfg).bn;
     const int MT = p.M / bm, NT = (p.N + bn - 1) / bn;
diff --git a/stable_diffusion_burn_amd/csrc/k_gemm_bf16x.hip b/stable_diffusion_burn_amd/csrc/k_gemm_bf16x.hip
--- a/stable_diffusion_burn_amd/csrc/k_gemm_bf16x.hip
+++ b/stable_diffusion_burn_amd/csrc/k_gemm_bf16x.hip
@@ -317,7 +317,7 @@
 }
 
 hipError_t launch_conv_gemm_bf16x(const ConvGemm& p, int cfg, hipStream_t stream) {
-    if (p.z_aux) return hipErrorInvalidValue;
+    if (p.z_aux || p.phases) return hipErrorInvalidValue;
     if (cfg < 0 || cfg >= kNumGemmTilesX) return hipErrorInvalidValue;
     if ((p.Cin % 64) || !p.zero_page) return hipErrorInvalidValue;
     if (p.geglu && (cfg == 0 || cfg == 3 || p.splits != 1 || (p.N & 7) || (p.ldc & 7) || p.rowvec || p.resid)) return hipErrorInvalidValue;
diff --git a/stable_diffusion_burn_amd/csrc/k_gemm_epi.hpp b/stable_diffusion_burn_amd/csrc/k_gemm_epi.hpp
--- a/stable_diffusion_burn_amd/csrc/k_gemm_epi.hpp
+++ b/stable_diffusion_burn_amd/csrc/k_gemm_epi.hpp
@@ -7,10 +7,10 @@
 
 typedef float epi_f32x4 __attribute__((ext_vector_type(4)));
 
-template <int MI, int NI, int WM, int WN>
+template <int MI, int NI, int WM, int WN, bool PH = false>
 __device__ __forceinline__ void gemm_epilogue_f32(const ConvGemm& p, epi_f32x4 (&acc)[MI][NI], unsigned char* smem_x32, const int m0,
                                                   const int n0, const int z, const int lid, const int wave, const int lane,
-                                                  const int HoWo) {
+                                                  const int HoWo, const int phase = 0) {
     typedef epi_f32x4 f32x4;
     constexpr int BM = 16 * MI * WM;
     constexpr int BN = 16 * NI * WN;
@@ -20,7 +20,9 @@
     const int c15 = lane & 15, g4 = lane >> 4;
     const bool geglu = p.geglu != 0;
     const bool split = p.splits > 1;
-    float* Cf = split ? (p.slabs + (long long)z * p.slab_stride) : p.C;
+    bool phased = false;
+    if constexpr (PH) phased = p.phases != 0;
+    float* Cf = split ? (p.slabs + (long long)z * p.slab_stride + (phased ? (long long)phase * p.M * p.N : 0ll)) : p.C;
     const int ldc = split ? p.N : p.ldc;
     const bool has_resid = !split && p.resid;
     const bool vec_ok = ((p.N & 3) == 0) && ((ldc & 3) == 0) && ((p.ldr & 3) == 0 || !has_resid);
@@ -113,7 +115,7 @@
         }
         return;
     }
-    if (!(p.variant & 64) && vec_ok && m0 + BM <= p.M && n0 + BN <= p.N) {
+    if (!(p.variant & 64) && !phased && vec_ok && m0 + BM <= p.M && n0 + BN <= p.N) {
         int smp0 = 0;
         bool one_smp = true;
         if (!split && p.rowvec) {
@@ -263,8 +265,9 @@
                     }
                     if (split) *reinterpret_cast<f32x4*>(Cf + (long long)m * ldc + n) = v;
                     else {
-                        if (Cf) *reinterpret_cast<f32x4*>(Cf + (long long)m * ldc + n) = v;
-                        if (p.C3) s3_store4(reinterpret_cast<unsigned char*>(p.C3) + (long long)m * p.ldc3, n, v);
+                        const long long mo = phased ? ups_phase_row(m, phase, p.Hs, p.Ws) : (long long)m;
+                        if (Cf) *reinterpret_cast<f32x4*>(Cf + mo * ldc + n) = v;
+                        if (p.C3) s3_store4(reinterpret_cast<unsigned char*>(p.C3) + mo * p.ldc3, n, v);
                     }
                 }
             }
@@ -276,6 +279,7 @@
         const int m = m0 + (wm * MI + mi) * 16 + c15;
         if (m >= p.M) continue;
         const int smp = m / HoWo;
+        const long long mo = (phased && !split) ? ups_phase_row(m, phase, p.Hs, p.Ws) : (long long)m;
 #pragma unroll
         for (int ni = 0; ni < NI; ++ni) {
             const int n = n0 + (wn * NI + ni) * 16 + g4 * 4;
@@ -291,7 +295,7 @@
                         sv += cv;
                         if (p.resid) sv += p.resid[(long long)m * p.ldr + n + r];
                     }
-                    Cf[(long long)m * ldc + n + r] = sv;
+                    Cf[mo * ldc + n + r] = sv;
                 }
             }
         }
diff --git a/stable_diffusion_burn_amd/csrc/kernels.hpp b/stable_diffusion_burn_amd/csrc/kernels.hpp
--- a/stable_diffusion_burn_amd/csrc/kernels.hpp
+++ b/stable_diffusion_burn_amd/csrc/kernels.hpp
@@ -48,7 +48,16 @@
     int Cin_aux, kt_total_aux;
     int z_aux;
     const float* bias_aux;
+    int phases;
+    long long phase_stride;
 };
+
+__host__ __device__ inline long long ups_phase_row(int m, int ph, int Hs, int Ws) {
+    const int hw = Hs * Ws;
+    const int nb = m / hw, rem = m - nb * hw;
+    const int y = rem / Ws, x = rem - y * Ws;
+    return ((long long)nb * (2 * Hs) + 2 * y + (ph >> 1)) * (2 * Ws) + 2 * x + (ph & 1);
+}
 
 constexpr int kGemmProbeBlocks = 1 << 13;
 
@@ -94,6 +103,7 @@
 hipError_t launch_pack_conv_weight(const float* w_oihw, float* bt, int cout, int cin, int kh, int kw, hipStream_t s);
 hipError_t launch_pack_linear_weight(const float* w_in_out, float* bt, int cin, int cout, hipStream_t s);
 hipError_t launch_fold_matmul_f64(const float* a, const float* b, float* out, int N, int Cn, int K, long long lda, long long ldb, long long ldo, hipStream_t s);
+hipError_t launch_fold_ups_phase_f64(const float* bt, float* out, int N, int Cin, int ph0, int nph, hipStream_t s);
 
 struct AttnParams {
     const float* q; const float* k; const float* v; float* o;
diff --git a/stable_diffusion_burn_amd/csrc/tuning_table_phases.inc b/stable_diffusion_burn_amd/csrc/tuning_table_phases.inc
--- /dev/null
+++ b/stable_diffusion_burn_amd/csrc/tuning_table_phases.inc
@@ -0,0 +1,6 @@
+{"128,1280,5120", 303, 8},
+{"512,1280,5120", 300, 4},
+{"2048,640,2560", 300, 2},
+{"4096,512,2048", 301, 1},
+{"16384,512,2048", 301, 1},
+{"65536,256,1024", 301, 1},
```

Measured after the change: 4.242 (median of 6 runs). 2.4% higher.
